# emmyoh/zebra

Measured on NVIDIA B200. Metric: queries_per_sec, higher is better.
Workload: dtype f32

## Files before the change

include/zebra_b200.h:

```cpp
#ifndef ZEBRA_B200_H
#define ZEBRA_B200_H

#include <stddef.h>
#include <stdint.h>

#ifdef __cplusplus
extern "C" {
#endif

#define ZB_ABI_VERSION 2

typedef struct zb_index zb_index;

typedef enum zb_status {
    ZB_OK = 0,
    ZB_ERR_INVALID = -1,
    ZB_ERR_CUDA = -2,
    ZB_ERR_NO_DEVICE = -3,
    ZB_ERR_OOM = -4,
    ZB_ERR_STATE = -5,
    ZB_ERR_COMM = -6
} zb_status;

typedef enum zb_metric {
    ZB_METRIC_COSINE = 0, ZB_METRIC_L2SQ = 1, ZB_METRIC_L2 = 2,
    ZB_METRIC_CHEBYSHEV = 3, ZB_METRIC_CANBERRA = 4, ZB_METRIC_BRAY_CURTIS = 5, ZB_METRIC_MANHATTAN = 6,
    ZB_METRIC_L3 = 7, ZB_METRIC_L4 = 8, ZB_METRIC_HAMMING = 9, ZB_METRIC_MINKOWSKI = 10, ZB_METRIC_PNORM = 11
} zb_metric;
#define ZB_METRIC_COUNT 12
#define ZB_METRIC_MAX_POWER 64

typedef struct zb_options {
    uint32_t dim;
    uint32_t metric;
    uint64_t max_node_size;
    uint32_t num_trees;
    int32_t device;
    uint64_t seed;
    uint32_t shard_rank;
    uint32_t shard_count;
    int32_t metric_power;
    uint32_t reserved[3];
} zb_options;

typedef struct zb_stats {
    uint64_t rows;
    uint64_t live_rows;
    uint64_t total_rows;
    uint64_t nodes, planes, leaves;
    uint64_t device_bytes;
    uint64_t last_queries, last_visits, last_pairs;
    uint64_t last_tile_visits, last_tile_pairs;
    uint64_t last_moved_bytes;
    float last_ms_plan, last_ms_scan, last_ms_select, last_ms_merge, last_ms_total;
    uint32_t last_scan_launches, last_total_launches;
    float last_ms_tile_kernel;
    uint32_t last_tiles;
    uint32_t last_filter_flagged;
    uint64_t last_unique_bytes;
    uint32_t last_filter_rows;
    float last_ms_refine;
    uint32_t last_filter_used;
} zb_stats;

const char* zb_last_error(void);
int zb_abi_version(void);
int zb_device_count(int* out_count);

int zb_index_create(const zb_options* options, zb_index** out_index);
int zb_index_destroy(zb_index* index);
int zb_index_options(zb_index* index, zb_options* out);

int zb_index_add(zb_index* index, uint64_t n, const float* rows, const uint8_t* ids16, uint8_t* out_ids16,
                 uint64_t* out_ordinals);
int zb_index_add_device(zb_index* index, uint64_t n, const float* d_rows, const uint8_t* ids16, uint8_t* out_ids16,
                        uint64_t* out_ordinals);
int zb_index_add_owned_device(zb_index* index, uint64_t n_local, const float* d_rows, const uint64_t* ordinals,
                              uint64_t total_n);

int zb_index_remove(zb_index* index, uint64_t n, const uint8_t* ids16, uint8_t* out_removed);
int zb_index_remove_ordinals(zb_index* index, uint64_t n, const uint64_t* ordinals, uint8_t* out_removed);

int zb_index_deduplicate(zb_index* index, uint64_t* out_count, uint64_t* out_ordinals, uint8_t* out_ids16, uint64_t cap);

int zb_index_clear(zb_index* index);

int zb_index_no_vectors(zb_index* index, int* out);
int zb_index_no_trees(zb_index* index, int* out);

int zb_index_search_batch(zb_index* index, uint64_t nq, const float* queries, uint64_t top_k, uint8_t* out_ids16,
                          uint64_t* out_ordinals, uint64_t* out_dist_bits, uint32_t* out_counts);
int zb_index_search_batch_device(zb_index* index, uint64_t nq, const float* d_queries, uint64_t top_k,
                                 uint64_t* d_out_ordinals, uint64_t* d_out_dist_bits, uint32_t* d_out_counts);
int zb_index_search_slice(zb_index* index, uint64_t nq_total, const float* slice_queries, uint64_t top_k, uint8_t* out_ids16,
                          uint64_t* out_ordinals, uint64_t* out_dist_bits, uint32_t* out_counts);
int zb_index_search_slice_device(zb_index* index, uint64_t nq_total, const float* d_slice_queries, uint64_t top_k,
                                 uint64_t* d_out_ordinals, uint64_t* d_out_dist_bits, uint32_t* d_out_counts);
int zb_index_search_prefetch(zb_index* index, uint64_t n, const float* queries);

int zb_index_search_exact(zb_index* index, uint64_t nq, const float* queries, uint64_t top_k, uint8_t* out_ids16,
                          uint64_t* out_ordinals, uint64_t* out_dist_bits, uint32_t* out_counts);
int zb_index_search_exact_device(zb_index* index, uint64_t nq, const float* d_queries, uint64_t top_k,
                                 uint64_t* d_out_ordinals, uint64_t* d_out_dist_bits, uint32_t* d_out_counts);

#define ZB_MAX_PROBES 32
int zb_index_search_probe(zb_index* index, uint64_t nq, const float* queries, uint64_t top_k, uint32_t probes, uint8_t* out_ids16,
                          uint64_t* out_ordinals, uint64_t* out_dist_bits, uint32_t* out_counts);
int zb_index_search_probe_device(zb_index* index, uint64_t nq, const float* d_queries, uint64_t top_k, uint32_t probes,
                                 uint64_t* d_out_ordinals, uint64_t* d_out_dist_bits, uint32_t* d_out_counts);
int zb_index_search_slice_probe(zb_index* index, uint64_t nq_total, const float* slice_queries, uint64_t top_k, uint32_t probes,
                                uint8_t* out_ids16, uint64_t* out_ordinals, uint64_t* out_dist_bits, uint32_t* out_counts);
int zb_index_search_slice_probe_device(zb_index* index, uint64_t nq_total, const float* d_slice_queries, uint64_t top_k,
                                       uint32_t probes, uint64_t* d_out_ordinals, uint64_t* d_out_dist_bits,
                                       uint32_t* d_out_counts);

int zb_index_hash(zb_index* index, uint64_t n, const float* rows, uint64_t* out_keys, uint32_t* out_depths,
                  int32_t* out_leaves);
int zb_index_hash_device(zb_index* index, uint64_t n, const float* d_rows, uint64_t* d_out_keys,
                         uint32_t* d_out_depths, int32_t* d_out_leaves);

int zb_index_forest_sizes(zb_index* index, int64_t* sizes4);
int zb_index_export_forest(zb_index* index, int32_t* nodes, int32_t* roots, float* coef, float* cst,
                           int64_t* leaf_off, uint64_t* members);
int zb_index_load_forest(zb_index* index, uint64_t n, const float* rows, const uint8_t* ids16,
                         const int64_t* sizes4, const int32_t* nodes, const int32_t* roots, const float* coef,
                         const float* cst, const int64_t* leaf_off, const uint64_t* members);

int zb_tree_blob_decode(uint32_t dim, const uint8_t* blob, uint64_t bytes, int64_t* sizes4, int32_t* nodes, float* coef,
                        float* cst, int64_t* leaf_off, uint8_t* member_ids16);
int zb_tree_blob_encode(uint32_t dim, int64_t n_nodes, const int32_t* nodes, int32_t root, const float* coef,
                        const float* cst, const int64_t* leaf_off, const uint8_t* member_ids16, uint8_t* out,
                        uint64_t cap, uint64_t* out_bytes);
int zb_zebra_file_encode(const uint8_t* uuid16, uint32_t metric, int32_t power, uint64_t max_node_size,
                         uint64_t num_trees, uint8_t* out, uint64_t cap, uint64_t* out_bytes);
int zb_zebra_file_decode(const uint8_t* data, uint64_t bytes, uint32_t metric, uint8_t* out_uuid16, int32_t* out_power,
                         uint64_t* out_max_node_size, uint64_t* out_num_trees);

typedef struct zb_import_report {
    uint64_t rows_loaded;
    uint64_t missing_ids;
    uint64_t orphan_rows;
    uint64_t nodes, planes, leaves;
    uint32_t max_depth;
    uint32_t reserved[3];
} zb_import_report;
typedef struct zb_flat_store zb_flat_store;
int zb_store_flatten(uint32_t dim, uint64_t n, const uint8_t* ids16, uint32_t n_trees, const uint8_t* const* tree_blobs,
                     const uint64_t* tree_blob_bytes, zb_flat_store** out, zb_import_report* report);
int zb_flat_store_view(const zb_flat_store* store, int64_t* sizes4, const int32_t** nodes, const int32_t** roots,
                       const float** coef, const float** cst, const int64_t** leaf_off, const uint64_t** members,
                       const uint32_t** row_order, const uint32_t** orphan_rows);
int zb_flat_store_free(zb_flat_store* store);
int zb_index_import_store(zb_index* index, uint64_t n, const uint8_t* ids16, const float* rows, uint32_t n_trees,
                          const uint8_t* const* tree_blobs, const uint64_t* tree_blob_bytes, zb_import_report* report,
                          uint8_t* out_orphan_ids16, uint64_t orphan_cap);
int zb_index_export_rows(zb_index* index, uint64_t first_ordinal, uint64_t n, float* out_rows, uint8_t* out_ids16,
                         uint8_t* out_live);
int zb_index_export_tree_blob(zb_index* index, uint32_t tree, uint8_t* out, uint64_t cap, uint64_t* out_bytes);
int zb_index_export_tree_blobs(zb_index* index, uint8_t* out, uint64_t cap, uint64_t* out_blob_bytes, uint64_t* out_total);

int zb_index_load_flat(zb_index* index, uint64_t n, const float* rows, const uint8_t* ids16, uint32_t bits,
                       const float* coef, const float* cst);

int zb_index_stats(zb_index* index, zb_stats* out);
int zb_index_stream(zb_index* index, void** out_stream);
int zb_index_set_param(zb_index* index, const char* key, int64_t value);

int zb_comm_unique_id(uint8_t* out_id128);
int zb_index_comm_init(zb_index* index, const uint8_t* id128);

int zb_metric_distance_batch(int device, uint32_t metric, int32_t power, uint64_t n, uint32_t dim, const float* a,
                             const float* b, uint64_t* out_bits);
int zb_point_is_above_batch(int device, uint64_t n, uint32_t dim, const float* coef, const float* cst, const float* x,
                            uint8_t* out);

int zb_synth_fill_device(int device, float* d_out, uint64_t first_row, uint64_t row_stride, uint64_t n, uint32_t dim,
                         uint64_t seed, uint32_t kind);

#ifdef __cplusplus
}
#endif
#endif
```

zebra_b200/_ffi.py:

```python
from __future__ import annotations

import ctypes as C
import os

_HERE = os.path.dirname(os.path.abspath(__file__))
LIB_PATH = os.path.join(_HERE, "libzebra_b200.so")

ZB_OK = 0
METRIC_COSINE, METRIC_L2SQ, METRIC_L2 = 0, 1, 2
(METRIC_CHEBYSHEV, METRIC_CANBERRA, METRIC_BRAY_CURTIS, METRIC_MANHATTAN, METRIC_L3, METRIC_L4, METRIC_HAMMING,
 METRIC_MINKOWSKI, METRIC_PNORM) = range(3, 12)
METRIC_MAX_POWER = 64


class ZebraError(RuntimeError):
    def __init__(self, code: int, msg: str):
        super().__init__(f"zebra_b200 error {code}: {msg}")
        self.code = code


class Options(C.Structure):
    _fields_ = [
        ("dim", C.c_uint32),
        ("metric", C.c_uint32),
        ("max_node_size", C.c_uint64),
        ("num_trees", C.c_uint32),
        ("device", C.c_int32),
        ("seed", C.c_uint64),
        ("shard_rank", C.c_uint32),
        ("shard_count", C.c_uint32),
        ("metric_power", C.c_int32),
        ("reserved", C.c_uint32 * 3),
    ]


class Stats(C.Structure):
    _fields_ = [
        ("rows", C.c_uint64),
        ("live_rows", C.c_uint64),
        ("total_rows", C.c_uint64),
        ("nodes", C.c_uint64),
        ("planes", C.c_uint64),
        ("leaves", C.c_uint64),
        ("device_bytes", C.c_uint64),
        ("last_queries", C.c_uint64),
        ("last_visits", C.c_uint64),
        ("last_pairs", C.c_uint64),
        ("last_tile_visits", C.c_uint64),
        ("last_tile_pairs", C.c_uint64),
        ("last_moved_bytes", C.c_uint64),
        ("last_ms_plan", C.c_float),
        ("last_ms_scan", C.c_float),
        ("last_ms_select", C.c_float),
        ("last_ms_merge", C.c_float),
        ("last_ms_total", C.c_float),
        ("last_scan_launches", C.c_uint32),
        ("last_total_launches", C.c_uint32),
        ("last_ms_tile_kernel", C.c_float),
        ("last_tiles", C.c_uint32),
        ("last_filter_flagged", C.c_uint32),
        ("last_unique_bytes", C.c_uint64),
        ("last_filter_rows", C.c_uint32),
        ("last_ms_refine", C.c_float),
        ("last_filter_used", C.c_uint32),
    ]

    def as_dict(self):
        return {n: getattr(self, n) for n, _ in self._fields_ if not n.startswith("reserved")}


class ImportReport(C.Structure):
    _fields_ = [
        ("rows_loaded", C.c_uint64),
        ("missing_ids", C.c_uint64),
        ("orphan_rows", C.c_uint64),
        ("nodes", C.c_uint64),
        ("planes", C.c_uint64),
        ("leaves", C.c_uint64),
        ("max_depth", C.c_uint32),
        ("reserved", C.c_uint32 * 3),
    ]

    def as_dict(self):
        return {n: getattr(self, n) for n, _ in self._fields_ if not n.startswith("reserved")}


_vp, _u64, _u32, _i32, _i64 = C.c_void_p, C.c_uint64, C.c_uint32, C.c_int32, C.c_int64
SYMBOLS = {
    "zb_last_error": (C.c_char_p, []),
    "zb_abi_version": (C.c_int, []),
    "zb_device_count": (C.c_int, [_vp]),
    "zb_index_create": (C.c_int, [C.POINTER(Options), C.POINTER(_vp)]),
    "zb_index_destroy": (C.c_int, [_vp]),
    "zb_index_options": (C.c_int, [_vp, C.POINTER(Options)]),
    "zb_index_add": (C.c_int, [_vp, _u64, _vp, _vp, _vp, _vp]),
    "zb_index_add_device": (C.c_int, [_vp, _u64, _vp, _vp, _vp, _vp]),
    "zb_index_add_owned_device": (C.c_int, [_vp, _u64, _vp, _vp, _u64]),
    "zb_index_remove": (C.c_int, [_vp, _u64, _vp, _vp]),
    "zb_index_remove_ordinals": (C.c_int, [_vp, _u64, _vp, _vp]),
    "zb_index_deduplicate": (C.c_int, [_vp, C.POINTER(_u64), _vp, _vp, _u64]),
    "zb_index_clear": (C.c_int, [_vp]),
    "zb_index_no_vectors": (C.c_int, [_vp, _vp]),
    "zb_index_no_trees": (C.c_int, [_vp, _vp]),
    "zb_index_search_batch": (C.c_int, [_vp, _u64, _vp, _u64, _vp, _vp, _vp, _vp]),
    "zb_index_search_batch_device": (C.c_int, [_vp, _u64, _vp, _u64, _vp, _vp, _vp]),
    "zb_index_search_slice": (C.c_int, [_vp, _u64, _vp, _u64, _vp, _vp, _vp, _vp]),
    "zb_index_search_slice_device": (C.c_int, [_vp, _u64, _vp, _u64, _vp, _vp, _vp]),
    "zb_index_search_prefetch": (C.c_int, [_vp, _u64, _vp]),
    "zb_index_search_exact": (C.c_int, [_vp, _u64, _vp, _u64, _vp, _vp, _vp, _vp]),
    "zb_index_search_exact_device": (C.c_int, [_vp, _u64, _vp, _u64, _vp, _vp, _vp]),
    "zb_index_search_probe": (C.c_int, [_vp, _u64, _vp, _u64, C.c_uint32, _vp, _vp, _vp, _vp]),
    "zb_index_search_probe_device": (C.c_int, [_vp, _u64, _vp, _u64, C.c_uint32, _vp, _vp, _vp]),
    "zb_index_search_slice_probe": (C.c_int, [_vp, _u64, _vp, _u64, C.c_uint32, _vp, _vp, _vp, _vp]),
    "zb_index_search_slice_probe_device": (C.c_int, [_vp, _u64, _vp, _u64, C.c_uint32, _vp, _vp, _vp]),
    "zb_index_hash": (C.c_int, [_vp, _u64, _vp, _vp, _vp, _vp]),
    "zb_index_hash_device": (C.c_int, [_vp, _u64, _vp, _vp, _vp, _vp]),
    "zb_index_forest_sizes": (C.c_int, [_vp, _vp]),
    "zb_index_export_forest": (C.c_int, [_vp, _vp, _vp, _vp, _vp, _vp, _vp]),
    "zb_index_load_forest": (C.c_int, [_vp, _u64, _vp, _vp, _vp, _vp, _vp, _vp, _vp, _vp, _vp]),
    "zb_tree_blob_decode": (C.c_int, [_u32, _vp, _u64, _vp, _vp, _vp, _vp, _vp, _vp]),
    "zb_tree_blob_encode": (C.c_int, [_u32, _i64, _vp, _i32, _vp, _vp, _vp, _vp, _vp, _u64, C.POINTER(_u64)]),
    "zb_zebra_file_encode": (C.c_int, [_vp, _u32, _i32, _u64, _u64, _vp, _u64, C.POINTER(_u64)]),
    "zb_zebra_file_decode": (C.c_int, [_vp, _u64, _u32, _vp, C.POINTER(_i32), C.POINTER(_u64), C.POINTER(_u64)]),
    "zb_store_flatten": (C.c_int, [_u32, _u64, _vp, _u32, _vp, _vp, C.POINTER(_vp), C.POINTER(ImportReport)]),
    "zb_flat_store_view": (C.c_int, [_vp] + [_vp] * 9),
    "zb_flat_store_free": (C.c_int, [_vp]),
    "zb_index_import_store": (C.c_int, [_vp, _u64, _vp, _vp, _u32, _vp, _vp, C.POINTER(ImportReport), _vp, _u64]),
    "zb_index_export_rows": (C.c_int, [_vp, _u64, _u64, _vp, _vp, _vp]),
    "zb_index_export_tree_blob": (C.c_int, [_vp, _u32, _vp, _u64, C.POINTER(_u64)]),
    "zb_index_export_tree_blobs": (C.c_int, [_vp, _vp, _u64, _vp, C.POINTER(_u64)]),
    "zb_index_load_flat": (C.c_int, [_vp, _u64, _vp, _vp, _u32, _vp, _vp]),
    "zb_index_stats": (C.c_int, [_vp, C.POINTER(Stats)]),
    "zb_index_stream": (C.c_int, [_vp, C.POINTER(_vp)]),
    "zb_index_set_param": (C.c_int, [_vp, C.c_char_p, _i64]),
    "zb_comm_unique_id": (C.c_int, [_vp]),
    "zb_index_comm_init": (C.c_int, [_vp, _vp]),
    "zb_metric_distance_batch": (C.c_int, [C.c_int, _u32, _i32, _u64, _u32, _vp, _vp, _vp]),
    "zb_point_is_above_batch": (C.c_int, [C.c_int, _u64, _u32, _vp, _vp, _vp, _vp]),
    "zb_synth_fill_device": (C.c_int, [C.c_int, _vp, _u64, _u64, _u64, _u32, _u64, _u32]),
}

_lib = None


def lib():
    global _lib
    if _lib is None:
        if not os.path.exists(LIB_PATH):
            raise ImportError(
                f"{LIB_PATH} is missing: build it with `make -C zebra_b200` (or __graft_entry__.build()); "
                "zebra_b200 has no CPU fallback"
            )
        L = C.CDLL(LIB_PATH, mode=C.RTLD_GLOBAL)
        for name, (res, args) in SYMBOLS.items():
            fn = getattr(L, name)
            fn.restype = res
            fn.argtypes = args
        _lib = L
    return _lib


def check(rc: int) -> None:
    if rc != ZB_OK:
        msg = lib().zb_last_error()
        raise ZebraError(rc, msg.decode("utf-8", "replace") if msg else "?")
```

zebra_b200/csrc/zb_index.cu:

```cuda
#include <algorithm>
#include <chrono>
#include <mutex>
#include <unordered_map>

#include "zb_host.h"
#include "zb_kernels.cuh"
#include "zb_scan.cuh"

namespace zb {
size_t g_device_bytes = 0;
thread_local std::string t_last_error;

struct Id16 {
    uint64_t hi, lo;
    bool operator==(const Id16& o) const { return hi == o.hi && lo == o.lo; }
};
struct Id16Hash {
    size_t operator()(const Id16& k) const { return (size_t)mix64(k.hi ^ mix64(k.lo)); }
};
static inline uint64_t load_be64(const uint8_t* p) {
    uint64_t v = 0;
    for (int i = 0; i < 8; ++i) v = (v << 8) | p[i];
    return v;
}
static inline void store_be64(uint8_t* p, uint64_t v) {
    for (int i = 7; i >= 0; --i) {
        p[i] = (uint8_t)v;
        v >>= 8;
    }
}

__global__ void remap_leaves_kernel(int* leaves, u64 n, const int* __restrict__ table) {
    u64 i = (u64)blockIdx.x * blockDim.x + threadIdx.x;
    if (i < n) leaves[i] = table[leaves[i]];
}
__global__ void count_live_kernel(const u32* __restrict__ members, const long long* __restrict__ leaf_off,
                                  const u32* __restrict__ leaf_len, const u32* __restrict__ tomb, u32 nleaves,
                                  u32* __restrict__ leaf_live) {
    u32 l = blockIdx.x * blockDim.x + threadIdx.x;
    if (l >= nleaves) return;
    u32 c = 0;
    const u32* m = members + leaf_off[l];
    for (u32 i = 0; i < leaf_len[l]; ++i) c += tomb_test(tomb, m[i]) ? 0u : 1u;
    leaf_live[l] = c;
}

struct BSeg {
    u64 key;
    int depth, node, tree;
    long long off;
    u32 len;
    u64 glen;
    u32 attempt;
};

}

using namespace zb;

struct zb_index {
    std::mutex mu;
    zb_options opt{};
    int dim = 0, dimp = 0, chunks = 0, T = 0, device = 0;
    u32 G = 1, rank = 0;
    cudaStream_t stream = nullptr;
    cudaEvent_t ev[8]{};
    Nccl nccl;
    bool comm_ready = false;
    u64 epoch_ms = 0;

    DBuf<float> rows;
    DBuf<u64> ord;
    DBuf<float> row_norm;
    DBuf<u32> tomb;
    DBuf<u32> slot_leaf;
    u64 slot_stride = 0;
    u64 n_slots = 0, n_live = 0, total_rows = 0;
    std::vector<u64> h_ord;
    std::vector<uint8_t> h_tomb;
    int id_mode = 0;
    std::vector<Id16> ids_by_ordinal;
    std::unordered_map<Id16, u64, Id16Hash> ordinal_by_id;

    std::vector<int4> h_nodes;
    std::vector<int> h_roots;
    u64 n_planes = 0;
    std::vector<long long> h_leaf_off;
    std::vector<u32> h_leaf_len, h_leaf_cap;
    std::vector<u64> h_leaf_key;
    std::vector<int> h_leaf_depth, h_leaf_node, h_leaf_tree;
    u64 members_used = 0;
    std::vector<u32> h_members;
    bool h_members_valid = false;
    bool built = false;
    u32 flat_bits = 0;
    size_t flat_nodes = 0;
    DBuf<u8> pj_sign;
    DBuf<int4> d_nodes;
    DBuf<int> d_roots;
    DBuf<float> d_coef, d_cst;
    DBuf<long long> d_leaf_off;
    DBuf<u32> d_leaf_len, d_leaf_live, d_leaf_plan, d_members;
    DBuf<int> d_leaf_export;
    bool export_table_valid = false;

    DBuf<float> bm_rows;
    DBuf<double> bm_rinv, q_rinv;
    DBuf<u32> w_tail;
    DBuf<float> bm_n2, bm_leaf_n2max;
    int filter_backoff = 0;
    DBuf<u32> bm_tomb, slot_pos, d_leaf_tree;
    alignas(64) unsigned char bm_tmap[128];
    alignas(64) unsigned char bm_tmap3[128];
    bool bm_valid = false, bm_failed = false;
    u64 bm_positions = 0;
    DBuf<long long> d_bm_off;
    DBuf<u32> d_bm_len;
    DBuf<u64> bm_ord;
    DBuf<u32> d_iota;
    DBuf<u64> srt_ord;
    DBuf<u32> srt_pos;
    DBuf<u64> d_tree_base, rm_ords;
    std::vector<u64> h_tree_base;
    DBuf<u64> loc_results;
    DBuf<u64> res_all;

    DBuf<u8> cub_tmp;
    DBuf<u32> w_counts, w_off, w_flag, w_loc_off, v_w, x_flags, x_pos;
    DBuf<uint4> x_send, x_all;
    u32 x_cap = 0;
    DBuf<float> q_all;
    struct PeerQ {
        float* mine = nullptr;
        u64 cap = 0;
        std::vector<float*> peer;
        bool failed = false;
        static const int NS = 4;
        cudaStream_t stream[NS] = {};
        cudaEvent_t fork = nullptr, done[NS] = {};
    } pq;
    DBuf<u64> plan_totals;
    DBuf<uint2> w_visits;
    u32 vpw = 32;
    DBuf<u32> v_leaf, v_np, v_q, v_ent_len, v_ent_off;
    DBuf<u64> v_pair_len, v_pair_off, pair_key;
    DBuf<u8> v_done;
    DBuf<Entry> entries, gathered;
    DBuf<float> q_stage, r_stage, hash_in;
    struct Prefetch {
        DBuf<float> buf;
        const float* host = nullptr;
        u64 rows = 0, seq = 0;
        cudaEvent_t done = nullptr;
    } pf[2];
    cudaStream_t copy_stream = nullptr;
    u64 pf_seq = 0;
    DBuf<u64> o_ord, o_bits, h_keys;
    DBuf<u32> o_counts, o_counts2, h_depths, rm_slots;
    DBuf<int> h_leaves;
    DBuf<u8> rm_flags;
    HBuf<u8> pin;
    DBuf<u32> b_work[2], b_flags, b_scan, b_above;
    DBuf<Tile> b_tiles;
    DBuf<SegDesc> b_segs;
    DBuf<u64> b_minh, b_minord, b_excl;
    DBuf<int> b_slot_a, b_slot_b;
    DBuf<float> b_pair_rows;
    ScanWorkspace scan_ws;
    ScanWorkspace pj_ws;
    ScanWorkspace qt_ws;
    ScanWorkspace ex_ws;
    u64 store_gen = 0, ex_gen = ~0ull;
    DBuf<u32> ex_iota, ex_counts;
    DBuf<double> ex_rinv;
    DBuf<float> ex_n2;
    DBuf<u64> ex_loc, ex_gath, ex_nmax;

    int64_t p_tile_min_rows = 64, p_tile_queries = 0, p_use_tile_scan = 1, p_hash_variant = 0, p_classify_variant = 0, p_seq_tile = 1, p_seq_prefetch = 0, p_flat_project = 1, p_quad_tile = 1, p_select_variant = 1, p_scan_gen = 3, p_bm_stage_mb = 2048, p_single_exchange = 1, p_p2p_queries = 1, p_l2_filter = 1, p_plan_tail = 1, p_exact_budget_mb = 256;
    zb_stats st{};

    ForestView view() const {
        ForestView f;
        f.nodes = d_nodes.p;
        f.roots = d_roots.p;
        f.coef = d_coef.p;
        f.cst = d_cst.p;
        f.leaf_off = d_leaf_off.p;
        f.leaf_len = d_leaf_len.p;
        f.leaf_plan = G > 1 ? d_leaf_plan.p : d_leaf_live.p;
        f.members = d_members.p;
        f.rows = rows.p;
        f.ord = ord.p;
        f.row_norm = row_norm.p;
        f.tomb = tomb.p;
        f.dimp = dimp;
        f.dim = dim;
        f.chunks = chunks;
        f.num_trees = T;
        return f;
    }
    ForestView scan_view() const {
        ForestView f = view();
        if (G > 1) {
            f.leaf_off = d_bm_off.p;
            f.leaf_len = d_bm_len.p;
            f.members = d_iota.p;
            f.rows = bm_rows.p;
            f.ord = bm_ord.p;
            f.tomb = bm_tomb.p;
            f.row_norm = nullptr;
        }
        return f;
    }
    bool trace_on = getenv("ZB_TRACE") != nullptr;
    bool trace_all = getenv("ZB_TRACE") != nullptr && atoi(getenv("ZB_TRACE")) >= 2;
    std::vector<std::pair<const char*, cudaEvent_t>> trace_ev;
    size_t trace_n = 0;
    void trace_mark(const char* what) {
        if (!trace_on) return;
        if (trace_n == trace_ev.size()) {
            cudaEvent_t e;
            ZB_CUDA(cudaEventCreate(&e));
            trace_ev.push_back({what, e});
        }
        trace_ev[trace_n].first = what;
        ZB_CUDA(cudaEventRecord(trace_ev[trace_n++].second, stream));
    }
    void trace_dump() {
        if (!trace_on || trace_n < 2) { trace_n = 0; return; }
        sync();
        if (rank == 0 || trace_all) {
            std::string line = fmt("[zb trace r%u]", rank);
            for (size_t i = 1; i < trace_n; ++i) {
                float ms = 0.f;
                cudaEventElapsedTime(&ms, trace_ev[i - 1].second, trace_ev[i].second);
                line += fmt(" %s %.3f |", trace_ev[i].first, ms);
            }
            line += "\n";
            fputs(line.c_str(), stderr);
        }
        trace_n = 0;
    }
    void sync() { ZB_CUDA(cudaStreamSynchronize(stream)); }
    void use_device() { ZB_CUDA(cudaSetDevice(device)); }
    void scan_tmp(size_t n) {
        size_t need = scan_temp_bytes(n);
        cub_tmp.ensure(need);
    }
    bool owns(u64 ordinal) const { return G <= 1 || ordinal % G == rank; }
    u64 slot_of(u64 ordinal) const { return G <= 1 ? ordinal : ordinal / G; }

    Id16 mint(u64 ordinal) const {
        uint64_t hi = (epoch_ms << 16) | 0x7000ull | ((ordinal >> 52) & 0xFFFull);
        uint64_t lo = (0x2ull << 62) | (((ordinal >> 46) & 0x3Full) << 56) | ((ordinal & ((1ull << 46) - 1)) << 10);
        return Id16{hi, lo};
    }
    bool unmint(const Id16& id, u64* ordinal) const {
        if ((id.hi >> 16) != (epoch_ms & 0xFFFFFFFFFFFFull) || ((id.hi >> 12) & 0xF) != 7 || (id.lo >> 62) != 2 ||
            (id.lo & 0x3FF))
            return false;
        *ordinal = ((id.hi & 0xFFFull) << 52) | (((id.lo >> 56) & 0x3Full) << 46) | ((id.lo >> 10) & ((1ull << 46) - 1));
        return true;
    }
    void id_of(u64 ordinal, uint8_t* out16) const {
        Id16 id = id_mode == 2 ? (ordinal < ids_by_ordinal.size() ? ids_by_ordinal[ordinal] : Id16{~0ull, ~0ull})
                               : mint(ordinal);
        store_be64(out16, id.hi);
        store_be64(out16 + 8, id.lo);
    }
    bool ordinal_of(const uint8_t* id16, u64* ordinal) const {
        Id16 id{load_be64(id16), load_be64(id16 + 8)};
        if (id_mode == 2) {
            auto it = ordinal_by_id.find(id);
            if (it == ordinal_by_id.end()) return false;
            *ordinal = it->second;
            return true;
        }
        return unmint(id, ordinal) && *ordinal < total_rows;
    }

    void reserve_slots(u64 need) {
        if (need <= slot_stride) return;
        u64 ncap = slot_stride ? slot_stride + slot_stride / 2 : need;
        if (ncap < need) ncap = need;
        ncap = (ncap + 31) & ~31ull;
        rows.ensure(ncap * (u64)dimp, n_slots * (u64)dimp, stream, true);
        ord.ensure(ncap, n_slots, stream, true);
        row_norm.ensure(ncap, n_slots, stream, true);
        size_t old_words = tomb.cap;
        tomb.ensure(ncap / 32 + 3, (n_slots + 31) / 32, stream, true);
        (void)old_words;
        DBuf<u32> nsl;
        nsl.ensure(ncap * (u64)T, 0, stream, true);
        if (slot_leaf.p && n_slots)
            ZB_CUDA(cudaMemcpy2DAsync(nsl.p, ncap * 4, slot_leaf.p, slot_stride * 4, n_slots * 4, T, cudaMemcpyDeviceToDevice,
                                      stream));
        sync();
        std::swap(nsl.p, slot_leaf.p);
        std::swap(nsl.cap, slot_leaf.cap);
        slot_stride = ncap;
    }
    void append_rows_device(const float* d_src, u64 src_stride, u64 n_local, const u64* ordinals) {
        if (!n_local) return;
        reserve_slots(n_slots + n_local);
        float* dst = rows.p + n_slots * (u64)dimp;
        if (dimp == dim) {
            ZB_CUDA(cudaMemcpy2DAsync(dst, (size_t)dimp * 4, d_src, src_stride * 4, (size_t)dim * 4, n_local,
                                      cudaMemcpyDeviceToDevice, stream));
        } else {
            ZB_REQUIRE(src_stride == (u64)dim, ZB_ERR_INVALID, "strided device rows need dim %% 16 == 0");
            launch_pad_rows(d_src, n_local, dim, dimp, dst, stream);
        }
        ZB_CUDA(cudaMemcpyAsync(ord.p + n_slots, ordinals, n_local * 8, cudaMemcpyHostToDevice, stream));
        if (opt.metric == ZB_METRIC_COSINE) launch_sq_norms(dst, n_local, dimp, row_norm.p + n_slots, stream);
        u64 w0 = (n_slots + 31) / 32, w1 = (n_slots + n_local + 31) / 32;
        if (n_slots == 0) w0 = 0;
        if (w1 > w0) ZB_CUDA(cudaMemsetAsync(tomb.p + w0, 0, (w1 - w0) * 4, stream));
        sync();
        h_ord.insert(h_ord.end(), ordinals, ordinals + n_local);
        h_tomb.resize(h_tomb.size() + n_local, 0);
        n_slots += n_local;
        n_live += n_local;
        ++store_gen;
    }
    void ensure_exact_side() {
        if (ex_gen == store_gen) return;
        const u64 n = n_slots ? n_slots : 1;
        ex_iota.ensure(n);
        launch_iota_u32(ex_iota.p, n_slots, 0u, stream);
        if (opt.metric == ZB_METRIC_COSINE) {
            ex_rinv.ensure(n);
            launch_rinv(rows.p, n_slots, dimp, ex_rinv.p, stream);
        } else {
            ex_n2.ensure(n);
            launch_n2(rows.p, n_slots, dimp, ex_n2.p, stream);
        }
        ex_gen = store_gen;
    }

    void upload_structure() {
        size_t nn = h_nodes.size(), nl = h_leaf_off.size();
        d_nodes.ensure(nn ? nn : 1);
        d_roots.ensure(T);
        d_leaf_off.ensure(nl ? nl : 1);
        d_leaf_len.ensure(nl ? nl : 1);
        if (nn) ZB_CUDA(cudaMemcpyAsync(d_nodes.p, h_nodes.data(), nn * sizeof(int4), cudaMemcpyHostToDevice, stream));
        ZB_CUDA(cudaMemcpyAsync(d_roots.p, h_roots.data(), (size_t)T * 4, cudaMemcpyHostToDevice, stream));
        if (nl) {
            ZB_CUDA(cudaMemcpyAsync(d_leaf_off.p, h_leaf_off.data(), nl * 8, cudaMemcpyHostToDevice, stream));
            ZB_CUDA(cudaMemcpyAsync(d_leaf_len.p, h_leaf_len.data(), nl * 4, cudaMemcpyHostToDevice, stream));
        }
        sync();
        export_table_valid = false;
        bm_valid = false;
    }
    bool ensure_bucket_major() {
        if (bm_valid) return true;
        if (G > 1) return ensure_bucket_major_sharded();
        if (bm_failed || !built || !members_used) return false;
        const u32 nl = (u32)h_leaf_off.size();
        try {
            bm_rows.ensure(members_used * (u64)dimp, 0, stream, true);
            bm_tomb.ensure(members_used / 32 + 8);
            slot_pos.ensure(slot_stride * (u64)T);
            d_leaf_tree.ensure(nl);
            if (opt.metric == ZB_METRIC_COSINE) bm_rinv.ensure(members_used);
            if (opt.metric == ZB_METRIC_L2SQ || opt.metric == ZB_METRIC_L2) {
                bm_n2.ensure(members_used);
                bm_leaf_n2max.ensure(nl ? nl : 1);
            }
        } catch (const Error& e) {
            if (e.code != ZB_ERR_OOM) throw;
            bm_rows.release();
            bm_failed = true;
            return false;
        }
        std::vector<u32> lt(h_leaf_tree.begin(), h_leaf_tree.end());
        ZB_CUDA(cudaMemcpyAsync(d_leaf_tree.p, lt.data(), (size_t)nl * 4, cudaMemcpyHostToDevice, stream));
        ZB_CUDA(cudaMemsetAsync(bm_tomb.p, 0, (members_used / 32 + 8) * 4, stream));
        u64 used = 0;
        for (u32 l = 0; l < nl; ++l) used += h_leaf_len[l];
        if (used != members_used) ZB_CUDA(cudaMemsetAsync(bm_rows.p, 0, members_used * (u64)dimp * 4, stream));
        launch_bm_gather(nl, d_leaf_off.p, d_leaf_len.p, d_leaf_tree.p, d_members.p, rows.p, tomb.p, dimp, slot_stride, bm_rows.p,
                         slot_pos.p, bm_tomb.p, stream);
        if (opt.metric == ZB_METRIC_COSINE) launch_rinv(bm_rows.p, members_used, dimp, bm_rinv.p, stream);
        if (opt.metric == ZB_METRIC_L2SQ || opt.metric == ZB_METRIC_L2) {
            launch_n2(bm_rows.p, members_used, dimp, bm_n2.p, stream);
            launch_leaf_n2max(nl, d_leaf_off.p, d_leaf_len.p, bm_n2.p, bm_leaf_n2max.p, stream);
        }
        make_row_tile_map(bm_tmap, bm_rows.p, members_used, dimp, 128, tile_scan_box_floats(2));
        make_row_tile_map(bm_tmap3, bm_rows.p, members_used, dimp, 64, tile_scan_box_floats(3));
        sync();
        bm_positions = members_used;
        bm_valid = true;
        return true;
    }
    bool ensure_bucket_major_sharded() {
        ZB_REQUIRE(comm_ready, ZB_ERR_STATE, "sharded index used before zb_index_comm_init");
        ZB_REQUIRE(total_rows < (1ull << 40), ZB_ERR_STATE, "bucket-sharded store supports up to 2^40 rows");
        const u32 nl = (u32)h_leaf_off.size();
        sync_host_members();
        DBuf<u32> d_all;
        d_all.ensure((size_t)nl * G);
        nccl.allgather(d_leaf_len.p, d_all.p, (size_t)nl * 4, stream);
        std::vector<u32> all_len((size_t)nl * G);
        ZB_CUDA(cudaMemcpyAsync(all_len.data(), d_all.p, all_len.size() * 4, cudaMemcpyDeviceToHost, stream));
        sync();
        std::vector<std::vector<u32>> owned(T);
        for (u32 l = 0; l < nl; ++l)
            if (h_leaf_node[l] >= 0 && l % G == rank) owned[h_leaf_tree[l]].push_back(l);
        std::vector<long long> off(nl, 0);
        std::vector<u32> len(nl, 0);
        h_tree_base.assign(T + 1, 0);
        u64 P = 0;
        for (int t = 0; t < T; ++t) {
            h_tree_base[t] = P;
            for (u32 l : owned[t]) {
                u64 g = 0;
                for (u32 r = 0; r < G; ++r) g += all_len[(size_t)r * nl + l];
                off[l] = (long long)P;
                len[l] = (u32)g;
                P += g;
            }
        }
        h_tree_base[T] = P;
        ZB_REQUIRE(P < (1ull << 31), ZB_ERR_STATE, "more than 2^31 bucket-major positions on one rank");
        const u64 Pa = P ? P : 1;
        bm_rows.ensure(Pa * (u64)dimp, 0, stream, true);
        bm_ord.ensure(Pa);
        bm_tomb.ensure(Pa / 32 + 8);
        d_iota.ensure(Pa);
        srt_ord.ensure(Pa);
        srt_pos.ensure(Pa);
        d_bm_off.ensure(nl ? nl : 1);
        d_bm_len.ensure(nl ? nl : 1);
        d_tree_base.ensure(T + 1);
        if (opt.metric == ZB_METRIC_COSINE) bm_rinv.ensure(Pa);
        if (opt.metric == ZB_METRIC_L2SQ || opt.metric == ZB_METRIC_L2) {
            bm_n2.ensure(Pa);
            bm_leaf_n2max.ensure(nl ? nl : 1);
        }
        ZB_CUDA(cudaMemsetAsync(bm_tomb.p, 0, (Pa / 32 + 8) * 4, stream));
        if (nl) {
            ZB_CUDA(cudaMemcpyAsync(d_bm_off.p, off.data(), (size_t)nl * 8, cudaMemcpyHostToDevice, stream));
            ZB_CUDA(cudaMemcpyAsync(d_bm_len.p, len.data(), (size_t)nl * 4, cudaMemcpyHostToDevice, stream));
        }
        ZB_CUDA(cudaMemcpyAsync(d_tree_base.p, h_tree_base.data(), (size_t)(T + 1) * 8, cudaMemcpyHostToDevice, stream));
        launch_iota_u32(d_iota.p, P, 0u, stream);
        sync();
        DBuf<u32> d_slots, sort_val[2];
        DBuf<float> snd_rows, st_rows;
        DBuf<u64> snd_key, st_key, sort_key[2];
        DBuf<RecvSeg> d_segs;
        DBuf<u8> sort_tmp;
        std::vector<std::vector<u32>> by_tree(T);
        for (u32 l = 0; l < nl; ++l)
            if (h_leaf_node[l] >= 0) by_tree[h_leaf_tree[l]].push_back(l);
        const u64 stage_rows = std::max<u64>(4096, (u64)p_bm_stage_mb * (1ull << 20) / ((u64)dimp * 4));
        for (int t = 0; t < T; ++t) {
            const std::vector<u32>& tl = by_tree[t];
            size_t own_i = 0;
            u64 tree_pos = h_tree_base[t];
            for (size_t g0 = 0; g0 < tl.size();) {
                std::vector<u64> snd_r(G, 0), st_r(G, 0);
                size_t g1 = g0;
                for (; g1 < tl.size(); ++g1) {
                    const u32 l = tl[g1];
                    u64 gl = 0, worst = 0;
                    for (u32 r = 0; r < G; ++r) gl += all_len[(size_t)r * nl + l];
                    for (u32 r = 0; r < G; ++r)
                        worst = std::max(worst, std::max(snd_r[r] + all_len[(size_t)r * nl + l], st_r[r] + (l % G == r ? gl : 0)));
                    if (g1 > g0 && worst > stage_rows) break;
                    for (u32 r = 0; r < G; ++r) snd_r[r] += all_len[(size_t)r * nl + l];
                    st_r[l % G] += gl;
                }
                std::vector<u32> slots;
                std::vector<u64> send_off(G + 1, 0);
                for (u32 d = 0; d < G; ++d) {
                    send_off[d] = slots.size();
                    for (size_t i = g0; i < g1; ++i) {
                        const u32 l = tl[i];
                        if (l % G == d)
                            slots.insert(slots.end(), h_members.begin() + h_leaf_off[l], h_members.begin() + h_leaf_off[l] + h_leaf_len[l]);
                    }
                }
                send_off[G] = slots.size();
                size_t own_j = own_i;
                while (own_j < owned[t].size() && owned[t][own_j] <= tl[g1 - 1]) ++own_j;
                std::vector<RecvSeg> segs;
                std::vector<u64> recv_off(G + 1, 0);
                u64 R = 0;
                for (u32 r = 0; r < G; ++r) {
                    recv_off[r] = R;
                    for (size_t i = own_i; i < own_j; ++i) {
                        const u32 c = all_len[(size_t)r * nl + owned[t][i]];
                        if (c) segs.push_back(RecvSeg{R, c, (u32)(i - own_i)});
                        R += c;
                    }
                }
                recv_off[G] = R;
                ZB_REQUIRE(R == st_r[rank], ZB_ERR_STATE, "bucket-sharded layout mismatch");
                ZB_REQUIRE(own_j - own_i < (1u << 24), ZB_ERR_STATE, "too many leaves in one exchange group");
                const u64 ns = slots.size();
                d_slots.ensure(ns ? ns : 1);
                snd_rows.ensure((ns ? ns : 1) * (u64)dimp);
                snd_key.ensure(ns ? ns : 1);
                st_rows.ensure((R ? R : 1) * (u64)dimp);
                st_key.ensure(R ? R : 1);
                for (int b = 0; b < 2; ++b) {
                    sort_key[b].ensure(R ? R : 1);
                    sort_val[b].ensure(R ? R : 1);
                }
                d_segs.ensure(segs.size() ? segs.size() : 1);
                sort_tmp.ensure(sort_temp_bytes(R ? R : 1));
                if (ns) ZB_CUDA(cudaMemcpyAsync(d_slots.p, slots.data(), ns * 4, cudaMemcpyHostToDevice, stream));
                if (!segs.empty()) ZB_CUDA(cudaMemcpyAsync(d_segs.p, segs.data(), segs.size() * sizeof(RecvSeg), cudaMemcpyHostToDevice, stream));
                launch_pack_rows(d_slots.p, ns, rows.p, ord.p, tomb.p, dimp, snd_rows.p, snd_key.p, stream);
                const size_t rb = (size_t)dimp * 4;
                nccl.group_start();
                for (u32 r = 0; r < G; ++r) {
                    if (r == rank) continue;
                    const u64 sc = send_off[r + 1] - send_off[r], rc = recv_off[r + 1] - recv_off[r];
                    nccl.send(snd_rows.p + send_off[r] * (u64)dimp, sc * rb, (int)r, stream);
                    nccl.send(snd_key.p + send_off[r], sc * 8, (int)r, stream);
                    nccl.recv(st_rows.p + recv_off[r] * (u64)dimp, rc * rb, (int)r, stream);
                    nccl.recv(st_key.p + recv_off[r], rc * 8, (int)r, stream);
                }
                nccl.group_end();
                {
                    const u64 sc = send_off[rank + 1] - send_off[rank];
                    ZB_REQUIRE(sc == recv_off[rank + 1] - recv_off[rank], ZB_ERR_STATE, "bucket-sharded self share mismatch");
                    if (sc) {
                        ZB_CUDA(cudaMemcpyAsync(st_rows.p + recv_off[rank] * (u64)dimp, snd_rows.p + send_off[rank] * (u64)dimp, sc * rb,
                                                cudaMemcpyDeviceToDevice, stream));
                        ZB_CUDA(cudaMemcpyAsync(st_key.p + recv_off[rank], snd_key.p + send_off[rank], sc * 8, cudaMemcpyDeviceToDevice, stream));
                    }
                }
                launch_seg_keys(d_segs.p, (u32)segs.size(), st_key.p, sort_key[0].p, sort_val[0].p, stream);
                sort_pairs_u64_u32(sort_tmp.p, sort_tmp.bytes(), sort_key[0].p, sort_key[1].p, sort_val[0].p, sort_val[1].p, R, 64, stream);
                launch_place_rows(sort_val[1].p, R, st_rows.p, st_key.p, dimp, tree_pos, bm_rows.p, bm_ord.p, bm_tomb.p, stream);
                sync();
                tree_pos += R;
                own_i = own_j;
                g0 = g1;
            }
            ZB_REQUIRE(tree_pos == h_tree_base[t + 1] && own_i == owned[t].size(), ZB_ERR_STATE, "bucket-sharded layout mismatch");
            const u64 Rt = h_tree_base[t + 1] - h_tree_base[t];
            sort_tmp.ensure(sort_temp_bytes(Rt ? Rt : 1));
            sort_pairs_u64_u32(sort_tmp.p, sort_tmp.bytes(), bm_ord.p + h_tree_base[t], srt_ord.p + h_tree_base[t],
                               d_iota.p + h_tree_base[t], srt_pos.p + h_tree_base[t], Rt, 40, stream);
            sync();
        }
        if (opt.metric == ZB_METRIC_COSINE) launch_rinv(bm_rows.p, P, dimp, bm_rinv.p, stream);
        if (opt.metric == ZB_METRIC_L2SQ || opt.metric == ZB_METRIC_L2) {
            launch_n2(bm_rows.p, P, dimp, bm_n2.p, stream);
            launch_leaf_n2max(nl, d_bm_off.p, d_bm_len.p, bm_n2.p, bm_leaf_n2max.p, stream);
        }
        make_row_tile_map(bm_tmap, bm_rows.p, Pa, dimp, 128, tile_scan_box_floats(2));
        make_row_tile_map(bm_tmap3, bm_rows.p, Pa, dimp, 64, tile_scan_box_floats(3));
        sync();
        bm_positions = P;
        bm_valid = true;
        return true;
    }
    bool ensure_peer_queries(u64 need) {
        if (pq.failed || !p_p2p_queries) return false;
        if (need <= pq.cap && !pq.peer.empty()) return true;
        release_peer_queries();
        const u64 ncap = need + need / 2;
        u32 ok = 1;
        if (cudaMalloc((void**)&pq.mine, ncap * 4) != cudaSuccess) { cudaGetLastError(); pq.mine = nullptr; ok = 0; }
        cudaIpcMemHandle_t h;
        memset(&h, 0, sizeof h);
        if (ok && cudaIpcGetMemHandle(&h, pq.mine) != cudaSuccess) { cudaGetLastError(); ok = 0; }
        const size_t rec = 80;
        DBuf<u8> d_rec, d_all;
        d_rec.ensure(rec);
        d_all.ensure(rec * G);
        u8 hrec[80];
        memset(hrec, 0, sizeof hrec);
        memcpy(hrec, &h, sizeof h);
        memcpy(hrec + 64, &ok, 4);
        ZB_CUDA(cudaMemcpyAsync(d_rec.p, hrec, rec, cudaMemcpyHostToDevice, stream));
        nccl.allgather(d_rec.p, d_all.p, rec, stream);
        std::vector<u8> all(rec * G);
        ZB_CUDA(cudaMemcpyAsync(all.data(), d_all.p, rec * G, cudaMemcpyDeviceToHost, stream));
        sync();
        bool all_ok = true;
        for (u32 r = 0; r < G; ++r) {
            u32 f = 0;
            memcpy(&f, all.data() + r * rec + 64, 4);
            all_ok = all_ok && f;
        }
        pq.peer.assign(G, nullptr);
        u32 mapped = all_ok ? 1u : 0u;
        if (all_ok) {
            for (u32 r = 0; r < G && mapped; ++r) {
                if (r == rank) { pq.peer[r] = pq.mine; continue; }
                cudaIpcMemHandle_t ph;
                memcpy(&ph, all.data() + r * rec, sizeof ph);
                void* ptr = nullptr;
                if (cudaIpcOpenMemHandle(&ptr, ph, cudaIpcMemLazyEnablePeerAccess) != cudaSuccess) { cudaGetLastError(); mapped = 0; }
                pq.peer[r] = (float*)ptr;
            }
        }
        DBuf<u32> d_flag;
        d_flag.ensure(1);
        ZB_CUDA(cudaMemcpyAsync(d_flag.p, &mapped, 4, cudaMemcpyHostToDevice, stream));
        nccl.allreduce(d_flag.p, 1, Nccl::U32, Nccl::MIN, stream);
        ZB_CUDA(cudaMemcpyAsync(&mapped, d_flag.p, 4, cudaMemcpyDeviceToHost, stream));
        sync();
        if (!mapped) {
            release_peer_queries();
            pq.failed = true;
            return false;
        }
        if (!pq.fork) {
            ZB_CUDA(cudaEventCreateWithFlags(&pq.fork, cudaEventDisableTiming));
            for (int i = 0; i < PeerQ::NS; ++i) {
                ZB_CUDA(cudaStreamCreateWithFlags(&pq.stream[i], cudaStreamNonBlocking));
                ZB_CUDA(cudaEventCreateWithFlags(&pq.done[i], cudaEventDisableTiming));
            }
        }
        pq.cap = ncap;
        g_device_bytes += ncap * 4;
        return true;
    }
    void release_peer_queries() {
        cudaDeviceSynchronize();
        for (u32 r = 0; r < pq.peer.size(); ++r)
            if (r != rank && pq.peer[r]) cudaIpcCloseMemHandle(pq.peer[r]);
        pq.peer.clear();
        if (pq.mine) {
            cudaFree(pq.mine);
            if (pq.cap) g_device_bytes -= pq.cap * 4;
        }
        pq.mine = nullptr;
        pq.cap = 0;
    }
    BucketMajor bm_view() const {
        BucketMajor b;
        b.rows = bm_rows.p;
        b.rinv = bm_rinv.p;
        b.tomb = bm_tomb.p;
        if (opt.metric == ZB_METRIC_L2SQ || opt.metric == ZB_METRIC_L2) {
            b.n2 = bm_n2.p;
            b.leaf_n2max = bm_leaf_n2max.p;
        }
        b.tmap = bm_tmap;
        b.tmap3 = bm_tmap3;
        b.positions = bm_positions;
        return b;
    }
    void recount_live() {
        u32 nl = (u32)h_leaf_off.size();
        d_leaf_live.ensure(nl ? nl : 1);
        d_leaf_plan.ensure(nl ? nl : 1);
        if (nl) count_live_kernel<<<(nl + 127) / 128, 128, 0, stream>>>(d_members.p, d_leaf_off.p, d_leaf_len.p, tomb.p, nl, d_leaf_live.p);
        refresh_plan_counts();
    }
    void refresh_plan_counts() {
        u32 nl = (u32)h_leaf_off.size();
        if (G > 1 && nl) {
            ZB_REQUIRE(comm_ready, ZB_ERR_STATE, "sharded index used before zb_index_comm_init");
            d_leaf_plan.ensure(nl);
            ZB_CUDA(cudaMemcpyAsync(d_leaf_plan.p, d_leaf_live.p, (size_t)nl * 4, cudaMemcpyDeviceToDevice, stream));
            nccl.allreduce(d_leaf_plan.p, nl, Nccl::U32, Nccl::SUM, stream);
        }
    }
    void sync_host_members() {
        if (h_members_valid) return;
        h_members.resize(members_used);
        if (members_used)
            ZB_CUDA(cudaMemcpyAsync(h_members.data(), d_members.p, members_used * 4, cudaMemcpyDeviceToHost, stream));
        sync();
        h_members_valid = true;
    }
    int new_leaf(int node, int tree, u64 key, int depth, long long off, u32 len, u32 cap) {
        int id = (int)h_leaf_off.size();
        h_leaf_off.push_back(off);
        h_leaf_len.push_back(len);
        h_leaf_cap.push_back(cap);
        h_leaf_key.push_back(key);
        h_leaf_depth.push_back(depth);
        h_leaf_node.push_back(node);
        h_leaf_tree.push_back(tree);
        return id;
    }

    void clear_forest() {
        h_nodes.clear();
        h_roots.assign(T, -1);
        n_planes = 0;
        h_leaf_off.clear(); h_leaf_len.clear(); h_leaf_cap.clear(); h_leaf_key.clear();
        h_leaf_depth.clear(); h_leaf_node.clear(); h_leaf_tree.clear();
        members_used = 0;
        h_members.clear();
        h_members_valid = false;
        built = false;
        export_table_valid = false;
        bm_valid = false;
        bm_failed = false;
    }

    void build_subtrees(std::vector<BSeg> active, u64 total) {
        const u64 max_node = opt.max_node_size;
        auto t_start = std::chrono::steady_clock::now();
        int level = 0;
        std::vector<BSeg> leaves;
        int cur = 0;
        b_work[1].ensure(total ? total : 1);
        b_flags.ensure(total + 1);
        b_scan.ensure(total + 1);
        scan_tmp(total + 1);
        std::vector<SegDesc> hsegs;
        std::vector<Tile> htiles;
        std::vector<u32> habove, hgabove;
        while (true) {
            std::vector<BSeg> split, next;
            for (const BSeg& s : active) {
                if (s.glen < max_node || s.glen < 2 || s.depth >= ZB_MAX_DEPTH || s.attempt >= ZB_MAX_ATTEMPTS) leaves.push_back(s);
                else split.push_back(s);
            }
            if (split.empty()) break;
            const u32 ns = (u32)split.size();
            d_coef.ensure((n_planes + ns) * (u64)dimp, n_planes * (u64)dimp, stream);
            d_cst.ensure(n_planes + ns, n_planes, stream);
            hsegs.resize(ns);
            htiles.clear();
            for (u32 i = 0; i < ns; ++i) {
                const BSeg& s = split[i];
                hsegs[i] = SegDesc{s.off, s.len, (u32)(n_planes + i), s.key, s.attempt, 0};
                for (u32 b = 0; b < s.len; b += 64) htiles.push_back(Tile{i, std::min<u32>(64, s.len - b), s.off + b});
            }
            const u32 nt = (u32)htiles.size();
            b_segs.ensure(ns);
            b_tiles.ensure(nt ? nt : 1);
            b_minh.ensure(ns); b_minord.ensure(ns); b_excl.ensure(ns);
            b_slot_a.ensure(ns); b_slot_b.ensure(ns); b_above.ensure(2 * (size_t)ns);
            b_pair_rows.ensure((size_t)ns * 2 * dimp);
            ZB_CUDA(cudaMemcpyAsync(b_segs.p, hsegs.data(), ns * sizeof(SegDesc), cudaMemcpyHostToDevice, stream));
            if (nt) ZB_CUDA(cudaMemcpyAsync(b_tiles.p, htiles.data(), nt * sizeof(Tile), cudaMemcpyHostToDevice, stream));
            const u32* work = b_work[cur].p;
            for (int which = 0; which < 2; ++which) {
                int* slot_out = which ? b_slot_b.p : b_slot_a.p;
                const u64* excl = which ? b_excl.p : nullptr;
                ZB_CUDA(cudaMemsetAsync(b_minh.p, 0xFF, ns * 8, stream));
                ZB_CUDA(cudaMemsetAsync(b_minord.p, 0xFF, ns * 8, stream));
                ZB_CUDA(cudaMemsetAsync(slot_out, 0xFF, ns * 4, stream));
                launch_pick(0, b_tiles.p, nt, b_segs.p, work, ord.p, excl, b_minh.p, b_minord.p, slot_out, stream);
                if (G > 1) nccl.allreduce(b_minh.p, ns, Nccl::U64, Nccl::MIN, stream);
                launch_pick(1, b_tiles.p, nt, b_segs.p, work, ord.p, excl, b_minh.p, b_minord.p, slot_out, stream);
                if (G > 1) nccl.allreduce(b_minord.p, ns, Nccl::U64, Nccl::MIN, stream);
                launch_pick(2, b_tiles.p, nt, b_segs.p, work, ord.p, excl, b_minh.p, b_minord.p, slot_out, stream);
                if (!which) ZB_CUDA(cudaMemcpyAsync(b_excl.p, b_minord.p, ns * 8, cudaMemcpyDeviceToDevice, stream));
            }
            launch_fetch_pair_rows(b_segs.p, ns, b_slot_a.p, b_slot_b.p, rows.p, dimp, b_pair_rows.p, stream);
            if (G > 1) nccl.allreduce(b_pair_rows.p, (size_t)ns * 2 * dimp, Nccl::I32, Nccl::SUM, stream);
            launch_make_planes(b_segs.p, ns, b_pair_rows.p, dimp, d_coef.p, d_cst.p, stream);
            ZB_CUDA(cudaMemsetAsync(b_flags.p, 0, (total + 1) * 4, stream));
            launch_classify(b_tiles.p, nt, b_segs.p, work, rows.p, d_coef.p, d_cst.p, dimp, b_flags.p, (int)p_classify_variant, stream);
            exclusive_scan_u32(cub_tmp.p, cub_tmp.bytes(), b_flags.p, b_scan.p, total + 1, stream);
            launch_seg_above(b_segs.p, ns, b_scan.p, b_above.p, stream);
            habove.resize(ns);
            hgabove.resize(ns);
            ZB_CUDA(cudaMemcpyAsync(habove.data(), b_above.p, ns * 4, cudaMemcpyDeviceToHost, stream));
            if (G > 1) {
                ZB_CUDA(cudaMemcpyAsync(b_above.p + ns, b_above.p, ns * 4, cudaMemcpyDeviceToDevice, stream));
                nccl.allreduce(b_above.p + ns, ns, Nccl::U32, Nccl::SUM, stream);
                ZB_CUDA(cudaMemcpyAsync(hgabove.data(), b_above.p + ns, ns * 4, cudaMemcpyDeviceToHost, stream));
            }
            if (total) ZB_CUDA(cudaMemcpyAsync(b_work[cur ^ 1].p, work, total * 4, cudaMemcpyDeviceToDevice, stream));
            launch_scatter(b_tiles.p, nt, b_segs.p, work, b_flags.p, b_scan.p, b_work[cur ^ 1].p, stream);
            sync();
            cur ^= 1;
            if (G <= 1) hgabove = habove;
            for (u32 i = 0; i < ns; ++i) {
                BSeg s = split[i];
                const u64 ga = hgabove[i], gb = s.glen - ga;
                if (ga == 0 || gb == 0) {
                    s.attempt++;
                    next.push_back(s);
                    continue;
                }
                const u32 la = habove[i], lb = s.len - la;
                const int nl = (int)h_nodes.size(), nr = nl + 1;
                h_nodes.push_back(make_int4(-1, -1, -1, -1));
                h_nodes.push_back(make_int4(-1, -1, -1, -1));
                h_nodes[s.node] = make_int4((int)(n_planes + i), nl, nr, -1);
                next.push_back(BSeg{child_key(s.key, 0), s.depth + 1, nl, s.tree, s.off, lb, gb, 0});
                next.push_back(BSeg{child_key(s.key, 1), s.depth + 1, nr, s.tree, s.off + lb, la, ga, 0});
            }
            n_planes += ns;
            active.swap(next);
            if (trace_on && rank == 0) {
                auto now = std::chrono::steady_clock::now();
                fprintf(stderr, "[zb trace] build level %d: %u nodes, %u tiles, %.3f ms\n", level, ns, nt,
                        std::chrono::duration<double, std::milli>(now - t_start).count());
                t_start = now;
            }
            ++level;
        }
        d_members.ensure(members_used + total, members_used, stream);
// ... 160 lines not shown
        const u64 slice = nqp * (u64)ix->dimp;
        ZB_CUDA(cudaEventRecord(ix->pq.fork, s));
        for (int i = 0; i < zb_index::PeerQ::NS; ++i) ZB_CUDA(cudaStreamWaitEvent(ix->pq.stream[i], ix->pq.fork, 0));
        for (u32 i = 0; i < G; ++i) {
            const u32 r = (ix->rank + i) % G;
            cudaStream_t ps = ix->pq.stream[i % zb_index::PeerQ::NS];
            float* dst = ix->pq.peer[r] + (u64)ix->rank * slice;
            if (qn) ZB_CUDA(cudaMemcpyAsync(dst, d_q, qn * (u64)ix->dimp * 4, cudaMemcpyDeviceToDevice, ps));
            if (qn < nqp) ZB_CUDA(cudaMemsetAsync(dst + qn * (u64)ix->dimp, 0, (nqp - qn) * (u64)ix->dimp * 4, ps));
        }
        for (int i = 0; i < zb_index::PeerQ::NS; ++i) ZB_CUDA(cudaEventRecord(ix->pq.done[i], ix->pq.stream[i]));
        d_q = ix->pq.mine;
    } else if (one_exchange) {
        ix->q_all.ensure(nqp * G * (u64)ix->dimp);
        d_q = ix->q_all.p;
    } else if (sliced) {
        ix->q_all.ensure(nqp * G * (u64)ix->dimp);
        float* mine = ix->q_all.p + (u64)ix->rank * nqp * ix->dimp;
        if (qn) ZB_CUDA(cudaMemcpyAsync(mine, d_q, qn * (u64)ix->dimp * 4, cudaMemcpyDeviceToDevice, s));
        if (qn < nqp) ZB_CUDA(cudaMemsetAsync(mine + qn * (u64)ix->dimp, 0, (nqp - qn) * (u64)ix->dimp * 4, s));
        ix->nccl.allgather(mine, ix->q_all.p, nqp * (u64)ix->dimp * 4, s);
        d_q = ix->q_all.p;
        ix->trace_mark("allgather of queries");
    }
    ix->w_counts.ensure(nw + 1);
    ix->w_off.ensure(nw + 1);
    ix->w_flag.ensure(4);
    ix->scan_tmp(nw + 1);
    u32 nv = 0, total_slots = 0;
    u64 total_pairs = 0;
    const bool gen3 = ix->p_scan_gen != 2 && tile_scan3_supported(ix->dimp, (u32)top_k);
    const bool tile_on = ix->opt.metric <= ZB_METRIC_L2 && ix->p_use_tile_scan && ix->opt.max_node_size >= (u64)ix->p_tile_min_rows &&
                         (gen3 || tile_scan_supported(ix->dimp, (u32)top_k)) && ix->ensure_bucket_major();
    u64 v_cap = std::max<u64>(ix->v_leaf.cap ? ix->v_leaf.cap - 1 : 0, nw * (1 + (u64)probes) + nw / 2 + 1024);
    if (probes) ix->vpw = std::max<u32>(ix->vpw, 32 + probes);
    if (sharded && !ix->x_cap) ix->x_cap = (u32)std::min<u64>(nwl + nwl / 2 + 64, 0x7FFFFFFFull);
    ix->plan_totals.ensure(8);
    bool need_plan = true, need_exchange = true;
    for (;;) {
        ix->v_leaf.ensure(v_cap + 1); ix->v_np.ensure(v_cap + 1); ix->v_q.ensure(v_cap + 1);
        ix->v_pair_len.ensure(v_cap + 1); ix->v_pair_off.ensure(v_cap + 1);
        ix->v_ent_len.ensure(v_cap + 1); ix->v_ent_off.ensure(v_cap + 1);
        ix->v_done.ensure(v_cap + 1);
        if (sharded) ix->v_w.ensure(v_cap + 1);
        ix->scan_tmp(std::max<u64>(std::max<u64>(nw, v_cap), sharded ? (u64)G * ix->x_cap : 0) + 1);
        if (need_plan) {
            ix->w_visits.ensure(nwl * ix->vpw);
            ZB_CUDA(cudaMemsetAsync(ix->w_flag.p, 0, 16, s));
            ZB_CUDA(cudaMemsetAsync(ix->w_counts.p + nwl, 0, 4, s));
            if (sharded && qn < nqp) {
                ZB_CUDA(cudaMemsetAsync(ix->w_visits.p + qn * T * ix->vpw, 0, (nqp - qn) * T * ix->vpw * sizeof(uint2), s));
                ZB_CUDA(cudaMemsetAsync(ix->w_counts.p + qn * T, 0, (nqp - qn) * T * 4, s));
            }
            u32* tail = nullptr;
            if (ix->p_plan_tail && ix->opt.max_node_size >= 4 * top_k) {
                ix->w_tail.ensure(nwl + 2);
                tail = ix->w_tail.p;
            }
            launch_plan(f, d_q_mine, (u32)qn, (u32)top_k, probes, ix->vpw, ix->w_visits.p, ix->w_counts.p, ix->w_flag.p, tail, s);
            if (tail) ix->st.last_total_launches += 1;
            ix->trace_mark("plan walk");
            if (sharded) {
                ix->w_loc_off.ensure(nwl + 1);
                exclusive_scan_u32(ix->cub_tmp.p, ix->cub_tmp.bytes(), ix->w_counts.p, ix->w_loc_off.p, nwl + 1, s);
            }
            need_plan = false;
            need_exchange = true;
            ix->st.last_total_launches += 1;
        }
        const size_t q4 = one_exchange ? (size_t)nqp * ix->dimp / 4 : 0;
        if (sharded && need_exchange) {
            const u32 C = ix->x_cap;
            const size_t B4 = (size_t)C + 1 + q4;
            ix->x_send.ensure(B4);
            ix->x_all.ensure(B4 * G);
            ix->x_flags.ensure((size_t)C * G + 1);
            ix->x_pos.ensure((size_t)C * G + 1);
            launch_pack_visits((u32)nwl, ix->vpw, ix->w_visits.p, ix->w_counts.p, ix->w_loc_off.p, (u32)((u64)ix->rank * nwl), C,
                               ix->w_flag.p, ix->x_send.p, s);
            if (one_exchange) {
                float* qdst = reinterpret_cast<float*>(ix->x_send.p + (size_t)C + 1);
                if (qn) ZB_CUDA(cudaMemcpyAsync(qdst, d_q_mine, qn * (u64)ix->dimp * 4, cudaMemcpyDeviceToDevice, s));
                if (qn < nqp) ZB_CUDA(cudaMemsetAsync(qdst + qn * (u64)ix->dimp, 0, (nqp - qn) * (u64)ix->dimp * 4, s));
            }
            if (p2p)
                for (int i = 0; i < zb_index::PeerQ::NS; ++i) ZB_CUDA(cudaStreamWaitEvent(s, ix->pq.done[i], 0));
            ix->nccl.allgather(ix->x_send.p, ix->x_all.p, B4 * sizeof(uint4), s);
            ix->trace_mark(p2p ? "push of queries + allgather of visits" : one_exchange ? "allgather of visits + queries" : "allgather of visits");
            if (one_exchange)
                ZB_CUDA(cudaMemcpy2DAsync(ix->q_all.p, (size_t)nqp * ix->dimp * 4, ix->x_all.p + (size_t)C + 1, B4 * sizeof(uint4),
                                          (size_t)nqp * ix->dimp * 4, G, cudaMemcpyDeviceToDevice, s));
            launch_own_flags(G, C, B4, ix->x_all.p, ix->rank, ix->x_flags.p, ix->w_flag.p + 2, s);
            exclusive_scan_u32(ix->cub_tmp.p, ix->cub_tmp.bytes(), ix->x_flags.p, ix->x_pos.p, (size_t)C * G + 1, s);
            need_exchange = false;
            ix->st.last_total_launches += 3;
        }
        ZB_CUDA(cudaMemsetAsync(ix->v_pair_len.p, 0, (v_cap + 1) * 8, s));
        ZB_CUDA(cudaMemsetAsync(ix->v_ent_len.p, 0, (v_cap + 1) * 4, s));
        if (sharded) {
            const u32 C = ix->x_cap;
            launch_own_scatter(fs, G, C, (size_t)C + 1 + q4, ix->x_all.p, ix->x_flags.p, ix->x_pos.p, (u32)v_cap, tile_on ? 1u : 0u, (u32)ix->p_tile_min_rows,
                               (u32)top_k, ix->v_leaf.p, ix->v_np.p, ix->v_q.p, ix->v_w.p, ix->v_pair_len.p, ix->v_ent_len.p,
                               ix->v_done.p, s);
            launch_walker_offsets((u32)nw, ix->x_pos.p + (size_t)C * G, (u32)v_cap, ix->v_w.p, ix->w_off.p, s);
        } else {
            exclusive_scan_u32(ix->cub_tmp.p, ix->cub_tmp.bytes(), ix->w_counts.p, ix->w_off.p, nw + 1, s);
            launch_compact_visits(fs, (u32)nw, ix->vpw, ix->w_visits.p, ix->w_counts.p, ix->w_off.p, 1, 0, (u32)v_cap,
                                  tile_on ? 1u : 0u, (u32)ix->p_tile_min_rows, (u32)top_k, ix->v_leaf.p, ix->v_np.p, ix->v_q.p,
                                  ix->v_pair_len.p, ix->v_ent_len.p, ix->v_done.p, s);
        }
        exclusive_scan_u32(ix->cub_tmp.p, ix->cub_tmp.bytes(), ix->v_ent_len.p, ix->v_ent_off.p, v_cap + 1, s);
        exclusive_scan_u64(ix->cub_tmp.p, ix->cub_tmp.bytes(), ix->v_pair_len.p, ix->v_pair_off.p, v_cap + 1, s);
        launch_plan_totals(sharded ? ix->w_flag.p + 2 : ix->w_flag.p, ix->w_off.p, (u32)nw, (u32)v_cap, ix->v_ent_off.p, ix->v_pair_off.p,
                           sharded ? ix->w_flag.p + 3 : nullptr, ix->plan_totals.p, s);
        u64 h_tot[5] = {0, 0, 0, 0, 0};
        ZB_CUDA(cudaMemcpyAsync(h_tot, ix->plan_totals.p, 40, cudaMemcpyDeviceToHost, s));
        ix->sync();
        ix->st.last_total_launches += 6;
        if (h_tot[0]) {
            ZB_REQUIRE(h_tot[0] == 1, ZB_ERR_STATE, "forest deeper than %d levels", ZB_MAX_DEPTH);
            ix->vpw *= 2;
            ZB_REQUIRE(ix->vpw <= (1u << 16), ZB_ERR_STATE, "visit plan does not converge");
            need_plan = true;
            continue;
        }
        if (sharded && h_tot[4] > ix->x_cap) {
            ix->x_cap = (u32)std::min<u64>(h_tot[4] + h_tot[4] / 4 + 64, 0x7FFFFFFFull);
            need_exchange = true;
            continue;
        }
        nv = (u32)h_tot[1];
        if (nv > v_cap) {
            v_cap = (u64)nv + nv / 4;
            continue;
        }
        total_slots = (u32)h_tot[2];
        total_pairs = h_tot[3];
        break;
    }
    ZB_CUDA(cudaEventRecord(ix->ev[1], s));
    ix->trace_mark("compact");

    ix->entries.ensure(total_slots ? total_slots : 1);
    ix->pair_key.ensure(total_pairs ? total_pairs : 1);
    u64 tile_pairs = 0, tile_visits = 0, moved = 0;
    u32 scan_launches = 0;
    ix->scan_ws.launched = false;
    if (nv && tile_on) {
        if (ix->opt.metric == ZB_METRIC_COSINE) {
            ix->q_rinv.ensure(nq);
            launch_rinv(d_q, nq, ix->dimp, ix->q_rinv.p, s);
        }
        ix->scan_ws.l2_filter = gen3 && ix->dimp >= 128 && (ix->p_l2_filter == 2 || (ix->p_l2_filter == 1 && ix->filter_backoff == 0));
        if (ix->filter_backoff > 0) --ix->filter_backoff;
        (gen3 ? tile_scan3 : tile_scan)(ix->scan_ws, fs, ix->bm_view(), ix->opt.metric, d_q, ix->q_rinv.p, (u32)nq, nv, ix->v_leaf.p,
                                        ix->v_np.p, ix->v_q.p, ix->v_ent_off.p, ix->v_pair_len.p, ix->v_done.p, ix->entries.p,
                                        (u32)top_k, (u32)ix->p_tile_min_rows, (u32)ix->p_tile_queries,
                                        (u32)ix->h_leaf_off.size(), s);
        ZB_REQUIRE(ix->scan_ws.launched, ZB_ERR_STATE, "tile scan did not launch for visits set aside for it");
        scan_launches = ix->scan_ws.launches + (ix->opt.metric == ZB_METRIC_COSINE ? 1 : 0);
    }

    ix->scan_ws.seq_launched = false;
    if (ix->opt.metric > ZB_METRIC_L2 && ix->p_seq_tile && total_pairs && seq_tile_scan_supported(ix->dimp))
        seq_tile_scan(ix->scan_ws, fs, ix->opt.metric, (int)ix->opt.metric_power, d_q, nv, ix->v_leaf.p, ix->v_q.p, ix->v_pair_off.p,
                      ix->pair_key.p, (u32)ix->h_leaf_off.size(), (int)ix->p_seq_prefetch, s);
    ix->qt_ws.seq_launched = false;
    if (ix->opt.metric <= ZB_METRIC_L2 && ix->p_quad_tile && total_pairs && quad_tile_scan_supported(ix->dimp))
        quad_tile_scan(ix->qt_ws, fs, ix->opt.metric, d_q, nv, ix->v_leaf.p, ix->v_q.p, ix->v_pair_off.p, ix->pair_key.p,
                       (u32)ix->h_leaf_off.size(), s);
    if (!ix->scan_ws.seq_launched && !ix->qt_ws.seq_launched)
        launch_score_pairs(fs, (int)ix->opt.metric, (int)ix->opt.metric_power, d_q, nv, ix->v_leaf.p, ix->v_q.p, ix->v_pair_off.p,
                           total_pairs, ix->pair_key.p, s);
    ZB_CUDA(cudaEventRecord(ix->ev[2], s));
    ix->trace_mark("scan");
    if (total_pairs)
        launch_select_visits(fs, nv, ix->v_leaf.p, ix->v_np.p, ix->v_pair_off.p, ix->pair_key.p, ix->v_ent_off.p,
                             ix->entries.p, ix->v_done.p, (u32)top_k, (int)ix->p_select_variant, s);
    ZB_CUDA(cudaEventRecord(ix->ev[3], s));
    ix->trace_mark("select");
    if (sharded) {
        const u64 nsk = nqp * top_k;
        const u64 nqP = nqp * G;
        u64* loc_ord = nullptr;
        u64* loc_bits = nullptr;
        ix->loc_results.ensure(2 * nqP * top_k + 1);
        loc_ord = ix->loc_results.p;
        loc_bits = loc_ord + nqP * top_k;
        if (nqP > nq) {
            ZB_CUDA(cudaMemsetAsync(loc_ord + nq * top_k, 0xFF, (nqP - nq) * top_k * 8, s));
            ZB_CUDA(cudaMemsetAsync(loc_bits + nq * top_k, 0xFF, (nqP - nq) * top_k * 8, s));
        }
        ix->o_counts.ensure(nq);
        launch_merge_queries((u32)nq, T, ix->w_off.p, ix->v_ent_off.p, ix->entries.p, (u32)top_k, loc_ord, loc_bits, ix->o_counts.p, s);
        ix->trace_mark("local merge");
        u64* gath = reinterpret_cast<u64*>((ix->gathered.ensure((size_t)nsk * G + 1), ix->gathered.p));
        ix->nccl.group_start();
        for (u32 r = 0; r < G; ++r) {
            if (r == ix->rank) continue;
            ix->nccl.send(loc_ord + (u64)r * nsk, nsk * 8, (int)r, s);
            ix->nccl.send(loc_bits + (u64)r * nsk, nsk * 8, (int)r, s);
            ix->nccl.recv(gath + (u64)r * 2 * nsk, nsk * 8, (int)r, s);
            ix->nccl.recv(gath + (u64)r * 2 * nsk + nsk, nsk * 8, (int)r, s);
        }
        ix->nccl.group_end();
        ZB_CUDA(cudaMemcpyAsync(gath + (u64)ix->rank * 2 * nsk, loc_ord + (u64)ix->rank * nsk, nsk * 8, cudaMemcpyDeviceToDevice, s));
        ZB_CUDA(cudaMemcpyAsync(gath + (u64)ix->rank * 2 * nsk + nsk, loc_bits + (u64)ix->rank * nsk, nsk * 8, cudaMemcpyDeviceToDevice, s));
        ix->trace_mark("all-to-all of local top-k");
        if (sliced) {
            launch_merge_gathered((u32)qn, (u32)nqp, (u32)top_k, G, gath, d_out_ord, d_out_bits, d_out_counts, s);
            ix->trace_mark("final merge of my slice");
        } else {
            const u64 blk = 2 * nsk + (nqp + 1) / 2;
            ix->res_all.ensure(blk * G + 1);
            u64* mine = ix->res_all.p + (u64)ix->rank * blk;
            launch_merge_gathered((u32)qn, (u32)nqp, (u32)top_k, G, gath, mine, mine + nsk, reinterpret_cast<u32*>(mine + 2 * nsk), s);
            ix->trace_mark("final merge of my slice");
            ix->nccl.allgather(mine, ix->res_all.p, blk * 8, s);
            launch_unpack_results(ix->res_all.p, blk, (u32)nq, (u32)nqp, (u32)top_k, d_out_ord, d_out_bits, d_out_counts, s);
        }
    } else {
        launch_merge_queries((u32)nq, T, ix->w_off.p, ix->v_ent_off.p, ix->entries.p, (u32)top_k, d_out_ord, d_out_bits,
                             d_out_counts, s);
    }
    ZB_CUDA(cudaEventRecord(ix->ev[4], s));
    ix->trace_mark(sharded ? "allgather of results" : "merge");
    float tile_ms = 0.f;
    u32 tiles = 0;
    u64 unique_bytes = 0;
    u64 flagged = 0, refined = 0;
    float refine_ms = 0.f;
    tile_scan_stats(ix->scan_ws, s, &tile_visits, &tile_pairs, &moved, &tile_ms, &tiles, &unique_bytes, &flagged, &refined, &refine_ms);
    ix->st.last_unique_bytes = unique_bytes;
    ix->st.last_filter_flagged = (u32)std::min<u64>(flagged, 0xFFFFFFFFull);
    ix->st.last_filter_rows = (u32)std::min<u64>(refined, 0xFFFFFFFFull);
    ix->st.last_ms_refine = refine_ms;
    ix->st.last_filter_used = ix->scan_ws.launched && ix->scan_ws.filtered ? 1u : 0u;
    if (ix->scan_ws.launched && ix->scan_ws.filtered && flagged * 16 > tile_visits) ix->filter_backoff = 32;
    u64 seq_moved = 0;
    if (ix->scan_ws.seq_launched) seq_tile_scan_stats(ix->scan_ws, s, &seq_moved, &tile_ms, &tiles);
    u64 qt_moved = 0;
    if (ix->qt_ws.seq_launched) {
        float qt_ms = 0.f;
        u32 qt_tiles = 0;
        seq_tile_scan_stats(ix->qt_ws, s, &qt_moved, &qt_ms, &qt_tiles);
        tile_ms += qt_ms;
        tiles += qt_tiles;
    }
    ix->st.last_ms_tile_kernel = tile_ms;
    ix->st.last_tiles = tiles;
    ix->sync();
    float ms;
    ix->trace_dump();
    cudaEventElapsedTime(&ms, ix->ev[0], ix->ev[1]); ix->st.last_ms_plan = ms;
    cudaEventElapsedTime(&ms, ix->ev[1], ix->ev[2]); ix->st.last_ms_scan = ms;
    cudaEventElapsedTime(&ms, ix->ev[2], ix->ev[3]); ix->st.last_ms_select = ms;
    cudaEventElapsedTime(&ms, ix->ev[3], ix->ev[4]); ix->st.last_ms_merge = ms;
    cudaEventElapsedTime(&ms, ix->ev[0], ix->ev[4]); ix->st.last_ms_total = ms;
    ix->st.last_visits = nv;
    ix->st.last_pairs = total_pairs + tile_pairs;
    ix->st.last_tile_visits = tile_visits;
    ix->st.last_tile_pairs = tile_pairs;
    ix->st.last_moved_bytes = ix->scan_ws.seq_launched ? seq_moved
                              : (ix->qt_ws.seq_launched ? moved + qt_moved : moved + total_pairs * (u64)ix->dim * 4);
    ix->st.last_scan_launches = scan_launches + (total_pairs ? (ix->scan_ws.seq_launched ? 7 : 1) : 0);
    ix->st.last_total_launches += scan_launches + 5 + (sharded ? 1 : 0) + ((ix->scan_ws.seq_launched || ix->qt_ws.seq_launched) ? 6 : 0);
}

static void exact_device(zb_index* ix, u64 nq, const float* d_q, u64 top_k, u64* d_out_ord, u64* d_out_bits, u32* d_out_counts) {
    cudaStream_t s = ix->stream;
    if (!nq) return;
    if (!top_k) {
        ZB_CUDA(cudaMemsetAsync(d_out_counts, 0, nq * 4, s));
        return;
    }
    const u32 G = ix->G;
    const bool sharded = G > 1;
    u64 n_max = ix->n_slots;
    if (sharded) {
        ix->ex_nmax.ensure(1);
        ZB_CUDA(cudaMemcpyAsync(ix->ex_nmax.p, &n_max, 8, cudaMemcpyHostToDevice, s));
        ix->nccl.allreduce(ix->ex_nmax.p, 1, Nccl::U64, Nccl::MAX, s);
        ZB_CUDA(cudaMemcpyAsync(&n_max, ix->ex_nmax.p, 8, cudaMemcpyDeviceToHost, s));
        ix->sync();
    }
    const u32 metric = ix->opt.metric;
    const bool filt = (metric == ZB_METRIC_L2SQ || metric == ZB_METRIC_L2) && top_k <= ZB_L2_FILTER_MAX_K && ix->dimp >= 128;
    ix->ensure_exact_side();
    const u64 per_query = 24 + (sharded ? 16 * top_k * (G + 1) + 4 : 0);
    const ExactPlan p = exact_plan(n_max, nq, ix->dimp, (u32)top_k, filt, per_query, (u64)ix->p_exact_budget_mb << 20);
    ForestView store = ix->view();
    store.members = ix->ex_iota.p;
    BucketMajor bm;
    bm.rows = ix->rows.p;
    bm.tomb = ix->tomb.p;
    bm.rinv = metric == ZB_METRIC_COSINE ? ix->ex_rinv.p : nullptr;
    bm.n2 = filt ? ix->ex_n2.p : nullptr;
    alignas(64) unsigned char tmap[128];
    if (ix->n_slots) make_row_tile_map(tmap, ix->rows.p, ix->n_slots, ix->dimp, 64, tile_scan_box_floats(3));
    bm.tmap3 = tmap;
    bm.positions = ix->n_slots;
    for (u64 c0 = 0; c0 < nq; c0 += p.chunk) {
        const u64 c = std::min<u64>(p.chunk, nq - c0);
        const float* q = d_q + c0 * (u64)ix->dimp;
        if (!sharded) {
            exact_scan3(ix->ex_ws, store, bm, ix->n_slots, metric, q, (u32)c, p.range_rows, (u32)top_k, filt, d_out_ord + c0 * top_k,
                        d_out_bits + c0 * top_k, d_out_counts + c0, s);
            continue;
        }
        const u64 nsk = c * top_k;
        ix->ex_loc.ensure(2 * p.chunk * top_k);
        ix->ex_gath.ensure(2 * p.chunk * top_k * G);
        ix->ex_counts.ensure(p.chunk);
        exact_scan3(ix->ex_ws, store, bm, ix->n_slots, metric, q, (u32)c, p.range_rows, (u32)top_k, filt, ix->ex_loc.p,
                    ix->ex_loc.p + nsk, ix->ex_counts.p, s);
        ix->nccl.allgather(ix->ex_loc.p, ix->ex_gath.p, 2 * nsk * 8, s);
        launch_merge_gathered((u32)c, (u32)c, (u32)top_k, G, ix->ex_gath.p, d_out_ord + c0 * top_k, d_out_bits + c0 * top_k,
                              d_out_counts + c0, s);
    }
    ix->sync();
}

static const float* stage_queries_device(zb_index* ix, const float* d_q, u64 nq) {
    if (ix->dim == ix->dimp && ((uintptr_t)d_q & 15) == 0) return d_q;
    ix->q_stage.ensure(nq * (u64)ix->dimp);
    launch_pad_rows(d_q, nq, ix->dim, ix->dimp, ix->q_stage.p, ix->stream);
    return ix->q_stage.p;
}

static void build_export_table(zb_index* ix, std::vector<int>* order_nodes, std::vector<int>* leaf_export) {
    leaf_export->assign(ix->h_leaf_off.size(), -1);
    int next_leaf = 0;
    std::vector<int> stack;
    for (int t = 0; t < ix->T && ix->built; ++t) {
        stack.push_back(ix->h_roots[t]);
        while (!stack.empty()) {
            int n = stack.back();
            stack.pop_back();
            if (order_nodes) order_nodes->push_back(n);
            int4 nd = ix->h_nodes[n];
            if (nd.x < 0) (*leaf_export)[nd.w] = next_leaf++;
            else {
                stack.push_back(nd.z);
                stack.push_back(nd.y);
            }
        }
    }
}

}

extern "C" {

const char* zb_last_error(void) { return zb::t_last_error.c_str(); }
int zb_abi_version(void) { return ZB_ABI_VERSION; }

int zb_device_count(int* out_count) {
    ZB_API_BEGIN
    ZB_REQUIRE(out_count, ZB_ERR_INVALID, "out_count is NULL");
    int n = 0;
    cudaError_t e = cudaGetDeviceCount(&n);
    if (e != cudaSuccess) {
        cudaGetLastError();
        n = 0;
    }
    *out_count = n;
    ZB_API_END
}

int zb_index_create(const zb_options* o, zb_index** out) {
    ZB_API_BEGIN
    ZB_REQUIRE(o && out, ZB_ERR_INVALID, "NULL argument");
    ZB_REQUIRE(o->dim >= 1 && o->dim <= 65536, ZB_ERR_INVALID, "dim %u out of range", o->dim);
    ZB_REQUIRE(o->metric < ZB_METRIC_COUNT, ZB_ERR_INVALID, "metric %u is not a zb_metric", o->metric);
    ZB_REQUIRE((o->metric != ZB_METRIC_MINKOWSKI && o->metric != ZB_METRIC_PNORM) ||
                   (o->metric_power >= 0 && o->metric_power <= ZB_METRIC_MAX_POWER),
               ZB_ERR_INVALID, "metric_power %d out of range 0..%d", o->metric_power, ZB_METRIC_MAX_POWER);
    ZB_REQUIRE(o->num_trees >= 1 && o->num_trees <= 4096, ZB_ERR_INVALID, "num_trees %u out of range", o->num_trees);
    int ndev = 0;
    cudaError_t e = cudaGetDeviceCount(&ndev);
    if (e != cudaSuccess || ndev == 0) {
        cudaGetLastError();
        throw zb::Error(ZB_ERR_NO_DEVICE, "no CUDA device: libzebra_b200 has no CPU fallback");
    }
    ZB_REQUIRE(o->device >= 0 && o->device < ndev, ZB_ERR_INVALID, "device %d out of range (%d devices)", o->device, ndev);
    cudaDeviceProp prop;
    ZB_CUDA(cudaGetDeviceProperties(&prop, o->device));
    ZB_REQUIRE(prop.major == 10, ZB_ERR_NO_DEVICE, "device %d is sm_%d%d; this library is built for sm_100a only",
               o->device, prop.major, prop.minor);
    zb_index* ix = new zb_index();
// ... 834 lines not shown
    ix->d_members.ensure(std::max<u64>(1, ix->members_used));
    if (ix->members_used)
        ZB_CUDA(cudaMemcpyAsync(ix->d_members.p, ix->h_members.data(), ix->members_used * 4, cudaMemcpyHostToDevice, ix->stream));
    if (ix->n_slots)
        ZB_CUDA(cudaMemcpy2DAsync(ix->slot_leaf.p, ix->slot_stride * 4, slot_leaf_h.data(), ix->n_slots * 4, ix->n_slots * 4, T,
                                  cudaMemcpyHostToDevice, ix->stream));
    ix->sync();
    ix->built = true;
    ix->upload_structure();
    ix->recount_live();
    ix->sync();
    ZB_API_END
}

static void pad_to_device(int device, const float* h, u64 n, u32 dim, int dimp, DBuf<float>& d);

int zb_index_load_flat(zb_index* ix, uint64_t n, const float* rows, const uint8_t* ids16, uint32_t bits, const float* coef,
                       const float* cst) {
    ZB_API_BEGIN
    ZB_REQUIRE(ix && (rows || !n) && coef && cst, ZB_ERR_INVALID, "NULL argument");
    ZB_REQUIRE(bits >= 1 && bits <= 16, ZB_ERR_INVALID, "bits %u out of range 1..16", bits);
    ZB_REQUIRE(n < (1ull << 32), ZB_ERR_INVALID, "too many rows for one load");
    int T, dim, dimp;
    {
        std::lock_guard<std::mutex> lk(ix->mu);
        ix->use_device();
        T = ix->T; dim = ix->dim; dimp = ix->dimp;
    }
    const int K = (int)bits, H = T * K, Hp = (H + 15) / 16 * 16;
    std::vector<u64> keys((size_t)n * T + 1);
    {
        DBuf<float> d_rows, d_coef, d_cst;
        DBuf<u8> d_sign;
        DBuf<u64> d_keys;
        pad_to_device(ix->device, rows, n, (u32)dim, dimp, d_rows);
        pad_to_device(ix->device, coef, (u64)H, (u32)dim, dimp, d_coef);
        d_cst.ensure((size_t)H);
        ZB_CUDA(cudaMemcpy(d_cst.p, cst, (size_t)H * 4, cudaMemcpyHostToDevice));
        d_sign.ensure(std::max<u64>(1, n * (u64)Hp));
        d_keys.ensure((size_t)n * T + 1);
        launch_project_flat(d_rows.p, n, d_coef.p, d_cst.p, H, dimp, d_sign.p, Hp, 0);
        launch_pack_flat_keys(d_sign.p, n, Hp, T, K, d_keys.p, nullptr, nullptr, 0);
        ZB_CUDA(cudaGetLastError());
        if (n) ZB_CUDA(cudaMemcpy(keys.data(), d_keys.p, (size_t)n * T * 8, cudaMemcpyDeviceToHost));
    }
    const int64_t per_tree = ((int64_t)2 << K) - 1, leaves_per_tree = (int64_t)1 << K;
    int64_t sizes4[4] = {per_tree * T, (int64_t)H, leaves_per_tree * T, (int64_t)n * T};
    std::vector<int32_t> nodes((size_t)sizes4[0] * 4), roots((size_t)T);
    for (int t = 0; t < T; ++t) {
        int32_t idx = (int32_t)(per_tree * t);
        roots[t] = idx;
        struct Fr { int depth; u32 prefix; int32_t parent; int side; };
        std::vector<Fr> stack{{0, 0u, -1, 0}};
        while (!stack.empty()) {
            const Fr fr = stack.back();
            stack.pop_back();
            const int32_t me = idx++;
            if (fr.parent >= 0) nodes[4 * (size_t)fr.parent + 1 + fr.side] = me;
            int32_t* nd = nodes.data() + 4 * (size_t)me;
            if (fr.depth == K) {
                nd[0] = -1; nd[1] = -1; nd[2] = -1; nd[3] = (int32_t)(leaves_per_tree * t + fr.prefix);
            } else {
                nd[0] = t * K + fr.depth; nd[1] = -1; nd[2] = -1; nd[3] = -1;
                stack.push_back({fr.depth + 1, (fr.prefix << 1) | 1u, me, 1});
                stack.push_back({fr.depth + 1, fr.prefix << 1, me, 0});
            }
        }
    }
    std::vector<int64_t> leaf_off((size_t)sizes4[2] + 1, 0);
    for (u64 o = 0; o < n; ++o)
        for (int t = 0; t < T; ++t) leaf_off[(size_t)(leaves_per_tree * t + (int64_t)keys[o * T + t]) + 1]++;
    for (size_t l = 0; l < (size_t)sizes4[2]; ++l) leaf_off[l + 1] += leaf_off[l];
    std::vector<int64_t> cursor(leaf_off.begin(), leaf_off.end() - 1);
    std::vector<uint64_t> members((size_t)n * T + 1);
    for (u64 o = 0; o < n; ++o)
        for (int t = 0; t < T; ++t) members[(size_t)cursor[(size_t)(leaves_per_tree * t + (int64_t)keys[o * T + t])]++] = o;
    int rc = zb_index_load_forest(ix, n, rows, ids16, sizes4, nodes.data(), roots.data(), coef, cst, leaf_off.data(), members.data());
    if (rc != ZB_OK) return rc;
    {
        std::lock_guard<std::mutex> lk(ix->mu);
        ix->flat_bits = bits;
        ix->flat_nodes = ix->h_nodes.size();
    }
    ZB_API_END
}

int zb_index_options(zb_index* ix, zb_options* out) {
    ZB_API_BEGIN
    ZB_REQUIRE(ix && out, ZB_ERR_INVALID, "NULL argument");
    std::lock_guard<std::mutex> lk(ix->mu);
    *out = ix->opt;
    ZB_API_END
}

int zb_index_export_rows(zb_index* ix, uint64_t first_ordinal, uint64_t n, float* out_rows, uint8_t* out_ids16,
                         uint8_t* out_live) {
    ZB_API_BEGIN
    ZB_REQUIRE(ix, ZB_ERR_INVALID, "NULL argument");
    std::lock_guard<std::mutex> lk(ix->mu);
    ix->use_device();
    ZB_REQUIRE(ix->G <= 1, ZB_ERR_STATE, "zb_index_export_rows needs an unsharded index (a shard holds 1/G of the rows)");
    ZB_REQUIRE(first_ordinal <= ix->total_rows && n <= ix->total_rows - first_ordinal, ZB_ERR_INVALID,
               "rows [%llu, +%llu) out of range (%llu rows)", (unsigned long long)first_ordinal, (unsigned long long)n,
               (unsigned long long)ix->total_rows);
    if (out_rows && n) {
        ZB_CUDA(cudaMemcpy2DAsync(out_rows, (size_t)ix->dim * 4, ix->rows.p + first_ordinal * (u64)ix->dimp, (size_t)ix->dimp * 4,
                                  (size_t)ix->dim * 4, n, cudaMemcpyDeviceToHost, ix->stream));
        ix->sync();
    }
    for (u64 i = 0; i < n; ++i) {
        if (out_ids16) ix->id_of(first_ordinal + i, out_ids16 + 16 * i);
        if (out_live) out_live[i] = ix->h_tomb[first_ordinal + i] ? 0 : 1;
    }
    ZB_API_END
}

int zb_index_stats(zb_index* ix, zb_stats* out) {
    ZB_API_BEGIN
    ZB_REQUIRE(ix && out, ZB_ERR_INVALID, "NULL argument");
    std::lock_guard<std::mutex> lk(ix->mu);
    ix->st.rows = ix->n_slots;
    ix->st.live_rows = ix->n_live;
    ix->st.total_rows = ix->total_rows;
    ix->st.nodes = ix->h_nodes.size();
    ix->st.planes = ix->n_planes;
    ix->st.leaves = ix->h_leaf_off.size();
    ix->st.device_bytes = zb::g_device_bytes;
    *out = ix->st;
    ZB_API_END
}

int zb_index_stream(zb_index* ix, void** out_stream) {
    ZB_API_BEGIN
    ZB_REQUIRE(ix && out_stream, ZB_ERR_INVALID, "NULL argument");
    *out_stream = (void*)ix->stream;
    ZB_API_END
}

int zb_index_set_param(zb_index* ix, const char* key, int64_t value) {
    ZB_API_BEGIN
    ZB_REQUIRE(ix && key, ZB_ERR_INVALID, "NULL argument");
    std::lock_guard<std::mutex> lk(ix->mu);
    std::string k(key);
    if (k == "tile_min_rows") ix->p_tile_min_rows = value;
    else if (k == "tile_queries") ix->p_tile_queries = value;
    else if (k == "use_tile_scan") ix->p_use_tile_scan = value;
    else if (k == "scan_gen") ix->p_scan_gen = value;
    else if (k == "classify_variant") ix->p_classify_variant = value;
    else if (k == "seq_prefetch") ix->p_seq_prefetch = value;
    else if (k == "select_variant") ix->p_select_variant = value;
    else if (k == "quad_tile") ix->p_quad_tile = value;
    else if (k == "flat_project") ix->p_flat_project = value;
    else if (k == "l2_filter") { ix->p_l2_filter = value; ix->filter_backoff = 0; }
    else if (k == "long_list_warps") { ZB_REQUIRE(value == 4 || value == 8, ZB_ERR_INVALID, "long_list_warps is 4 or 8"); ix->scan_ws.long_list_warps = (int)value; }
    else if (k == "exact_budget_mb") {
        ZB_REQUIRE(value >= 1 && value <= (1 << 20), ZB_ERR_INVALID, "exact_budget_mb out of range");
        ix->p_exact_budget_mb = value;
    }
    else if (k == "plan_tail") ix->p_plan_tail = value;
    else if (k == "p2p_queries") ix->p_p2p_queries = value;
    else if (k == "single_exchange") ix->p_single_exchange = value;
    else if (k == "bm_stage_mb") ix->p_bm_stage_mb = value > 0 ? value : 1;
    else if (k == "seq_tile") ix->p_seq_tile = value;
    else if (k == "hash_variant") ix->p_hash_variant = value;
    else if (k == "visit_slots") {
        ZB_REQUIRE(value >= 2 && value <= 65536, ZB_ERR_INVALID, "visit_slots out of range");
        ix->vpw = (u32)value;
    }
    else throw zb::Error(ZB_ERR_INVALID, "unknown parameter " + k);
    ZB_API_END
}

int zb_comm_unique_id(uint8_t* out_id128) {
    ZB_API_BEGIN
    ZB_REQUIRE(out_id128, ZB_ERR_INVALID, "NULL argument");
    Nccl::unique_id(out_id128);
    ZB_API_END
}

int zb_index_comm_init(zb_index* ix, const uint8_t* id128) {
    ZB_API_BEGIN
    ZB_REQUIRE(ix && id128, ZB_ERR_INVALID, "NULL argument");
    std::lock_guard<std::mutex> lk(ix->mu);
    ZB_REQUIRE(ix->G > 1, ZB_ERR_STATE, "index is not sharded");
    ZB_REQUIRE(!ix->comm_ready, ZB_ERR_STATE, "communicator already initialised");
    ix->nccl.init(id128, (int)ix->rank, (int)ix->G, ix->device);
    ix->comm_ready = true;
    ix->b_minh.ensure(1);
    ZB_CUDA(cudaMemcpyAsync(ix->b_minh.p, &ix->epoch_ms, 8, cudaMemcpyHostToDevice, ix->stream));
    ix->nccl.allreduce(ix->b_minh.p, 1, Nccl::U64, Nccl::MIN, ix->stream);
    ZB_CUDA(cudaMemcpyAsync(&ix->epoch_ms, ix->b_minh.p, 8, cudaMemcpyDeviceToHost, ix->stream));
    ix->sync();
    ZB_API_END
}

static void pad_to_device(int device, const float* h, u64 n, u32 dim, int dimp, DBuf<float>& d) {
    d.ensure(std::max<u64>(1, n * (u64)dimp));
    if (!n) return;
    ZB_CUDA(cudaMemset(d.p, 0, n * (u64)dimp * 4));
    ZB_CUDA(cudaMemcpy2D(d.p, (size_t)dimp * 4, h, (size_t)dim * 4, (size_t)dim * 4, n, cudaMemcpyHostToDevice));
}

int zb_metric_distance_batch(int device, uint32_t metric, int32_t power, uint64_t n, uint32_t dim, const float* a, const float* b,
                             uint64_t* out_bits) {
    ZB_API_BEGIN
    ZB_REQUIRE(metric < ZB_METRIC_COUNT && dim >= 1 && ((a && b && out_bits) || !n), ZB_ERR_INVALID, "bad argument");
    ZB_REQUIRE((metric != ZB_METRIC_MINKOWSKI && metric != ZB_METRIC_PNORM) || (power >= 0 && power <= ZB_METRIC_MAX_POWER),
               ZB_ERR_INVALID, "power %d out of range 0..%d", power, ZB_METRIC_MAX_POWER);
    int ndev = 0;
    if (cudaGetDeviceCount(&ndev) != cudaSuccess || !ndev) {
        cudaGetLastError();
        throw zb::Error(ZB_ERR_NO_DEVICE, "no CUDA device: libzebra_b200 has no CPU fallback");
    }
    ZB_CUDA(cudaSetDevice(device));
    const int dimp = ((int)dim + 15) / 16 * 16;
    DBuf<float> da, db;
    DBuf<u64> dout;
    pad_to_device(device, a, n, dim, dimp, da);
    pad_to_device(device, b, n, dim, dimp, db);
    dout.ensure(std::max<u64>(1, n));
    launch_pair_metric((int)metric, (int)power, da.p, db.p, n, (int)dim, dimp, dout.p, 0);
    ZB_CUDA(cudaMemcpy(out_bits, dout.p, n * 8, cudaMemcpyDeviceToHost));
    ZB_API_END
}

int zb_point_is_above_batch(int device, uint64_t n, uint32_t dim, const float* coef, const float* cst, const float* x,
                            uint8_t* out) {
    ZB_API_BEGIN
    ZB_REQUIRE(dim >= 1 && ((coef && cst && x && out) || !n), ZB_ERR_INVALID, "bad argument");
    int ndev = 0;
    if (cudaGetDeviceCount(&ndev) != cudaSuccess || !ndev) {
        cudaGetLastError();
        throw zb::Error(ZB_ERR_NO_DEVICE, "no CUDA device: libzebra_b200 has no CPU fallback");
    }
    ZB_CUDA(cudaSetDevice(device));
    const int dimp = ((int)dim + 15) / 16 * 16;
    DBuf<float> dc, dx, dk;
    DBuf<u8> dout;
    pad_to_device(device, coef, n, dim, dimp, dc);
    pad_to_device(device, x, n, dim, dimp, dx);
    dk.ensure(std::max<u64>(1, n));
    dout.ensure(std::max<u64>(1, n));
    if (n) ZB_CUDA(cudaMemcpy(dk.p, cst, n * 4, cudaMemcpyHostToDevice));
    launch_pair_above(dc.p, dk.p, dx.p, n, dimp, dout.p, 0);
    if (n) ZB_CUDA(cudaMemcpy(out, dout.p, n, cudaMemcpyDeviceToHost));
    ZB_API_END
}

int zb_synth_fill_device(int device, float* d_out, uint64_t first_row, uint64_t row_stride, uint64_t n, uint32_t dim,
                         uint64_t seed, uint32_t kind) {
    ZB_API_BEGIN
    ZB_REQUIRE(d_out || !n, ZB_ERR_INVALID, "NULL argument");
    ZB_CUDA(cudaSetDevice(device));
    launch_synth(d_out, first_row, row_stride, n, dim, seed, kind, 0);
    ZB_CUDA(cudaStreamSynchronize(0));
    ZB_API_END
}

}
```

zebra_b200/csrc/zb_scan.cu:

```cuda
#include <cub/device/device_radix_sort.cuh>
#include <cub/device/device_scan.cuh>
#include <cuda.h>

#include "zb_scan.cuh"

namespace zb {

#define TS_TEAMS 2
#define TS_TWARPS 4
#define TS_QT 8
#define TS_RB 128
#define TS_KC 3
#define TS_SLICE_FLOATS (TS_KC * 16)
#define TS_STAGE_BYTES (TS_RB * TS_SLICE_FLOATS * 4)
#define TS_CWARPS (TS_TEAMS * TS_TWARPS)
#define TS_THREADS 384
#define TS_MAX_STAGES 8
#define TS_KL 32
#define TS_NOPOS 0xFFFFFFFFu
#define TS_PACE_WINDOW 8
#define TS_PACE_EVERY 4

#ifdef ZB_SCAN_TIMING
#define TS_T(var) const long long var = clock64()
// ... 367 lines not shown
    cx.s_stage = s_stage; cx.s_q = s_q; cx.s_list = s_list;
    cx.bar_full = bar_full; cx.bar_empty = bar_empty;
    cx.S = S; cx.dimp = dimp; cx.chunks = chunks; cx.nsl = nsl;
    const int tw = warp % TS_TWARPS, sub = lane & 3;
    u32 rbuf = 0, rph = 0;
#ifdef ZB_SCAN_TIMING
    long long tacc[8] = {0, 0, 0, 0, 0, 0, 0, 0};
#define TS_TACC , tacc
#else
#define TS_TACC
#endif
    for (u32 it = 0;; ++it) {
        TS_T(t_tile0);
        mbar_wait(bar_ifull + 8 * (it & 1), (it >> 1) & 1);
        const TileInfo inf = s_info[it & 1];
        if (inf.tile == 0xFFFFFFFFu) break;
        const u32 nqt = inf.nqt;
        const bool narrow = nqt <= 4;
        const int g = narrow ? 0 : tw >> 1, wr = narrow ? tw : tw & 1;
        const int nq_mine = min(4, (int)nqt - g * 4);
        u32 my_visit = 0, my_np = 0, my_q = 0;
        double my_qrinv = 0.0;
        if (sub < nq_mine) {
            my_visit = tp.order[inf.first + g * 4 + sub];
            my_np = tp.v_np[my_visit];
            my_q = tp.v_q[my_visit];
            if (METRIC == 0) my_qrinv = tp.q_rinv[my_q];
        }
        mbar_wait(bar_qfull, it & 1);
        TS_T(t_tile1);
        TS_ACC(0, t_tile0, t_tile1);
        if (narrow) scan_tile<METRIC, 4>(cx, f, tp, inf, g, wr, tw, lane, rbuf, rph, my_np, my_q, my_qrinv, nq_mine TS_TACC);
        else scan_tile<METRIC, 8>(cx, f, tp, inf, g, wr, tw, lane, rbuf, rph, my_np, my_q, my_qrinv, nq_mine TS_TACC);
        TS_T(t_m0);
        if (lane == 0) mbar_arrive(bar_qempty);
        asm volatile("bar.sync %0, 128;" ::"r"(team + 1) : "memory");
        if (wr == 0) {
            const int nslab = narrow ? 4 : 2;
            const ListEntry* mine_l = s_list + (size_t)tw * 4 * TS_KL;
#pragma unroll 1
            for (int j = 0; j < nq_mine; ++j) {
                const int np = (int)__shfl_sync(0xffffffffu, my_np, j);
                const u32 v = __shfl_sync(0xffffffffu, my_visit, j);
                ListEntry a = mine_l[j * TS_KL + lane];
                u64 k = a.key;
                u32 p = a.pos;
#pragma unroll 1
                for (int o = 1; o < nslab; ++o) {
                    const ListEntry bb = mine_l[(size_t)o * 4 * TS_KL + j * TS_KL + (31 - lane)];
                    if (kp_less(bb.key, bb.pos, k, p)) { k = bb.key; p = bb.pos; }
#pragma unroll
                    for (int x = 16; x >= 1; x >>= 1) {
                        const u64 ok = shfl_xor64(k, x);
                        const u32 op = __shfl_xor_sync(0xffffffffu, p, x);
                        const bool lower = (lane & x) == 0;
                        const bool other_less = kp_less(ok, op, k, p);
                        if (lower == other_less) { k = ok; p = op; }
                    }
                }
                const u32 e0 = tp.v_ent_off[v], e1 = tp.v_ent_off[v + 1];
                if ((u32)lane < e1 - e0) {
                    Entry e{ZB_SENTINEL, ZB_SENTINEL};
                    if (lane < np && p != TS_NOPOS) e = Entry{k, f.ord[f.members[p]]};
                    tp.entries[e0 + lane] = e;
                }
            }
        }
        asm volatile("bar.sync %0, 128;" ::"r"(team + 1) : "memory");
        TS_T(t_m1);
        TS_ACC(5, t_m0, t_m1);
    }
#ifdef ZB_SCAN_TIMING
    if (lane == 0)
        for (int i = 0; i < 8; ++i) atomicAdd(&tp.stats[8 + i], (u64)tacc[i]);
#endif
}

typedef CUtensorMap T3Map;
__device__ __forceinline__ bool t3_isinf_pos(double x) { return isinf(x) && x > 0.0; }
__device__ __forceinline__ double t3_dmul(double a, double b) { return __dmul_rn(a, b); }
__device__ __forceinline__ double t3_dsub(double a, double b) { return __dsub_rn(a, b); }
__device__ __forceinline__ u64 t3_dbits(double x) { return (u64)__double_as_longlong(x); }
__device__ __forceinline__ float t3_fadd(float a, float b) { return __fadd_rn(a, b); }
__host__ __device__ __forceinline__ u32 t3_fbits(float x) {
#ifdef __CUDA_ARCH__
    return __float_as_uint(x);
#else
    u32 b; memcpy(&b, &x, 4); return b;
#endif
}
__host__ __device__ __forceinline__ float t3_bitsf(u32 b) {
#ifdef __CUDA_ARCH__
    return __uint_as_float(b);
#else
    float x; memcpy(&x, &b, 4); return x;
#endif
}
__device__ __forceinline__ float t3_fadd_ru(float a, float b) { return __fadd_ru(a, b); }
__device__ __forceinline__ float t3_fmul_ru(float a, float b) { return __fmul_ru(a, b); }
__device__ __forceinline__ float t3_fmaf(float a, float b, float c) { return __fmaf_rn(a, b, c); }
__device__ __forceinline__ float t3_fsub(float a, float b) { return __fsub_rn(a, b); }
typedef float4 T3F4;
__device__ __forceinline__ T3F4 t3_ld_f4(const float* p) { return __ldg(reinterpret_cast<const float4*>(p)); }
__device__ __forceinline__ u64 t3_pk2(float lo, float hi) { return pk2(lo, hi); }
__device__ __forceinline__ void t3_upk2(u64 v, float& lo, float& hi) { upk2(v, lo, hi); }
#ifndef T3_ASM_ORDER
#define T3_ASM_ORDER
#endif
__device__ __forceinline__ u64 t3_fma2(u64 a, u64 b, u64 c) {
    u64 d;
    asm T3_ASM_ORDER("fma.rn.f32x2 %0, %1, %2, %3;" : "=l"(d) : "l"(a), "l"(b), "l"(c));
    return d;
}
__device__ __forceinline__ u64 t3_sub2(u64 a, u64 b) {
    u64 d;
    asm T3_ASM_ORDER("sub.rn.f32x2 %0, %1, %2;" : "=l"(d) : "l"(a), "l"(b));
    return d;
}
__device__ __forceinline__ u64 t3_ldcg_u64(const u64* p) { return __ldcg(p); }
__device__ __forceinline__ void t3_atomic_min_u64(u64* p, u64 v) { atomicMin(p, v); }
__device__ __forceinline__ u64 t3_shfl64(u64 v, int src) { return shfl64(v, src); }
__device__ __forceinline__ double t3_shfl_f64(double v, int src) { return __longlong_as_double((long long)shfl64((u64)__double_as_longlong(v), src)); }
__device__ __forceinline__ u64 t3_shfl_up64(u64 v) { return shfl_up64(v); }
__device__ __forceinline__ void t3_team_sync(int team, int threads) { asm volatile("bar.sync %0, %1;" ::"r"(team + 1), "r"(threads) : "memory"); }
__device__ __forceinline__ void t3_fence_barrier_init() {
    asm volatile("fence.mbarrier_init.release.cluster;" ::: "memory");
    asm volatile("fence.proxy.async.shared::cta;" ::: "memory");
}
#ifndef T3_REGS_MATH
#define T3_REGS_MATH 232
#define T3_REGS_AUX 40
#endif
#define T3_STR2(x) #x
#define T3_STR(x) T3_STR2(x)
static_assert(256 * T3_REGS_MATH + 128 * T3_REGS_AUX <= 384 * 168, "setmaxnreg split exceeds the CTA's registers");
template <int TW>
__device__ __forceinline__ void t3_setmaxnreg_dec() {
    if (TW == 4) asm volatile("setmaxnreg.dec.sync.aligned.u32 " T3_STR(T3_REGS_AUX) ";");
    else asm volatile("setmaxnreg.dec.sync.aligned.u32 32;");
}
template <int TW>
__device__ __forceinline__ void t3_setmaxnreg_inc() {
    if (TW == 4) asm volatile("setmaxnreg.inc.sync.aligned.u32 " T3_STR(T3_REGS_MATH) ";");
    else asm volatile("setmaxnreg.inc.sync.aligned.u32 112;");
}
__device__ __forceinline__ void t3_prefetch_map(const T3Map& m) { asm volatile("prefetch.tensormap [%0];" ::"l"(&m) : "memory"); }
__device__ __forceinline__ void t3_tma_2d_g2s(u32 dst, const T3Map& map, int c0, long long row, u32 bar) {
    tma_2d_g2s(dst, &map, c0, (int)row, bar);
}
__device__ __forceinline__ void t3_prefetch_l1(const void* p) { asm volatile("prefetch.global.L1 [%0];" ::"l"(p)); }
__device__ __forceinline__ bool t3_above_from_dot(float dot, float constant) { return above_from_dot(dot, constant); }
}
#include "zb_scan3_kernel.cuh"
namespace zb {

template <int METRIC, int KR, int TW>
__global__ void __launch_bounds__(T3Shape<TW>::THREADS, 1) tile_scan3_kernel(const __grid_constant__ CUtensorMap tmap, ForestView f, T3Params tp) {
    extern __shared__ __align__(1024) unsigned char smem3[];
    t3_body<METRIC, 0, KR, TW>(tmap, f, tp, smem3);
}
#define RF_THREADS 256
template <int METRIC>
__global__ void __launch_bounds__(RF_THREADS) refine_visits_kernel(ForestView f, T3RefineParams rp) {
    t3_refine_warp<METRIC>(f, rp, (int)(threadIdx.x & 31u));
}
__global__ void __launch_bounds__(T3Shape<4>::THREADS, 1) project3_kernel(const __grid_constant__ CUtensorMap tmap, ForestView f, T3Params tp) {
    extern __shared__ __align__(1024) unsigned char smem3[];
    t3_body<0, 1, 1, 4>(tmap, f, tp, smem3);
}

__global__ void ts_count_kernel(ForestView f, u32 nv, const u32* __restrict__ v_leaf, const u32* __restrict__ v_np,
                                u32 min_rows, u32 kmax, u32* __restrict__ leaf_count) {
    u32 v = blockIdx.x * blockDim.x + threadIdx.x;
    if (v >= nv) return;
    u32 leaf = v_leaf[v];
    if (f.leaf_len[leaf] >= min_rows && v_np[v] <= kmax) atomicAdd(&leaf_count[leaf], 1u);
}
__global__ void ts_tilecount_kernel(u32 nleaves, const u32* __restrict__ leaf_count, u32 tq, u32* __restrict__ tile_cnt) {
    u32 l = blockIdx.x * blockDim.x + threadIdx.x;
    if (l <= nleaves) tile_cnt[l] = l < nleaves ? (leaf_count[l] + tq - 1) / tq : 0u;
}
__global__ void ts_scatter_kernel(ForestView f, u32 nv, const u32* __restrict__ v_leaf, const u32* __restrict__ v_np,
                                  u32 min_rows, u32 kmax, const u32* __restrict__ leaf_start, u32* __restrict__ leaf_cursor,
                                  u32* __restrict__ order, u64* __restrict__ v_pair_len, u8* __restrict__ v_done) {
    u32 v = blockIdx.x * blockDim.x + threadIdx.x;
    if (v >= nv) return;
    u32 leaf = v_leaf[v];
    if (f.leaf_len[leaf] >= min_rows && v_np[v] <= kmax) {
        u32 pos = leaf_start[leaf] + atomicAdd(&leaf_cursor[leaf], 1u);
        order[pos] = v;
        v_pair_len[v] = 0;
        v_done[v] = 1;
    }
}
__global__ void ts_filltiles_kernel(u32 nleaves, const u32* __restrict__ leaf_count, const u32* __restrict__ leaf_start,
                                    const u32* __restrict__ tile_start, u32 tq, u32* __restrict__ tile_leaf,
                                    u32* __restrict__ tile_first, u32* __restrict__ tile_count, const u32* __restrict__ leaf_len,
                                    u64 row_bytes, u64* __restrict__ unique_bytes) {
    u32 l = blockIdx.x * blockDim.x + threadIdx.x;
    if (l >= nleaves) return;
    const u32 c = leaf_count[l], ts = tile_start[l];
    if (!c) return;
    atomicAdd(unique_bytes, (u64)leaf_len[l] * row_bytes);
    const u32 nt = (c + tq - 1) / tq;
    for (u32 j = 0, done = 0; j < nt; ++j) {
        const u32 n = c - done < tq ? c - done : tq;
        tile_leaf[ts + j] = l;
        tile_first[ts + j] = leaf_start[l] + done;
        tile_count[ts + j] = n;
        done += n;
    }
}

__global__ void ts_leafkey_kernel(u32 nleaves, const u32* __restrict__ leaf_count, const u32* __restrict__ leaf_len,
                                  u32* __restrict__ key, u32* __restrict__ val) {
    const u32 l = blockIdx.x * blockDim.x + threadIdx.x;
    if (l >= nleaves) return;
    const u64 cost = (u64)leaf_count[l] * leaf_len[l];
    key[l] = leaf_count[l] ? ~(u32)(cost > 0xFFFFFFFEull ? 0xFFFFFFFEull : cost) : 0xFFFFFFFFu;
    val[l] = l;
}
__global__ void ts_tilecount_sorted_kernel(u32 nleaves, const u32* __restrict__ sorted_leaf, const u32* __restrict__ leaf_count, u32 tq,
                                           u32* __restrict__ tile_cnt) {
    const u32 i = blockIdx.x * blockDim.x + threadIdx.x;
    if (i <= nleaves) tile_cnt[i] = i < nleaves ? (leaf_count[sorted_leaf[i]] + tq - 1) / tq : 0u;
}
__global__ void ts_filltiles_sorted_kernel(u32 nleaves, const u32* __restrict__ sorted_leaf, const u32* __restrict__ leaf_count,
                                           const u32* __restrict__ leaf_start, const u32* __restrict__ tile_start, u32 tq,
                                           u32* __restrict__ tile_leaf, u32* __restrict__ tile_first, u32* __restrict__ tile_count,
                                           const u32* __restrict__ leaf_len, u64 row_bytes, u64* __restrict__ unique_bytes) {
    const u32 i = blockIdx.x * blockDim.x + threadIdx.x;
    if (i >= nleaves) return;
    const u32 l = sorted_leaf[i];
    const u32 c = leaf_count[l], ts = tile_start[i];
    if (!c) return;
    atomicAdd(unique_bytes, (u64)leaf_len[l] * row_bytes);
    const u32 nt = (c + tq - 1) / tq;
    const u32 per = c / nt, extra = c - per * nt;
    for (u32 j = 0, done = 0; j < nt; ++j) {
        const u32 n = per + (j < extra ? 1u : 0u);
        tile_leaf[ts + j] = l;
        tile_first[ts + j] = leaf_start[l] + done;
        tile_count[ts + j] = n;
        done += n;
    }
}

__global__ void __launch_bounds__(128) rinv_kernel(const float* __restrict__ x_, u64 n, int dimp, double* __restrict__ out) {
    const u64 i = (u64)blockIdx.x * 32ull + (threadIdx.x >> 2);
    if (i >= n) return;
    const int sub = threadIdx.x & 3;
    const float4* x = reinterpret_cast<const float4*>(x_ + i * dimp);
    float4 acc = make_float4(0.f, 0.f, 0.f, 0.f);
    for (int c = 0; c < dimp / 16; ++c) {
        float4 v = x[c * 4 + sub];
        fma4(acc, v, v);
    }
    float sum = quad_reduce16(acc, quad_mask());
    if (sub == 0) out[i] = __ddiv_rn(1.0, __dsqrt_rn((double)sum));
}
void launch_rinv(const float* d_x, u64 n, int dimp, double* d_out, cudaStream_t s) {
    if (!n) return;
    rinv_kernel<<<(u32)((n + 31) / 32), 128, 0, s>>>(d_x, n, dimp, d_out);
}

__global__ void __launch_bounds__(128) n2_kernel(const float* __restrict__ x_, u64 n, int dimp, float* __restrict__ out) {
    const u64 i = (u64)blockIdx.x * 32ull + (threadIdx.x >> 2);
    if (i >= n) return;
    const int sub = threadIdx.x & 3;
    const float4* x = reinterpret_cast<const float4*>(x_ + i * dimp);
    float4 acc = make_float4(0.f, 0.f, 0.f, 0.f);
    for (int c = 0; c < dimp / 16; ++c) {
        float4 v = x[c * 4 + sub];
        fma4(acc, v, v);
    }
    float sum = quad_reduce16(acc, quad_mask());
    if (sub == 0) out[i] = sum;
}
void launch_n2(const float* d_x, u64 n, int dimp, float* d_out, cudaStream_t s) {
    if (!n) return;
    n2_kernel<<<(u32)((n + 31) / 32), 128, 0, s>>>(d_x, n, dimp, d_out);
}
__global__ void __launch_bounds__(256) leaf_n2max_kernel(u32 nleaves, const long long* __restrict__ leaf_off, const u32* __restrict__ leaf_len,
                                                         const float* __restrict__ n2, float* __restrict__ out) {
    const u32 l = blockIdx.x * 8u + (threadIdx.x >> 5);
    if (l >= nleaves) return;
    const u32 lane = threadIdx.x & 31u, len = leaf_len[l];
    const float* x = n2 + leaf_off[l];
    float m = 0.f;
    for (u32 i = lane; i < len; i += 32u) {
        const float v = x[i];
        if (v <= T3_N2_LIMIT && v > m) m = v;
    }
    for (int o = 16; o >= 1; o >>= 1) m = fmaxf(m, __shfl_xor_sync(0xffffffffu, m, o));
    if (lane == 0) out[l] = m;
}
void launch_leaf_n2max(u32 nleaves, const long long* d_leaf_off, const u32* d_leaf_len, const float* d_n2, float* d_out, cudaStream_t s) {
    if (!nleaves) return;
    leaf_n2max_kernel<<<(nleaves + 7) / 8, 256, 0, s>>>(nleaves, d_leaf_off, d_leaf_len, d_n2, d_out);
}

static size_t ts_smem_bytes(int nst, int dimp) { return TS_TEAMS * ts_team_bytes(nst, dimp) + 1024; }

typedef CUresult (*EncodeTiledFn)(CUtensorMap*, CUtensorMapDataType, cuuint32_t, void*, const cuuint64_t*, const cuuint64_t*,
                                  const cuuint32_t*, const cuuint32_t*, CUtensorMapInterleave, CUtensorMapSwizzle,
                                  CUtensorMapL2promotion, CUtensorMapFloatOOBfill);
static EncodeTiledFn encode_tiled_fn() {
    static EncodeTiledFn fn = nullptr;
    if (!fn) {
        void* p = nullptr;
        cudaDriverEntryPointQueryResult qres;
        ZB_CUDA(cudaGetDriverEntryPoint("cuTensorMapEncodeTiled", &p, cudaEnableDefault, &qres));
        ZB_REQUIRE(p && qres == cudaDriverEntryPointSuccess, ZB_ERR_CUDA, "cuTensorMapEncodeTiled is not available");
        fn = (EncodeTiledFn)p;
    }
    return fn;
}
void make_row_tile_map(void* out_map128, const float* bm_rows, u64 positions, int dimp, int box_rows, int box_floats) {
    CUtensorMap* m = reinterpret_cast<CUtensorMap*>(out_map128);
    cuuint64_t gdim[2] = {(cuuint64_t)dimp, (cuuint64_t)(positions ? positions : 1)};
    cuuint64_t gstride[1] = {(cuuint64_t)dimp * 4};
    cuuint32_t box[2] = {(cuuint32_t)box_floats, (cuuint32_t)box_rows};
    cuuint32_t estr[2] = {1, 1};
    CUresult r = encode_tiled_fn()(m, CU_TENSOR_MAP_DATA_TYPE_FLOAT32, 2, (void*)bm_rows, gdim, gstride, box, estr,
                                   CU_TENSOR_MAP_INTERLEAVE_NONE, CU_TENSOR_MAP_SWIZZLE_NONE, CU_TENSOR_MAP_L2_PROMOTION_L2_256B,
                                   CU_TENSOR_MAP_FLOAT_OOB_FILL_NONE);
    ZB_REQUIRE(r == CUDA_SUCCESS, ZB_ERR_CUDA, "cuTensorMapEncodeTiled failed (%d)", (int)r);
}

int tile_scan_box_floats(int generation) { return generation == 2 ? TS_SLICE_FLOATS : T3_SLICE_FLOATS; }

bool tile_scan_supported(int dimp, u32 top_k) {
    int dev = 0, max_smem = 0;
    cudaGetDevice(&dev);
    cudaDeviceGetAttribute(&max_smem, cudaDevAttrMaxSharedMemoryPerBlockOptin, dev);
    return top_k >= 1 && top_k <= TS_KL && ts_smem_bytes(2, dimp) <= (size_t)max_smem;
}

void tile_scan(ScanWorkspace& ws, const ForestView& f, const BucketMajor& bm, u32 metric, const float* d_q, const double* d_q_rinv,
               u32 nq, u32 nv, const u32* v_leaf, const u32* v_np, const u32* v_q, const u32* v_ent_off, u64* v_pair_len,
               u8* v_done, Entry* entries, u32 top_k, u32 min_rows, u32 tile_queries, u32 nleaves, cudaStream_t s) {
    ws.launched = false;
    ws.filtered = false;
    const u32 pace_window = tile_queries >> 9;
    const bool lpt_order = false;
    tile_queries &= 0xFF;
    if (!nv || !nleaves || !tile_scan_supported(f.dimp, top_k)) return;
    const u32 tq = tile_queries >= 1 && tile_queries <= TS_QT ? tile_queries : TS_QT;
    int dev = 0, max_smem = 0, sms = 0;
    cudaGetDevice(&dev);
    cudaDeviceGetAttribute(&max_smem, cudaDevAttrMaxSharedMemoryPerBlockOptin, dev);
    cudaDeviceGetAttribute(&sms, cudaDevAttrMultiProcessorCount, dev);
    int nst = 0;
    for (int cand = TS_MAX_STAGES; cand >= 2; --cand)
        if (ts_smem_bytes(cand, f.dimp) <= (size_t)max_smem) { nst = cand; break; }
    if (!nst) return;
    const size_t smem = ts_smem_bytes(nst, f.dimp);

    ws.leaf_count.ensure(nleaves + 1);
    ws.leaf_start.ensure(nleaves + 1);
    ws.leaf_cursor.ensure(nleaves + 1);
    ws.order.ensure(nv);
    ws.tile_leaf.ensure(nv);
    ws.tile_first.ensure(nv);
    ws.counters.ensure(64);
    ws.tile_prog.ensure(nv);
    ZB_CUDA(cudaMemsetAsync(ws.tile_prog.p, 0, (size_t)nv * 4, s));
    ws.gthr.ensure(nq ? nq : 1);
    ZB_CUDA(cudaMemsetAsync(ws.gthr.p, 0xFF, (size_t)(nq ? nq : 1) * 8, s));
    size_t tmp_bytes = 0;
    cub::DeviceScan::ExclusiveSum(nullptr, tmp_bytes, (const u32*)nullptr, (u32*)nullptr, (long long)(nleaves + 1));
    ws.tmp.ensure(tmp_bytes + 256);

    ZB_CUDA(cudaMemsetAsync(ws.leaf_count.p, 0, (size_t)(nleaves + 1) * 4, s));
    ZB_CUDA(cudaMemsetAsync(ws.leaf_cursor.p, 0, (size_t)(nleaves + 1) * 4, s));
    ZB_CUDA(cudaMemsetAsync(ws.counters.p, 0, 64 * 4, s));
    const u32 kmax = top_k;
    ts_count_kernel<<<(nv + 255) / 256, 256, 0, s>>>(f, nv, v_leaf, v_np, min_rows, kmax, ws.leaf_count.p);
    cub::DeviceScan::ExclusiveSum(ws.tmp.p, tmp_bytes, ws.leaf_count.p, ws.leaf_start.p, (long long)(nleaves + 1), s);
    ts_scatter_kernel<<<(nv + 255) / 256, 256, 0, s>>>(f, nv, v_leaf, v_np, min_rows, kmax, ws.leaf_start.p,
                                                       ws.leaf_cursor.p, ws.order.p, v_pair_len, v_done);
    ws.tile_per_leaf.ensure(nleaves + 1);
    ws.tile_start.ensure(nleaves + 1);
    ws.tile_cnt.ensure(nv);
    if (lpt_order) {
        for (int b = 0; b < 2; ++b) {
            ws.sort_key[b].ensure(nleaves);
            ws.sort_val[b].ensure(nleaves);
        }
        size_t sort_bytes = 0;
        cub::DeviceRadixSort::SortPairs(nullptr, sort_bytes, (const u32*)nullptr, (u32*)nullptr, (const u32*)nullptr, (u32*)nullptr,
                                        (long long)nleaves, 0, 32, s);
        ws.sort_tmp.ensure(sort_bytes + 256);
        ts_leafkey_kernel<<<(nleaves + 255) / 256, 256, 0, s>>>(nleaves, ws.leaf_count.p, f.leaf_len, ws.sort_key[0].p, ws.sort_val[0].p);
        cub::DeviceRadixSort::SortPairs(ws.sort_tmp.p, sort_bytes, ws.sort_key[0].p, ws.sort_key[1].p, ws.sort_val[0].p, ws.sort_val[1].p,
                                        (long long)nleaves, 0, 32, s);
        ts_tilecount_sorted_kernel<<<(nleaves + 256) / 256, 256, 0, s>>>(nleaves, ws.sort_val[1].p, ws.leaf_count.p, tq, ws.tile_per_leaf.p);
        cub::DeviceScan::ExclusiveSum(ws.tmp.p, tmp_bytes, ws.tile_per_leaf.p, ws.tile_start.p, (long long)(nleaves + 1), s);
        ts_filltiles_sorted_kernel<<<(nleaves + 255) / 256, 256, 0, s>>>(nleaves, ws.sort_val[1].p, ws.leaf_count.p, ws.leaf_start.p,
                                                                         ws.tile_start.p, tq, ws.tile_leaf.p, ws.tile_first.p, ws.tile_cnt.p,
                                                                         f.leaf_len, (u64)f.dimp * 4ull,
                                                                         reinterpret_cast<u64*>(ws.counters.p + 4) + 3);
    } else {
        ts_tilecount_kernel<<<(nleaves + 256) / 256, 256, 0, s>>>(nleaves, ws.leaf_count.p, tq, ws.tile_per_leaf.p);
        cub::DeviceScan::ExclusiveSum(ws.tmp.p, tmp_bytes, ws.tile_per_leaf.p, ws.tile_start.p, (long long)(nleaves + 1), s);
        ts_filltiles_kernel<<<(nleaves + 255) / 256, 256, 0, s>>>(nleaves, ws.leaf_count.p, ws.leaf_start.p, ws.tile_start.p, tq,
                                                                  ws.tile_leaf.p, ws.tile_first.p, ws.tile_cnt.p, f.leaf_len,
                                                                  (u64)f.dimp * 4ull, reinterpret_cast<u64*>(ws.counters.p + 4) + 3);
    }

    TileParams tp;
    tp.tile_leaf = ws.tile_leaf.p;
    tp.tile_first = ws.tile_first.p;
    tp.tile_count = ws.tile_cnt.p;
    tp.ntiles = ws.tile_start.p + nleaves;
    ws.ntiles_ptr = tp.ntiles;
    tp.tile_counter = ws.counters.p;
    tp.order = ws.order.p;
    tp.v_np = v_np;
    tp.v_q = v_q;
    tp.v_ent_off = v_ent_off;
    tp.entries = entries;
    tp.queries = d_q;
    tp.q_rinv = d_q_rinv;
    tp.bm_rinv = bm.rinv;
    tp.bm_tomb = bm.tomb;
    tp.stats = reinterpret_cast<u64*>(ws.counters.p + 4);
    tp.pace_window = pace_window;
    tp.tile_prog = ws.tile_prog.p;
    tp.gthr = ws.gthr.p;
    tp.top_k = top_k;
    tp.nst = nst;
    const CUtensorMap& tmap = *reinterpret_cast<const CUtensorMap*>(bm.tmap);
    const int grid = sms;
    if (!ws.ev0) {
        ZB_CUDA(cudaEventCreate(&ws.ev0));
        ZB_CUDA(cudaEventCreate(&ws.ev1));
    }
    ZB_CUDA(cudaEventRecord(ws.ev0, s));
    if (metric == 0) {
        ZB_CUDA(cudaFuncSetAttribute(tile_scan_kernel<0>, cudaFuncAttributeMaxDynamicSharedMemorySize, (int)smem));
        tile_scan_kernel<0><<<grid, TS_THREADS, smem, s>>>(tmap, f, tp);
    } else if (metric == 1) {
        ZB_CUDA(cudaFuncSetAttribute(tile_scan_kernel<1>, cudaFuncAttributeMaxDynamicSharedMemorySize, (int)smem));
        tile_scan_kernel<1><<<grid, TS_THREADS, smem, s>>>(tmap, f, tp);
    } else {
        ZB_CUDA(cudaFuncSetAttribute(tile_scan_kernel<2>, cudaFuncAttributeMaxDynamicSharedMemorySize, (int)smem));
        tile_scan_kernel<2><<<grid, TS_THREADS, smem, s>>>(tmap, f, tp);
    }
    ZB_CUDA(cudaGetLastError());
    ZB_CUDA(cudaEventRecord(ws.ev1, s));
    ws.launched = true;
    ws.launches = 7;
}

void tile_scan_stats(ScanWorkspace& ws, cudaStream_t s, u64* tile_visits, u64* tile_pairs, u64* moved_bytes, float* kernel_ms,
                     u32* tiles, u64* unique_bytes, u64* flagged_visits, u64* refined_rows, float* refine_ms) {
    *tile_visits = *tile_pairs = *moved_bytes = *unique_bytes = 0;
    *kernel_ms = 0.f;
    *tiles = 0;
    if (flagged_visits) *flagged_visits = 0;
    if (refined_rows) *refined_rows = 0;
    if (refine_ms) *refine_ms = 0.f;
    if (!ws.launched) return;
    u64 h[6] = {0, 0, 0, 0, 0, 0};
    ZB_CUDA(cudaMemcpyAsync(h, reinterpret_cast<u64*>(ws.counters.p + 4), 48, cudaMemcpyDeviceToHost, s));
    ZB_CUDA(cudaMemcpyAsync(tiles, ws.ntiles_ptr, 4, cudaMemcpyDeviceToHost, s));
    ZB_CUDA(cudaStreamSynchronize(s));
    cudaEventElapsedTime(kernel_ms, ws.ev0, ws.ev1);
    *tile_visits = h[0];
    *tile_pairs = h[1];
    *moved_bytes = h[2];
    *unique_bytes = h[3];
    if (ws.filtered) {
        if (flagged_visits) *flagged_visits = h[4];
        if (refined_rows) *refined_rows = h[5];
        if (refine_ms) cudaEventElapsedTime(refine_ms, ws.ev1, ws.ev2);
    }
#ifdef ZB_SCAN_TIMING
    u64 t[8];
    ZB_CUDA(cudaMemcpy(t, reinterpret_cast<u64*>(ws.counters.p + 4) + 8, 64, cudaMemcpyDeviceToHost));
    fprintf(stderr, "[scan timing, Mcycles summed over math warps] tile-wait %.1f stage-wait %.1f math %.1f fold %.1f insert %.1f merge %.1f idle %.1f\n",
            t[0] / 1e6, t[1] / 1e6, t[2] / 1e6, t[3] / 1e6, t[4] / 1e6, t[5] / 1e6, t[7] / 1e6);
#endif
}

static size_t t3_smem_bytes(int nst, int dimp, int qcap, int kr) { return T3_TEAMS * (size_t)t3_layout(nst, dimp, qcap, kr).total + 1024; }
static int t3_kr(u32 top_k) { return top_k <= T3_KL ? 1 : T3_KR_MAX; }
static bool t3_config(int dimp, int kr, int* nst_out, int* qcap_out) {
    int dev = 0, max_smem = 0;
    cudaGetDevice(&dev);
    cudaDeviceGetAttribute(&max_smem, cudaDevAttrMaxSharedMemoryPerBlockOptin, dev);
    for (int qcap = T3_QT; qcap >= 4; qcap >>= 1)
        for (int nst = T3_MAX_STAGES; nst >= 3; --nst)
            if (t3_smem_bytes(nst, dimp, qcap, kr) <= (size_t)max_smem) {
                *nst_out = nst;
                *qcap_out = qcap;
                return true;
            }
    return false;
}
bool tile_scan3_supported(int dimp, u32 top_k) {
    int nst, qcap;
    return top_k >= 1 && top_k <= T3_KL * T3_KR_MAX && t3_config(dimp, t3_kr(top_k), &nst, &qcap);
}
static void t3_launch(ScanWorkspace& ws, const ForestView& f, const BucketMajor& bm, u32 metric, const float* d_q, const double* d_q_rinv,
                      u32 nq, u32 nv, const u32* v_leaf, const u32* v_np, const u32* v_q, const u32* v_ent_off, Entry* entries, u32 top_k,
                      int kr, int nst, int qcap, int sms, const u32* ntiles, const u32* nvisits, cudaStream_t s);

void tile_scan3(ScanWorkspace& ws, const ForestView& f, const BucketMajor& bm, u32 metric, const float* d_q, const double* d_q_rinv,
                u32 nq, u32 nv, const u32* v_leaf, const u32* v_np, const u32* v_q, const u32* v_ent_off, u64* v_pair_len,
                u8* v_done, Entry* entries, u32 top_k, u32 min_rows, u32 tile_queries, u32 nleaves, cudaStream_t s) {
    ws.launched = false;
    ws.filtered = false;
    int nst = 0, qcap = 0;
    const int kr = t3_kr(top_k);
    if (!nv || !nleaves || top_k < 1 || top_k > T3_KL * T3_KR_MAX || !t3_config(f.dimp, kr, &nst, &qcap)) return;
    const bool lpt_order = ((tile_queries >> 8) & 1u) == 0;
    tile_queries &= 0xFF;
    const u32 tq = tile_queries >= 1 && tile_queries <= (u32)qcap ? tile_queries : (u32)qcap;
    int dev = 0, sms = 0;
    cudaGetDevice(&dev);
    cudaDeviceGetAttribute(&sms, cudaDevAttrMultiProcessorCount, dev);

    ws.leaf_count.ensure(nleaves + 1);
    ws.leaf_start.ensure(nleaves + 1);
    ws.leaf_cursor.ensure(nleaves + 1);
    ws.order.ensure(nv);
    ws.tile_leaf.ensure(nv);
    ws.tile_first.ensure(nv);
    ws.counters.ensure(64);
    ws.gthr.ensure(nq ? nq : 1);
    ZB_CUDA(cudaMemsetAsync(ws.gthr.p, 0xFF, (size_t)(nq ? nq : 1) * 8, s));
    size_t tmp_bytes = 0;
    cub::DeviceScan::ExclusiveSum(nullptr, tmp_bytes, (const u32*)nullptr, (u32*)nullptr, (long long)(nleaves + 1));
    ws.tmp.ensure(tmp_bytes + 256);
    ZB_CUDA(cudaMemsetAsync(ws.leaf_count.p, 0, (size_t)(nleaves + 1) * 4, s));
    ZB_CUDA(cudaMemsetAsync(ws.leaf_cursor.p, 0, (size_t)(nleaves + 1) * 4, s));
    ZB_CUDA(cudaMemsetAsync(ws.counters.p, 0, 64 * 4, s));
    const u32 kmax = top_k;
    ts_count_kernel<<<(nv + 255) / 256, 256, 0, s>>>(f, nv, v_leaf, v_np, min_rows, kmax, ws.leaf_count.p);
    cub::DeviceScan::ExclusiveSum(ws.tmp.p, tmp_bytes, ws.leaf_count.p, ws.leaf_start.p, (long long)(nleaves + 1), s);
    ts_scatter_kernel<<<(nv + 255) / 256, 256, 0, s>>>(f, nv, v_leaf, v_np, min_rows, kmax, ws.leaf_start.p,
                                                       ws.leaf_cursor.p, ws.order.p, v_pair_len, v_done);
    ws.tile_per_leaf.ensure(nleaves + 1);
    ws.tile_start.ensure(nleaves + 1);
    ws.tile_cnt.ensure(nv);
    if (lpt_order) {
        for (int b = 0; b < 2; ++b) {
            ws.sort_key[b].ensure(nleaves);
            ws.sort_val[b].ensure(nleaves);
        }
        size_t sort_bytes = 0;
        cub::DeviceRadixSort::SortPairs(nullptr, sort_bytes, (const u32*)nullptr, (u32*)nullptr, (const u32*)nullptr, (u32*)nullptr,
                                        (long long)nleaves, 0, 32, s);
        ws.sort_tmp.ensure(sort_bytes + 256);
        ts_leafkey_kernel<<<(nleaves + 255) / 256, 256, 0, s>>>(nleaves, ws.leaf_count.p, f.leaf_len, ws.sort_key[0].p, ws.sort_val[0].p);
        cub::DeviceRadixSort::SortPairs(ws.sort_tmp.p, sort_bytes, ws.sort_key[0].p, ws.sort_key[1].p, ws.sort_val[0].p, ws.sort_val[1].p,
                                        (long long)nleaves, 0, 32, s);
        ts_tilecount_sorted_kernel<<<(nleaves + 256) / 256, 256, 0, s>>>(nleaves, ws.sort_val[1].p, ws.leaf_count.p, tq, ws.tile_per_leaf.p);
        cub::DeviceScan::ExclusiveSum(ws.tmp.p, tmp_bytes, ws.tile_per_leaf.p, ws.tile_start.p, (long long)(nleaves + 1), s);
        ts_filltiles_sorted_kernel<<<(nleaves + 255) / 256, 256, 0, s>>>(nleaves, ws.sort_val[1].p, ws.leaf_count.p, ws.leaf_start.p,
                                                                         ws.tile_start.p, tq, ws.tile_leaf.p, ws.tile_first.p, ws.tile_cnt.p,
                                                                         f.leaf_len, (u64)f.dimp * 4ull,
                                                                         reinterpret_cast<u64*>(ws.counters.p + 4) + 3);
    } else {
        ts_tilecount_kernel<<<(nleaves + 256) / 256, 256, 0, s>>>(nleaves, ws.leaf_count.p, tq, ws.tile_per_leaf.p);
        cub::DeviceScan::ExclusiveSum(ws.tmp.p, tmp_bytes, ws.tile_per_leaf.p, ws.tile_start.p, (long long)(nleaves + 1), s);
        ts_filltiles_kernel<<<(nleaves + 255) / 256, 256, 0, s>>>(nleaves, ws.leaf_count.p, ws.leaf_start.p, ws.tile_start.p, tq,
                                                                  ws.tile_leaf.p, ws.tile_first.p, ws.tile_cnt.p, f.leaf_len,
                                                                  (u64)f.dimp * 4ull, reinterpret_cast<u64*>(ws.counters.p + 4) + 3);
    }
    t3_launch(ws, f, bm, metric, d_q, d_q_rinv, nq, nv, v_leaf, v_np, v_q, v_ent_off, entries, top_k, kr, nst, qcap, sms,
              ws.tile_start.p + nleaves, ws.leaf_start.p + nleaves, s);
}

static void t3_launch(ScanWorkspace& ws, const ForestView& f, const BucketMajor& bm, u32 metric, const float* d_q, const double* d_q_rinv,
                      u32 nq, u32 nv, const u32* v_leaf, const u32* v_np, const u32* v_q, const u32* v_ent_off, Entry* entries, u32 top_k,
                      int kr, int nst, int qcap, int sms, const u32* ntiles, const u32* nvisits, cudaStream_t s) {
    const size_t smem = t3_smem_bytes(nst, f.dimp, qcap, kr);
    const bool filt = ws.l2_filter && (metric == 1 || metric == 2) && kr == 1 && top_k <= ZB_L2_FILTER_MAX_K && bm.n2 && bm.leaf_n2max;
    ws.filtered = filt;
    T3Params tp{};
    if (filt) {
        ws.q_n2.ensure(nq ? nq : 1);
        launch_n2(d_q, nq, f.dimp, ws.q_n2.p, s);
        ws.cand.ensure((size_t)nv * T3_KL);
        ws.cand_cut.ensure(nv);
        ws.cand_flag.ensure(nv);
        tp.bm_n2 = bm.n2;
        tp.q_n2 = ws.q_n2.p;
        tp.leaf_n2max = bm.leaf_n2max;
        tp.ecoef = (float)(4 * f.chunks + 32) * 5.9604645e-8f * 1.01f;
        tp.cand = ws.cand.p;
        tp.cand_cut = ws.cand_cut.p;
        tp.cand_flag = ws.cand_flag.p;
    }
    tp.tile_leaf = ws.tile_leaf.p;
    tp.tile_first = ws.tile_first.p;
    tp.tile_count = ws.tile_cnt.p;
    tp.ntiles = ntiles;
    ws.ntiles_ptr = tp.ntiles;
    tp.tile_counter = ws.counters.p;
    tp.order = ws.order.p;
    tp.v_np = v_np;
    tp.v_q = v_q;
    tp.v_ent_off = v_ent_off;
    tp.entries = entries;
    tp.queries = d_q;
    tp.q_rinv = d_q_rinv;
    tp.bm_rinv = bm.rinv;
    tp.bm_tomb = bm.tomb;
    tp.stats = reinterpret_cast<u64*>(ws.counters.p + 4);
    tp.gthr = ws.gthr.p;
    tp.top_k = top_k;
    tp.nst = nst;
    tp.qcap = qcap;
    tp.kr = kr;
    const CUtensorMap& tmap = *reinterpret_cast<const CUtensorMap*>(bm.tmap3);
    const int grid = sms;
    if (!ws.ev0) {
        ZB_CUDA(cudaEventCreate(&ws.ev0));
        ZB_CUDA(cudaEventCreate(&ws.ev1));
    }
    ZB_CUDA(cudaEventRecord(ws.ev0, s));
    auto launch = [&](auto kern, int threads) {
        ZB_CUDA(cudaFuncSetAttribute(kern, cudaFuncAttributeMaxDynamicSharedMemorySize, (int)smem));
        kern<<<grid, threads, smem, s>>>(tmap, f, tp);
    };
    if (filt) launch(tile_scan3_kernel<3, 1, 4>, T3Shape<4>::THREADS);
    else if (kr == 1) {
        if (metric == 0) launch(tile_scan3_kernel<0, 1, 4>, T3Shape<4>::THREADS);
        else if (metric == 1) launch(tile_scan3_kernel<1, 1, 4>, T3Shape<4>::THREADS);
        else launch(tile_scan3_kernel<2, 1, 4>, T3Shape<4>::THREADS);
    } else if (ws.long_list_warps == 4) {
        if (metric == 0) launch(tile_scan3_kernel<0, T3_KR_MAX, 4>, T3Shape<4>::THREADS);
        else if (metric == 1) launch(tile_scan3_kernel<1, T3_KR_MAX, 4>, T3Shape<4>::THREADS);
        else launch(tile_scan3_kernel<2, T3_KR_MAX, 4>, T3Shape<4>::THREADS);
    } else {
        if (metric == 0) launch(tile_scan3_kernel<0, T3_KR_MAX, 8>, T3Shape<8>::THREADS);
        else if (metric == 1) launch(tile_scan3_kernel<1, T3_KR_MAX, 8>, T3Shape<8>::THREADS);
        else launch(tile_scan3_kernel<2, T3_KR_MAX, 8>, T3Shape<8>::THREADS);
    }
    ZB_CUDA(cudaGetLastError());
    ZB_CUDA(cudaEventRecord(ws.ev1, s));
    ws.launched = true;
    ws.launches = 7;
    if (filt) {
        T3RefineParams rp{};
        rp.bm_rows = bm.rows;
        rp.bm_tomb = bm.tomb;
        rp.queries = d_q;
        rp.order = ws.order.p;
        rp.nvisits = nvisits;
        rp.v_leaf = v_leaf;
        rp.v_np = v_np;
        rp.v_q = v_q;
        rp.v_ent_off = v_ent_off;
        rp.cand = ws.cand.p;
        rp.cand_cut = ws.cand_cut.p;
        rp.cand_flag = ws.cand_flag.p;
        rp.gthr = ws.gthr.p;
        rp.q_n2 = ws.q_n2.p;
        rp.leaf_n2max = bm.leaf_n2max;
        rp.ecoef = tp.ecoef;
        rp.entries = entries;
        rp.work_counter = ws.counters.p + 1;
        rp.stats = tp.stats;
        const int rgrid = sms * 6;
        if (metric == 1) refine_visits_kernel<1><<<rgrid, RF_THREADS, 0, s>>>(f, rp);
        else refine_visits_kernel<2><<<rgrid, RF_THREADS, 0, s>>>(f, rp);
        ZB_CUDA(cudaGetLastError());
        if (!ws.ev2) ZB_CUDA(cudaEventCreate(&ws.ev2));
        ZB_CUDA(cudaEventRecord(ws.ev2, s));
        ws.launches = 9;
    }
}

__global__ void pj_tiles_kernel(u32 nranges, u32 npt, u32 range_rows, u64 n, u32 H, u32 tq, long long* __restrict__ leaf_off,
                                u32* __restrict__ leaf_len, u32* __restrict__ tile_leaf, u32* __restrict__ tile_first,
                                u32* __restrict__ tile_count, u32* __restrict__ ntiles) {
    const u32 i = blockIdx.x * blockDim.x + threadIdx.x;
    if (i == 0) *ntiles = nranges * npt;
    if (i < nranges) {
        leaf_off[i] = (long long)i * range_rows;
        const u64 left = n - (u64)i * range_rows;
        leaf_len[i] = left < range_rows ? (u32)left : range_rows;
    }
    if (i < nranges * npt) {
        const u32 r = i / npt, p = i - r * npt;
        tile_leaf[i] = r;
        tile_first[i] = p * tq;
        tile_count[i] = H - p * tq < tq ? H - p * tq : tq;
    }
}
bool project3_supported(int dimp) {
    int nst, qcap;
    return t3_config(dimp, 1, &nst, &qcap);
}
void project3(ScanWorkspace& ws, const float* d_rows, u64 n, const float* d_coef, const float* d_cst, int H, int dimp, u8* d_sign, int Hp,
              cudaStream_t s) {
    int nst = 0, qcap = 0;
    if (!n || !H) return;
    ZB_REQUIRE(t3_config(dimp, 1, &nst, &qcap), ZB_ERR_STATE, "project3: rows of %d floats do not fit the tile kernel", dimp);
    ZB_REQUIRE(n < (1ull << 31), ZB_ERR_INVALID, "project3: too many rows in one call");
    int dev = 0, sms = 0;
    cudaGetDevice(&dev);
    cudaDeviceGetAttribute(&sms, cudaDevAttrMultiProcessorCount, dev);
    const u32 tq = (u32)qcap;
    const u32 npt = ((u32)H + tq - 1) / tq;
    u32 range_rows = 2048;
    while (range_rows > 64 && (n + range_rows - 1) / range_rows * npt < (u64)sms * T3_TEAMS * 8) range_rows >>= 1;
    const u32 nranges = (u32)((n + range_rows - 1) / range_rows);
    const u64 nt = (u64)nranges * npt;
    ZB_REQUIRE(nt < (1ull << 31), ZB_ERR_INVALID, "project3: too many tiles");
    ws.pj_off.ensure(nranges);
    ws.leaf_count.ensure(nranges);
    ws.tile_leaf.ensure(nt);
    ws.tile_first.ensure(nt);
    ws.tile_cnt.ensure(nt);
    ws.counters.ensure(64);
    ZB_CUDA(cudaMemsetAsync(ws.counters.p, 0, 64 * 4, s));
    pj_tiles_kernel<<<(u32)((nt + 255) / 256), 256, 0, s>>>(nranges, npt, range_rows, n, (u32)H, tq, ws.pj_off.p, ws.leaf_count.p,
                                                           ws.tile_leaf.p, ws.tile_first.p, ws.tile_cnt.p, ws.counters.p + 2);
    alignas(64) CUtensorMap tmap;
    make_row_tile_map(&tmap, d_rows, n, dimp, T3_RB, T3_SLICE_FLOATS);
    ForestView f{};
    f.leaf_off = ws.pj_off.p;
    f.leaf_len = ws.leaf_count.p;
    f.dimp = dimp;
    f.dim = dimp;
    f.chunks = dimp / 16;
    T3Params tp{};
    tp.tile_leaf = ws.tile_leaf.p;
    tp.tile_first = ws.tile_first.p;
    tp.tile_count = ws.tile_cnt.p;
    tp.ntiles = ws.counters.p + 2;
    tp.tile_counter = ws.counters.p;
    tp.queries = d_coef;
    tp.stats = reinterpret_cast<u64*>(ws.counters.p + 4);
    tp.nst = nst;
    tp.qcap = qcap;
    tp.kr = 1;
    tp.pj_cst = d_cst;
    tp.pj_sign = d_sign;
    tp.pj_hp = Hp;
    const size_t smem = t3_smem_bytes(nst, dimp, qcap, 1);
    ZB_CUDA(cudaFuncSetAttribute(project3_kernel, cudaFuncAttributeMaxDynamicSharedMemorySize, (int)smem));
    project3_kernel<<<sms, T3Shape<4>::THREADS, smem, s>>>(tmap, f, tp);
    ZB_CUDA(cudaGetLastError());
}

__global__ void ex_visits_kernel(u32 nranges, u32 nq, u32 ntq, u32 range_rows, u64 n, u32 top_k, long long* __restrict__ leaf_off,
                                 u32* __restrict__ leaf_len, u32* __restrict__ v_leaf, u32* __restrict__ v_np, u32* __restrict__ v_q,
                                 u32* __restrict__ order, u32* __restrict__ ent_off, u32* __restrict__ woff, u32* __restrict__ tile_leaf,
                                 u32* __restrict__ tile_first, u32* __restrict__ tile_count, u32* __restrict__ counters) {
    const u64 i = (u64)blockIdx.x * blockDim.x + threadIdx.x;
    const u64 nv = (u64)nranges * nq, nt = (u64)nranges * ntq;
    if (i == 0) {
        counters[2] = (u32)nt;
        counters[3] = (u32)nv;
    }
    if (i < nranges) {
        leaf_off[i] = (long long)i * range_rows;
        const u64 left = n - i * range_rows;
        leaf_len[i] = left < range_rows ? (u32)left : range_rows;
    }
    if (i < nv) {
        const u32 q = (u32)(i / nranges), r = (u32)(i - (u64)q * nranges);
        v_leaf[i] = r;
        v_np[i] = top_k;
        v_q[i] = q;
        order[(u64)r * nq + q] = (u32)i;
    }
    if (i <= nv) ent_off[i] = (u32)(i * top_k);
    if (i <= nq) woff[i] = (u32)(i * nranges);
    if (i < nt) {
        const u32 r = (u32)(i / ntq), j = (u32)(i - (u64)r * ntq);
        const u32 per = nq / ntq, extra = nq - per * ntq;
        tile_leaf[i] = r;
        tile_first[i] = r * nq + j * per + (j < extra ? j : extra);
        tile_count[i] = per + (j < extra ? 1u : 0u);
    }
}

static u64 ex_visit_bytes(u32 top_k, bool l2_filter) {
    return 5 * 4 + 3 * 4 + (u64)top_k * sizeof(Entry) + (l2_filter ? (u64)T3_KL * 8 + 4 + 1 : 0);
}

ExactPlan exact_plan(u64 n, u64 nq, int dimp, u32 top_k, bool l2_filter, u64 per_query_bytes, u64 budget_bytes) {
    ExactPlan p;
    int nst = 0, qcap = 0;
    ZB_REQUIRE(t3_config(dimp, t3_kr(top_k), &nst, &qcap), ZB_ERR_INVALID, "exact search: rows of %d floats do not fit the tile kernel", dimp);
    int dev = 0, sms = 0;
    cudaGetDevice(&dev);
    cudaDeviceGetAttribute(&sms, cudaDevAttrMultiProcessorCount, dev);
    const u64 vb = ex_visit_bytes(top_k, l2_filter);
    n = n ? n : 1;
    auto nranges = [&](u64 rr) { return (n + rr - 1) / rr; };
    auto chunk = [&](u64 rr) { return std::max<u64>(1, budget_bytes / (nranges(rr) * vb + per_query_bytes + 16)); };
    u64 rr = 4096;
    while (rr > 64 && nranges(rr) * ((std::min(nq, chunk(rr)) + qcap - 1) / qcap) < (u64)sms * T3_TEAMS * 8) rr >>= 1;
    while (nranges(rr) * vb + per_query_bytes > budget_bytes && rr < (1ull << 24)) rr <<= 1;
    p.range_rows = (u32)rr;
    p.chunk = std::min<u64>(chunk(rr), nq ? nq : 1);
    ZB_REQUIRE(nranges(rr) * p.chunk < (1ull << 31) && nranges(rr) * p.chunk * top_k < (1ull << 32), ZB_ERR_INVALID,
               "exact search: too many visits in one chunk");
    return p;
}

__global__ void ex_empty_kernel(u32 nq, u32 top_k, u64* __restrict__ out_ord, u64* __restrict__ out_bits, u32* __restrict__ out_counts) {
    const u64 i = (u64)blockIdx.x * blockDim.x + threadIdx.x;
    if (i < (u64)nq * top_k) out_ord[i] = out_bits[i] = ZB_SENTINEL;
    if (i < nq) out_counts[i] = 0;
}

void exact_scan3(ScanWorkspace& ws, const ForestView& store, const BucketMajor& bm, u64 n, u32 metric, const float* d_q, u32 nq,
                 u32 range_rows, u32 top_k, bool l2_filter, u64* out_ord, u64* out_bits, u32* out_counts, cudaStream_t s) {
    ws.launched = false;
    ws.filtered = false;
    if (!nq || !top_k) return;
    if (!n) {
        const u64 tot = std::max<u64>((u64)nq * top_k, nq);
        ex_empty_kernel<<<(u32)((tot + 255) / 256), 256, 0, s>>>(nq, top_k, out_ord, out_bits, out_counts);
        ZB_CUDA(cudaGetLastError());
        return;
    }
    int nst = 0, qcap = 0;
    const int kr = t3_kr(top_k);
    ZB_REQUIRE(metric <= 2 && top_k <= T3_KL * T3_KR_MAX && t3_config(store.dimp, kr, &nst, &qcap), ZB_ERR_INVALID,
               "exact search: no fused-kernel configuration for metric %u, top_k %u, %d floats", metric, top_k, store.dimp);
    ZB_REQUIRE(n < (1ull << 31) && range_rows % T3_RB == 0, ZB_ERR_INVALID, "exact search: %llu rows in ranges of %u",
               (unsigned long long)n, range_rows);
    int dev = 0, sms = 0;
    cudaGetDevice(&dev);
    cudaDeviceGetAttribute(&sms, cudaDevAttrMultiProcessorCount, dev);
    const u32 nranges = (u32)((n + range_rows - 1) / range_rows);
    const u32 ntq = (nq + (u32)qcap - 1) / (u32)qcap;
    const u64 nv = (u64)nranges * nq, nt = (u64)nranges * ntq;
    ZB_REQUIRE(nv < (1ull << 31) && nv * top_k < (1ull << 32), ZB_ERR_INVALID, "exact search: too many visits in one call");
    ws.pj_off.ensure(nranges);
    ws.leaf_count.ensure(nranges);
    ws.ex_leaf.ensure(nv);
    ws.ex_np.ensure(nv);
    ws.ex_q.ensure(nv);
    ws.order.ensure(nv);
    ws.ex_ent_off.ensure(nv + 1);
    ws.ex_woff.ensure((u64)nq + 1);
    ws.tile_leaf.ensure(nt);
    ws.tile_first.ensure(nt);
    ws.tile_cnt.ensure(nt);
    ws.ex_entries.ensure(nv * top_k);
    ws.counters.ensure(64);
    ws.gthr.ensure(nq);
    ZB_CUDA(cudaMemsetAsync(ws.counters.p, 0, 64 * 4, s));
    ZB_CUDA(cudaMemsetAsync(ws.gthr.p, 0xFF, (size_t)nq * 8, s));
    ex_visits_kernel<<<(u32)((nv + 1 + 255) / 256), 256, 0, s>>>(nranges, nq, ntq, range_rows, n, top_k, ws.pj_off.p, ws.leaf_count.p,
                                                                ws.ex_leaf.p, ws.ex_np.p, ws.ex_q.p, ws.order.p, ws.ex_ent_off.p,
                                                                ws.ex_woff.p, ws.tile_leaf.p, ws.tile_first.p, ws.tile_cnt.p,
                                                                ws.counters.p);
    ZB_CUDA(cudaGetLastError());
    ForestView f = store;
    f.leaf_off = ws.pj_off.p;
    f.leaf_len = ws.leaf_count.p;
    f.num_trees = 1;
    BucketMajor b = bm;
    const double* q_rinv = nullptr;
    if (metric == 0) {
        ws.ex_q_rinv.ensure(nq);
        launch_rinv(d_q, nq, f.dimp, ws.ex_q_rinv.p, s);
        q_rinv = ws.ex_q_rinv.p;
    }
    ws.l2_filter = l2_filter && (metric == 1 || metric == 2) && bm.n2;
    if (ws.l2_filter) {
        ws.ex_n2max.ensure(nranges);
        launch_leaf_n2max(nranges, ws.pj_off.p, ws.leaf_count.p, bm.n2, ws.ex_n2max.p, s);
        b.leaf_n2max = ws.ex_n2max.p;
    }
    t3_launch(ws, f, b, metric, d_q, q_rinv, nq, (u32)nv, ws.ex_leaf.p, ws.ex_np.p, ws.ex_q.p, ws.ex_ent_off.p, ws.ex_entries.p, top_k, kr,
              nst, qcap, sms, ws.counters.p + 2, ws.counters.p + 3, s);
    launch_merge_queries(nq, 1, ws.ex_woff.p, ws.ex_ent_off.p, ws.ex_entries.p, top_k, out_ord, out_bits, out_counts, s);
}

#define SQ_THREADS 256
#define SQ_TQ 8
#define SQ_CTAS_PER_SM 4

__global__ void sq_count_kernel(u32 nv, const u32* __restrict__ v_leaf, const u64* __restrict__ v_pair_off, u32* __restrict__ leaf_count) {
    u32 v = blockIdx.x * blockDim.x + threadIdx.x;
    if (v >= nv) return;
    if (v_pair_off[v + 1] > v_pair_off[v]) atomicAdd(&leaf_count[v_leaf[v]], 1u);
}
__global__ void sq_scatter_kernel(u32 nv, const u32* __restrict__ v_leaf, const u64* __restrict__ v_pair_off,
                                  const u32* __restrict__ leaf_start, u32* __restrict__ leaf_cursor, u32* __restrict__ order) {
    u32 v = blockIdx.x * blockDim.x + threadIdx.x;
    if (v >= nv) return;
    if (v_pair_off[v + 1] > v_pair_off[v]) {
        const u32 leaf = v_leaf[v];
        order[leaf_start[leaf] + atomicAdd(&leaf_cursor[leaf], 1u)] = v;
    }
}

struct SeqTileParams {
    const u32* tile_leaf;
    const u32* tile_first;
    const u32* tile_count;
    const u32* ntiles;
    u32* tile_counter;
    const u32* order;
    const u32* v_q;
    const u64* v_pair_off;
    u64* pair_key;
    const float* queries;
    u64* stats;
    int power;
    int pf_lines;
};

template <int CODE, int NQ>
__device__ __forceinline__ void seq_tile_rows(const ForestView& f, const SeqTileParams& tp, const float* __restrict__ s_q,
                                              const u64* __restrict__ s_pbase, u32 c, u32 leaf) {
    const u32 len = f.leaf_len[leaf];
    const long long off = f.leaf_off[leaf];
    const int n4 = f.dim >> 2, q4 = f.dimp >> 2;
    const int n8 = n4 >> 1;
    const int pf = tp.pf_lines * 8;
    const float4* q = reinterpret_cast<const float4*>(s_q);
    for (u32 r = threadIdx.x; r < len; r += SQ_THREADS) {
        const u32 slot = f.members[off + r];
        if (tomb_test(f.tomb, slot)) {
#pragma unroll
            for (int j = 0; j < NQ; ++j)
                if ((u32)j < c) tp.pair_key[s_pbase[j] + r] = ZB_SENTINEL;
            continue;
        }
        SeqAcc st[NQ];
#pragma unroll
        for (int j = 0; j < NQ; ++j) seq_init(st[j]);
        const float* row = f.rows + (size_t)slot * f.dimp;
        const float4* a = reinterpret_cast<const float4*>(row);
        float4 c0 = make_float4(0.f, 0.f, 0.f, 0.f), c1 = c0;
        if (n8 > 0) { c0 = __ldg(a); c1 = __ldg(a + 1); }
#pragma unroll 1
        for (int g = 0; g < n8; ++g) {
            float4 x0 = c0, x1 = c1;
            if (g + 1 < n8) { c0 = __ldg(a + 2 * g + 2); c1 = __ldg(a + 2 * g + 3); }
            if (pf != 0 && (g & 3) == 0 && 2 * g + pf < n4) asm volatile("prefetch.global.L2 [%0];" ::"l"(a + 2 * g + pf));
#pragma unroll
            for (int j = 0; j < NQ; ++j) {
                const float4 b0 = q[j * q4 + 2 * g], b1 = q[j * q4 + 2 * g + 1];
                seq_step<CODE>(st[j], x0.x, b0.x, tp.power);
                seq_step<CODE>(st[j], x0.y, b0.y, tp.power);
                seq_step<CODE>(st[j], x0.z, b0.z, tp.power);
                seq_step<CODE>(st[j], x0.w, b0.w, tp.power);
                seq_step<CODE>(st[j], x1.x, b1.x, tp.power);
                seq_step<CODE>(st[j], x1.y, b1.y, tp.power);
                seq_step<CODE>(st[j], x1.z, b1.z, tp.power);
                seq_step<CODE>(st[j], x1.w, b1.w, tp.power);
            }
        }
        for (int i = n8 * 2; i < n4; ++i) {
            const float4 av = __ldg(a + i);
#pragma unroll
            for (int j = 0; j < NQ; ++j) {
                const float4 bv = q[j * q4 + i];
                seq_step<CODE>(st[j], av.x, bv.x, tp.power);
                seq_step<CODE>(st[j], av.y, bv.y, tp.power);
                seq_step<CODE>(st[j], av.z, bv.z, tp.power);
                seq_step<CODE>(st[j], av.w, bv.w, tp.power);
            }
        }
        for (int i = n4 * 4; i < f.dim; ++i) {
            const float x = __ldg(row + i);
// ... 214 lines not shown
```

zebra_b200/csrc/zb_scan.cuh:

```cuda
#pragma once
#include "zb_host.h"
#include "zb_kernels.cuh"

namespace zb {

struct ScanWorkspace {
    DBuf<u32> leaf_count, leaf_start, leaf_cursor, tile_per_leaf, tile_start, order, tile_leaf, tile_first, tile_cnt;
    DBuf<u32> counters, tile_prog;
    DBuf<u64> gthr;
    DBuf<float> q_n2, cand_cut;
    DBuf<u64> cand;
    DBuf<u8> cand_flag;
    bool l2_filter = false;
    bool filtered = false;
    int long_list_warps = 8;
    cudaEvent_t ev2 = nullptr;
    DBuf<long long> pj_off;
    DBuf<u32> ex_leaf, ex_np, ex_q, ex_ent_off, ex_woff;
    DBuf<float> ex_n2max;
    DBuf<Entry> ex_entries;
    DBuf<double> ex_q_rinv;
    DBuf<u8> tmp, sort_tmp;
    DBuf<u32> sort_key[2], sort_val[2];
    bool launched = false;
    bool seq_launched = false;
    u32 launches = 0;
    cudaEvent_t ev0 = nullptr, ev1 = nullptr;
    const u32* ntiles_ptr = nullptr;
};

struct BucketMajor {
    const float* rows = nullptr;
    const double* rinv = nullptr;
    const u32* tomb = nullptr;
    const float* n2 = nullptr;
    const float* leaf_n2max = nullptr;
    const void* tmap = nullptr;
    const void* tmap3 = nullptr;
    u64 positions = 0;
};

void make_row_tile_map(void* out_map128, const float* bm_rows, u64 positions, int dimp, int box_rows, int box_floats);
int tile_scan_box_floats(int generation);
bool tile_scan_supported(int dimp, u32 top_k);
void launch_rinv(const float* d_x, u64 n, int dimp, double* d_out, cudaStream_t s);
void launch_n2(const float* d_x, u64 n, int dimp, float* d_out, cudaStream_t s);
void launch_leaf_n2max(u32 nleaves, const long long* d_leaf_off, const u32* d_leaf_len, const float* d_n2, float* d_out, cudaStream_t s);
#define ZB_L2_FILTER_MAX_K 16

void tile_scan(ScanWorkspace& ws, const ForestView& f, const BucketMajor& bm, u32 metric, const float* d_q, const double* d_q_rinv,
               u32 nq, u32 nv, const u32* v_leaf, const u32* v_np, const u32* v_q, const u32* v_ent_off, u64* v_pair_len,
               u8* v_done, Entry* entries, u32 top_k, u32 min_rows, u32 tile_queries, u32 nleaves, cudaStream_t s);
bool tile_scan3_supported(int dimp, u32 top_k);
void tile_scan3(ScanWorkspace& ws, const ForestView& f, const BucketMajor& bm, u32 metric, const float* d_q, const double* d_q_rinv,
                u32 nq, u32 nv, const u32* v_leaf, const u32* v_np, const u32* v_q, const u32* v_ent_off, u64* v_pair_len,
                u8* v_done, Entry* entries, u32 top_k, u32 min_rows, u32 tile_queries, u32 nleaves, cudaStream_t s);
bool project3_supported(int dimp);
void project3(ScanWorkspace& ws, const float* d_rows, u64 n, const float* d_coef, const float* d_cst, int H, int dimp, u8* d_sign, int Hp,
              cudaStream_t s);
#define ZB_EXACT_MAX_K 128
struct ExactPlan {
    u32 range_rows = 0;
    u64 chunk = 0;
};
ExactPlan exact_plan(u64 n, u64 nq, int dimp, u32 top_k, bool l2_filter, u64 per_query_bytes, u64 budget_bytes);
void exact_scan3(ScanWorkspace& ws, const ForestView& store, const BucketMajor& bm, u64 n, u32 metric, const float* d_q, u32 nq,
                 u32 range_rows, u32 top_k, bool l2_filter, u64* out_ord, u64* out_bits, u32* out_counts, cudaStream_t s);
void tile_scan_stats(ScanWorkspace& ws, cudaStream_t s, u64* tile_visits, u64* tile_pairs, u64* moved_bytes, float* kernel_ms,
                     u32* tiles, u64* unique_bytes, u64* flagged_visits = nullptr, u64* refined_rows = nullptr, float* refine_ms = nullptr);

bool seq_tile_scan_supported(int dimp);
void seq_tile_scan(ScanWorkspace& ws, const ForestView& f, u32 metric, int power, const float* d_q, u32 nv, const u32* v_leaf,
                   const u32* v_q, const u64* v_pair_off, u64* pair_key, u32 nleaves, int prefetch_lines, cudaStream_t s);
bool quad_tile_scan_supported(int dimp);
void quad_tile_scan(ScanWorkspace& ws, const ForestView& f, u32 metric, const float* d_q, u32 nv, const u32* v_leaf, const u32* v_q,
                    const u64* v_pair_off, u64* pair_key, u32 nleaves, cudaStream_t s);
void seq_tile_scan_stats(ScanWorkspace& ws, cudaStream_t s, u64* moved_bytes, float* kernel_ms, u32* tiles);

}
```

Measured before the change: 2.631 million.

## Add tcgen05 TF32 tensor-core L2 filter scan kernel with split-precision dot products

```diff
diff --git a/include/zebra_b200.h b/include/zebra_b200.h
--- a/include/zebra_b200.h
+++ b/include/zebra_b200.h
@@ -61,6 +61,7 @@
     uint32_t last_filter_rows;
     float last_ms_refine;
     uint32_t last_filter_used;
+    uint32_t last_filter_tc;
 } zb_stats;
 
 const char* zb_last_error(void);
diff --git a/zebra_b200/_ffi.py b/zebra_b200/_ffi.py
--- a/zebra_b200/_ffi.py
+++ b/zebra_b200/_ffi.py
@@ -63,6 +63,7 @@
         ("last_filter_rows", C.c_uint32),
         ("last_ms_refine", C.c_float),
         ("last_filter_used", C.c_uint32),
+        ("last_filter_tc", C.c_uint32),
     ]
 
     def as_dict(self):
diff --git a/zebra_b200/csrc/zb_index.cu b/zebra_b200/csrc/zb_index.cu
--- a/zebra_b200/csrc/zb_index.cu
+++ b/zebra_b200/csrc/zb_index.cu
@@ -112,6 +112,7 @@
     DBuf<u32> bm_tomb, slot_pos, d_leaf_tree;
     alignas(64) unsigned char bm_tmap[128];
     alignas(64) unsigned char bm_tmap3[128];
+    alignas(64) unsigned char bm_tmap_tc[128];
     bool bm_valid = false, bm_failed = false;
     u64 bm_positions = 0;
     DBuf<long long> d_bm_off;
@@ -176,7 +177,7 @@
     DBuf<float> ex_n2;
     DBuf<u64> ex_loc, ex_gath, ex_nmax;
 
-    int64_t p_tile_min_rows = 64, p_tile_queries = 0, p_use_tile_scan = 1, p_hash_variant = 0, p_classify_variant = 0, p_seq_tile = 1, p_seq_prefetch = 0, p_flat_project = 1, p_quad_tile = 1, p_select_variant = 1, p_scan_gen = 3, p_bm_stage_mb = 2048, p_single_exchange = 1, p_p2p_queries = 1, p_l2_filter = 1, p_plan_tail = 1, p_exact_budget_mb = 256;
+    int64_t p_tile_min_rows = 64, p_tile_queries = 0, p_use_tile_scan = 1, p_hash_variant = 0, p_classify_variant = 0, p_seq_tile = 1, p_seq_prefetch = 0, p_flat_project = 1, p_quad_tile = 1, p_select_variant = 1, p_scan_gen = 3, p_bm_stage_mb = 2048, p_single_exchange = 1, p_p2p_queries = 1, p_l2_filter = 1, p_l2_filter_tc = 1, p_plan_tail = 1, p_exact_budget_mb = 256;
     zb_stats st{};
 
     ForestView view() const {
@@ -390,6 +391,7 @@
         }
         make_row_tile_map(bm_tmap, bm_rows.p, members_used, dimp, 128, tile_scan_box_floats(2));
         make_row_tile_map(bm_tmap3, bm_rows.p, members_used, dimp, 64, tile_scan_box_floats(3));
+        make_row_tile_map(bm_tmap_tc, bm_rows.p, members_used, dimp, 128, 32, true);
         sync();
         bm_positions = members_used;
         bm_valid = true;
@@ -558,6 +560,7 @@
         }
         make_row_tile_map(bm_tmap, bm_rows.p, Pa, dimp, 128, tile_scan_box_floats(2));
         make_row_tile_map(bm_tmap3, bm_rows.p, Pa, dimp, 64, tile_scan_box_floats(3));
+        make_row_tile_map(bm_tmap_tc, bm_rows.p, Pa, dimp, 128, 32, true);
         sync();
         bm_positions = P;
         bm_valid = true;
@@ -649,6 +652,7 @@
         }
         b.tmap = bm_tmap;
         b.tmap3 = bm_tmap3;
+        if (opt.metric == ZB_METRIC_L2SQ || opt.metric == ZB_METRIC_L2) b.tmap_tc = bm_tmap_tc;
         b.positions = bm_positions;
         return b;
     }
@@ -1115,6 +1119,7 @@
             launch_rinv(d_q, nq, ix->dimp, ix->q_rinv.p, s);
         }
         ix->scan_ws.l2_filter = gen3 && ix->dimp >= 128 && (ix->p_l2_filter == 2 || (ix->p_l2_filter == 1 && ix->filter_backoff == 0));
+        ix->scan_ws.l2_filter_tc = ix->p_l2_filter_tc != 0;
         if (ix->filter_backoff > 0) --ix->filter_backoff;
         (gen3 ? tile_scan3 : tile_scan)(ix->scan_ws, fs, ix->bm_view(), ix->opt.metric, d_q, ix->q_rinv.p, (u32)nq, nv, ix->v_leaf.p,
                                         ix->v_np.p, ix->v_q.p, ix->v_ent_off.p, ix->v_pair_len.p, ix->v_done.p, ix->entries.p,
@@ -1199,6 +1204,7 @@
     ix->st.last_filter_rows = (u32)std::min<u64>(refined, 0xFFFFFFFFull);
     ix->st.last_ms_refine = refine_ms;
     ix->st.last_filter_used = ix->scan_ws.launched && ix->scan_ws.filtered ? 1u : 0u;
+    ix->st.last_filter_tc = ix->scan_ws.launched && ix->scan_ws.filtered_tc ? 1u : 0u;
     if (ix->scan_ws.launched && ix->scan_ws.filtered && flagged * 16 > tile_visits) ix->filter_backoff = 32;
     u64 seq_moved = 0;
     if (ix->scan_ws.seq_launched) seq_tile_scan_stats(ix->scan_ws, s, &seq_moved, &tile_ms, &tiles);
@@ -2339,6 +2345,7 @@
     else if (k == "quad_tile") ix->p_quad_tile = value;
     else if (k == "flat_project") ix->p_flat_project = value;
     else if (k == "l2_filter") { ix->p_l2_filter = value; ix->filter_backoff = 0; }
+    else if (k == "l2_filter_tc") ix->p_l2_filter_tc = value;
     else if (k == "long_list_warps") { ZB_REQUIRE(value == 4 || value == 8, ZB_ERR_INVALID, "long_list_warps is 4 or 8"); ix->scan_ws.long_list_warps = (int)value; }
     else if (k == "exact_budget_mb") {
         ZB_REQUIRE(value >= 1 && value <= (1 << 20), ZB_ERR_INVALID, "exact_budget_mb out of range");
diff --git a/zebra_b200/csrc/zb_scan.cu b/zebra_b200/csrc/zb_scan.cu
--- a/zebra_b200/csrc/zb_scan.cu
+++ b/zebra_b200/csrc/zb_scan.cu
@@ -543,12 +543,17 @@
 __device__ __forceinline__ bool t3_above_from_dot(float dot, float constant) { return above_from_dot(dot, constant); }
 }
 #include "zb_scan3_kernel.cuh"
+#include "zb_scan_tc.cuh"
 namespace zb {
 
 template <int METRIC, int KR, int TW>
 __global__ void __launch_bounds__(T3Shape<TW>::THREADS, 1) tile_scan3_kernel(const __grid_constant__ CUtensorMap tmap, ForestView f, T3Params tp) {
     extern __shared__ __align__(1024) unsigned char smem3[];
     t3_body<METRIC, 0, KR, TW>(tmap, f, tp, smem3);
+}
+__global__ void __launch_bounds__(TC_THREADS, 1) tile_scan_tc_kernel(const __grid_constant__ CUtensorMap tmap, ForestView f, T3Params tp) {
+    extern __shared__ __align__(1024) unsigned char smem_tc[];
+    tc_body(tmap, f, tp, smem_tc);
 }
 #define RF_THREADS 256
 template <int METRIC>
@@ -707,14 +712,15 @@
     }
     return fn;
 }
-void make_row_tile_map(void* out_map128, const float* bm_rows, u64 positions, int dimp, int box_rows, int box_floats) {
+void make_row_tile_map(void* out_map128, const float* bm_rows, u64 positions, int dimp, int box_rows, int box_floats, bool swizzle128) {
     CUtensorMap* m = reinterpret_cast<CUtensorMap*>(out_map128);
     cuuint64_t gdim[2] = {(cuuint64_t)dimp, (cuuint64_t)(positions ? positions : 1)};
     cuuint64_t gstride[1] = {(cuuint64_t)dimp * 4};
     cuuint32_t box[2] = {(cuuint32_t)box_floats, (cuuint32_t)box_rows};
     cuuint32_t estr[2] = {1, 1};
     CUresult r = encode_tiled_fn()(m, CU_TENSOR_MAP_DATA_TYPE_FLOAT32, 2, (void*)bm_rows, gdim, gstride, box, estr,
-                                   CU_TENSOR_MAP_INTERLEAVE_NONE, CU_TENSOR_MAP_SWIZZLE_NONE, CU_TENSOR_MAP_L2_PROMOTION_L2_256B,
+                                   CU_TENSOR_MAP_INTERLEAVE_NONE, swizzle128 ? CU_TENSOR_MAP_SWIZZLE_128B : CU_TENSOR_MAP_SWIZZLE_NONE,
+                                   CU_TENSOR_MAP_L2_PROMOTION_L2_256B,
                                    CU_TENSOR_MAP_FLOAT_OOB_FILL_NONE);
     ZB_REQUIRE(r == CUDA_SUCCESS, ZB_ERR_CUDA, "cuTensorMapEncodeTiled failed (%d)", (int)r);
 }
@@ -733,6 +739,7 @@
                u8* v_done, Entry* entries, u32 top_k, u32 min_rows, u32 tile_queries, u32 nleaves, cudaStream_t s) {
     ws.launched = false;
     ws.filtered = false;
+    ws.filtered_tc = false;
     const u32 pace_window = tile_queries >> 9;
     const bool lpt_order = false;
     tile_queries &= 0xFF;
@@ -898,12 +905,22 @@
 static void t3_launch(ScanWorkspace& ws, const ForestView& f, const BucketMajor& bm, u32 metric, const float* d_q, const double* d_q_rinv,
                       u32 nq, u32 nv, const u32* v_leaf, const u32* v_np, const u32* v_q, const u32* v_ent_off, Entry* entries, u32 top_k,
                       int kr, int nst, int qcap, int sms, const u32* ntiles, const u32* nvisits, cudaStream_t s);
+static int tc_stages(int dimp) {
+    int dev = 0, max_smem = 0;
+    cudaGetDevice(&dev);
+    cudaDeviceGetAttribute(&max_smem, cudaDevAttrMaxSharedMemoryPerBlockOptin, dev);
+    if (dimp < 128) return 0;
+    for (int nst = TC_MAX_STAGES; nst >= 3; --nst)
+        if ((size_t)tc_layout(nst, dimp).total + 1024 <= (size_t)max_smem) return nst;
+    return 0;
+}
 
 void tile_scan3(ScanWorkspace& ws, const ForestView& f, const BucketMajor& bm, u32 metric, const float* d_q, const double* d_q_rinv,
                 u32 nq, u32 nv, const u32* v_leaf, const u32* v_np, const u32* v_q, const u32* v_ent_off, u64* v_pair_len,
                 u8* v_done, Entry* entries, u32 top_k, u32 min_rows, u32 tile_queries, u32 nleaves, cudaStream_t s) {
     ws.launched = false;
     ws.filtered = false;
+    ws.filtered_tc = false;
     int nst = 0, qcap = 0;
     const int kr = t3_kr(top_k);
     if (!nv || !nleaves || top_k < 1 || top_k > T3_KL * T3_KR_MAX || !t3_config(f.dimp, kr, &nst, &qcap)) return;
@@ -971,7 +988,9 @@
                       int kr, int nst, int qcap, int sms, const u32* ntiles, const u32* nvisits, cudaStream_t s) {
     const size_t smem = t3_smem_bytes(nst, f.dimp, qcap, kr);
     const bool filt = ws.l2_filter && (metric == 1 || metric == 2) && kr == 1 && top_k <= ZB_L2_FILTER_MAX_K && bm.n2 && bm.leaf_n2max;
+    const int tc_nst = filt && ws.l2_filter_tc && bm.tmap_tc ? tc_stages(f.dimp) : 0;
     ws.filtered = filt;
+    ws.filtered_tc = tc_nst > 0;
     T3Params tp{};
     if (filt) {
         ws.q_n2.ensure(nq ? nq : 1);
@@ -983,6 +1002,10 @@
         tp.q_n2 = ws.q_n2.p;
         tp.leaf_n2max = bm.leaf_n2max;
         tp.ecoef = (float)(4 * f.chunks + 32) * 5.9604645e-8f * 1.01f;
+        if (tc_nst) {
+            const int ksteps = 4 * ((f.dimp + tc::ATOM_FLOATS - 1) / tc::ATOM_FLOATS);
+            tp.ecoef = (float)(3 * f.chunks + 20 * ksteps + 80) * 5.9604645e-8f * 1.01f;
+        }
         tp.cand = ws.cand.p;
         tp.cand_cut = ws.cand_cut.p;
         tp.cand_flag = ws.cand_flag.p;
@@ -1019,7 +1042,12 @@
         ZB_CUDA(cudaFuncSetAttribute(kern, cudaFuncAttributeMaxDynamicSharedMemorySize, (int)smem));
         kern<<<grid, threads, smem, s>>>(tmap, f, tp);
     };
-    if (filt) launch(tile_scan3_kernel<3, 1, 4>, T3Shape<4>::THREADS);
+    if (tc_nst) {
+        tp.nst = tc_nst;
+        const size_t tsmem = (size_t)tc_layout(tc_nst, f.dimp).total + 1024;
+        ZB_CUDA(cudaFuncSetAttribute(tile_scan_tc_kernel, cudaFuncAttributeMaxDynamicSharedMemorySize, (int)tsmem));
+        tile_scan_tc_kernel<<<grid, TC_THREADS, tsmem, s>>>(*reinterpret_cast<const CUtensorMap*>(bm.tmap_tc), f, tp);
+    } else if (filt) launch(tile_scan3_kernel<3, 1, 4>, T3Shape<4>::THREADS);
     else if (kr == 1) {
         if (metric == 0) launch(tile_scan3_kernel<0, 1, 4>, T3Shape<4>::THREADS);
         else if (metric == 1) launch(tile_scan3_kernel<1, 1, 4>, T3Shape<4>::THREADS);
@@ -1210,6 +1238,7 @@
                  u32 range_rows, u32 top_k, bool l2_filter, u64* out_ord, u64* out_bits, u32* out_counts, cudaStream_t s) {
     ws.launched = false;
     ws.filtered = false;
+    ws.filtered_tc = false;
     if (!nq || !top_k) return;
     if (!n) {
         const u64 tot = std::max<u64>((u64)nq * top_k, nq);
diff --git a/zebra_b200/csrc/zb_scan.cuh b/zebra_b200/csrc/zb_scan.cuh
--- a/zebra_b200/csrc/zb_scan.cuh
+++ b/zebra_b200/csrc/zb_scan.cuh
@@ -13,6 +13,8 @@
     DBuf<u8> cand_flag;
     bool l2_filter = false;
     bool filtered = false;
+    bool l2_filter_tc = true;
+    bool filtered_tc = false;
     int long_list_warps = 8;
     cudaEvent_t ev2 = nullptr;
     DBuf<long long> pj_off;
@@ -37,10 +39,11 @@
     const float* leaf_n2max = nullptr;
     const void* tmap = nullptr;
     const void* tmap3 = nullptr;
+    const void* tmap_tc = nullptr;
     u64 positions = 0;
 };
 
-void make_row_tile_map(void* out_map128, const float* bm_rows, u64 positions, int dimp, int box_rows, int box_floats);
+void make_row_tile_map(void* out_map128, const float* bm_rows, u64 positions, int dimp, int box_rows, int box_floats, bool swizzle128 = false);
 int tile_scan_box_floats(int generation);
 bool tile_scan_supported(int dimp, u32 top_k);
 void launch_rinv(const float* d_x, u64 n, int dimp, double* d_out, cudaStream_t s);
diff --git a/zebra_b200/csrc/zb_scan_tc.cuh b/zebra_b200/csrc/zb_scan_tc.cuh
--- /dev/null
+++ b/zebra_b200/csrc/zb_scan_tc.cuh
@@ -0,0 +1,346 @@
+#pragma once
+#include "zb_tc.cuh"
+
+namespace zb {
+
+#define TC_WARPS 10
+#define TC_THREADS (TC_WARPS * 32)
+#define TC_MAX_STAGES 8
+#define TC_TMEM_COLS 512u
+#define TC_ACC_COL(b) (64u * (b))
+#define TC_LO_COL(s) (128u + 32u * (s))
+#define TC_N2_FLOOR 1.2621774e-29f
+
+struct TcLayout {
+    u32 stage, qimg, sums, lists, meta, info, bars, tmem, total;
+};
+__host__ __device__ __forceinline__ TcLayout tc_layout(int nst, int dimp) {
+    const u32 natoms = (u32)(dimp + tc::ATOM_FLOATS - 1) / tc::ATOM_FLOATS;
+    TcLayout l;
+    u32 o = 0;
+    l.stage = o; o += (u32)nst * tc::ATOM_A_BYTES;
+    l.qimg = o; o += natoms * tc::ATOM_B_BYTES;
+    l.sums = o; o += 2u * tc::QN * tc::ROWS * 4u;
+    l.lists = o; o += tc::QN * 3u * T3_KL * 4u;
+    l.meta = o; o += tc::QN * 5u * 4u;
+    o = (o + 15u) & ~15u;
+    l.info = o; o += 2u * (u32)sizeof(T3TileInfo);
+    l.bars = o; o += (3u * TC_MAX_STAGES + 16u) * 8u;
+    l.tmem = o; o += 16u;
+    l.total = (o + 1023u) & ~1023u;
+    return l;
+}
+
+__device__ __forceinline__ void tc_list_block(const T3Params& tp, const float* sums, u32* s_lists, const u32* s_meta, const u32 nqt,
+                                              const u32 nrows, const u32 base, const int lw, const int lane, u64 (&thr)[4]) {
+    constexpr int NR = tc::ROWS / 32;
+    u64 gbound[4];
+#pragma unroll
+    for (int e = 0; e < 4; ++e) {
+        const u32 q = (u32)lw + 4u * e;
+        gbound[e] = t3_ldcg_u64(tp.gthr + (q < nqt ? s_meta[2 * tc::QN + q] : 0u));
+    }
+    float n2[NR];
+#pragma unroll
+    for (int i = 0; i < NR; ++i) n2[i] = (u32)(lane + 32 * i) < nrows ? tp.bm_n2[base + lane + 32 * i] : 0.f;
+    u32 tword = 0;
+    if (lane < 5 && (base >> 5) + lane <= (base + nrows - 1) >> 5) tword = tp.bm_tomb[(base >> 5) + lane];
+#pragma unroll
+    for (int e = 0; e < 4; ++e) {
+        const u32 q = (u32)lw + 4u * e;
+        if (q >= nqt) break;
+        const int np = (int)s_meta[tc::QN + q];
+        const u32 gq = s_meta[2 * tc::QN + q];
+        const u64 gb = t3_shfl64(gbound[e], 0);
+        const float n2q = t3_bitsf(s_meta[3 * tc::QN + q]), Eq = t3_bitsf(s_meta[4 * tc::QN + q]);
+        if (gb != ZB_SENTINEL) {
+            const u64 gf = (u64)t3_ford(t3_fadd_ru(t3_funord((u32)gb), Eq));
+            if (gf < thr[e]) thr[e] = gf;
+        }
+        u64 key[NR];
+        bool any = false;
+#pragma unroll
+        for (int i = 0; i < NR; ++i) {
+            key[i] = ZB_SENTINEL;
+            if ((u32)(lane + 32 * i) < nrows) {
+                const float w = t3_fadd(n2[i], n2q);
+                const float a = t3_fmaf(-2.0f, sums[(size_t)q * tc::ROWS + lane + 32 * i], w);
+                key[i] = (w <= T3_N2_LIMIT && w >= TC_N2_FLOOR && a == a) ? (u64)t3_ford(a) : 0ull;
+                any = any || key[i] <= thr[e];
+            }
+        }
+        if (!__ballot_sync(0xffffffffu, any)) continue;
+        u32* lst = s_lists + (size_t)q * 3 * T3_KL;
+        u64 Lk = ((u64)lst[T3_KL + lane] << 32) | lst[lane];
+        u32 Lp = lst[2 * T3_KL + lane];
+        u64 th = thr[e];
+#pragma unroll
+        for (int i = 0; i < NR; ++i) {
+            unsigned m = __ballot_sync(0xffffffffu, (u32)(lane + 32 * i) < nrows && key[i] <= th);
+            while (m) {
+                const int src = __ffs(m) - 1;
+                m &= m - 1;
+                const u64 nk = t3_shfl64(key[i], src);
+                if (nk > th) continue;
+                const u32 npos = base + (u32)src + 32u * i;
+                const u32 w = __shfl_sync(0xffffffffu, tword, (int)((npos >> 5) - (base >> 5)));
+                if ((w >> (npos & 31)) & 1u) continue;
+                const unsigned mm = __ballot_sync(0xffffffffu, t3_kp_less(nk, npos, Lk, Lp));
+                const int il = mm ? __ffs(mm) - 1 : T3_KL;
+                if (il >= T3_KL) continue;
+                const u64 upk = t3_shfl_up64(Lk);
+                const u32 upp = __shfl_up_sync(0xffffffffu, Lp, 1);
+                if (lane > il) { Lk = upk; Lp = upp; }
+                else if (lane == il) { Lk = nk; Lp = npos; }
+                u64 lk = t3_shfl64(Lk, np - 1);
+                if (lk != ZB_SENTINEL) lk = (u64)t3_ford(t3_fadd_ru(t3_funord((u32)lk), t3_fadd_ru(Eq, Eq)));
+                if (lk < th) th = lk;
+            }
+        }
+        lst[lane] = (u32)Lk;
+        lst[T3_KL + lane] = (u32)(Lk >> 32);
+        lst[2 * T3_KL + lane] = Lp;
+        thr[e] = th;
+        if (np == (int)tp.top_k) {
+            const u64 kn = t3_shfl64(Lk, np - 1), k0 = t3_shfl64(Lk, 0);
+            if (lane == 0 && kn != ZB_SENTINEL && k0 != 0ull) {
+                const u64 g = (u64)t3_ford(t3_fadd_ru(t3_funord((u32)kn), Eq));
+                if (g < gb) t3_atomic_min_u64(tp.gthr + gq, g);
+            }
+        }
+        __syncwarp();
+    }
+}
+
+__device__ __forceinline__ void tc_body(const CUtensorMap& tmap, const ForestView& f, const T3Params& tp, unsigned char* smem_raw) {
+    const int tid = threadIdx.x, warp = tid >> 5, lane = tid & 31;
+    const int dimp = f.dimp, natoms = (dimp + tc::ATOM_FLOATS - 1) / tc::ATOM_FLOATS;
+    const u32 S = (u32)tp.nst;
+    const TcLayout lay = tc_layout(tp.nst, dimp);
+    unsigned char* tb = smem_raw + ((1024u - (smem_u32(smem_raw) & 1023u)) & 1023u);
+    const u32 sb = smem_u32(tb);
+    T3TileInfo* s_info = reinterpret_cast<T3TileInfo*>(tb + lay.info);
+    float* s_sums = reinterpret_cast<float*>(tb + lay.sums);
+    u32* s_lists = reinterpret_cast<u32*>(tb + lay.lists);
+    u32* s_meta = reinterpret_cast<u32*>(tb + lay.meta);
+    const u32 bar_full = sb + lay.bars, bar_split = bar_full + 8 * TC_MAX_STAGES, bar_empty = bar_split + 8 * TC_MAX_STAGES;
+    const u32 bar_x = bar_empty + 8 * TC_MAX_STAGES;
+    const u32 bar_ifull = bar_x, bar_iempty = bar_x + 16, bar_afull = bar_x + 32, bar_aempty = bar_x + 48;
+    const u32 bar_sfull = bar_x + 64, bar_sempty = bar_x + 80, bar_qready = bar_x + 96, bar_qfree = bar_x + 104;
+    volatile u32* s_tmem = reinterpret_cast<volatile u32*>(tb + lay.tmem);
+
+    if (tid == 0) {
+        for (u32 i = 0; i < S; ++i) {
+            mbar_init(bar_full + 8 * i, 1);
+            mbar_init(bar_split + 8 * i, 4);
+            mbar_init(bar_empty + 8 * i, 1);
+        }
+        for (u32 i = 0; i < 2; ++i) {
+            mbar_init(bar_ifull + 8 * i, 1);
+            mbar_init(bar_iempty + 8 * i, 9);
+            mbar_init(bar_afull + 8 * i, 1);
+            mbar_init(bar_aempty + 8 * i, 4);
+            mbar_init(bar_sfull + 8 * i, 4);
+            mbar_init(bar_sempty + 8 * i, 4);
+        }
+        mbar_init(bar_qready, 4);
+        mbar_init(bar_qfree, 1);
+        t3_fence_barrier_init();
+    }
+    if (warp == 1) tc::tmem_alloc(sb + lay.tmem, TC_TMEM_COLS);
+    tc::fence_before();
+    __syncthreads();
+    tc::fence_after();
+    const u32 tmem = *s_tmem;
+
+    if (warp == 0) {
+        if (lane == 0) {
+            t3_prefetch_map(tmap);
+            const u32 ntiles = *tp.ntiles;
+            u32 buf = 0, eph = 1;
+            u32 tile = atomicAdd(tp.tile_counter, 1u);
+            for (u32 it = 0;; ++it) {
+                mbar_wait(bar_iempty + 8 * (it & 1), ((it >> 1) & 1) ^ 1u);
+                T3TileInfo* inf = s_info + (it & 1);
+                if (tile >= ntiles) {
+                    inf->tile = T3_NOTILE;
+                    mbar_arrive(bar_ifull + 8 * (it & 1));
+                    break;
+                }
+                const u32 leaf = tp.tile_leaf[tile], first = tp.tile_first[tile], nqt = tp.tile_count[tile];
+                const u32 L = f.leaf_len[leaf];
+                const long long moff = f.leaf_off[leaf];
+                inf->tile = tile; inf->leaf = leaf; inf->first = first; inf->nqt = nqt; inf->L = L; inf->qh = 0; inf->moff = moff;
+                mbar_arrive(bar_ifull + 8 * (it & 1));
+                const u32 nblocks = (L + tc::ROWS - 1) / tc::ROWS;
+                for (u32 b = 0; b < nblocks; ++b)
+                    for (int s = 0; s < natoms; ++s) {
+                        mbar_wait(bar_empty + 8 * buf, eph);
+                        mbar_arrive_expect_tx(bar_full + 8 * buf, tc::ATOM_A_BYTES);
+                        t3_tma_2d_g2s(sb + lay.stage + buf * tc::ATOM_A_BYTES, tmap, s * tc::ATOM_FLOATS, moff + (long long)b * tc::ROWS,
+                                      bar_full + 8 * buf);
+                        if (++buf == S) { buf = 0; eph ^= 1u; }
+                    }
+                const u32 next_tile = atomicAdd(tp.tile_counter, 1u);
+                atomicAdd(&tp.stats[0], (u64)nqt);
+                atomicAdd(&tp.stats[1], (u64)nqt * L);
+                atomicAdd(&tp.stats[2], ((u64)L + nqt) * (u64)dimp * 4ull);
+                tile = next_tile;
+            }
+        }
+    } else if (warp == 1) {
+        if (lane == 0) {
+            u32 buf = 0, ph = 0, ab = 0;
+            for (u32 it = 0;; ++it) {
+                mbar_wait(bar_ifull + 8 * (it & 1), (it >> 1) & 1);
+                const T3TileInfo inf = s_info[it & 1];
+                mbar_arrive(bar_iempty + 8 * (it & 1));
+                if (inf.tile == T3_NOTILE) break;
+                mbar_wait(bar_qready, it & 1);
+                const u32 nblocks = (inf.L + tc::ROWS - 1) / tc::ROWS;
+                for (u32 b = 0; b < nblocks; ++b, ++ab) {
+                    const u32 acc = tmem + TC_ACC_COL(ab & 1u);
+                    mbar_wait(bar_aempty + 8 * (ab & 1u), ((ab >> 1) & 1u) ^ 1u);
+                    tc::fence_after();
+                    for (int s = 0; s < natoms; ++s) {
+                        mbar_wait(bar_split + 8 * buf, ph);
+                        tc::fence_after();
+                        tc::mma_atom(acc, sb + lay.stage + buf * tc::ATOM_A_BYTES, sb + lay.qimg + (u32)s * tc::ATOM_B_BYTES,
+                                     tmem + TC_LO_COL(buf), s == 0);
+                        tc::commit(bar_empty + 8 * buf);
+                        if (++buf == S) { buf = 0; ph ^= 1u; }
+                    }
+                    tc::commit(bar_afull + 8 * (ab & 1u));
+                }
+                tc::commit(bar_qfree);
+            }
+        }
+    } else if (warp < 6) {
+        const int quarter = warp & 3, row = 32 * quarter + lane;
+        const u32 lanebase = (u32)(32 * quarter) << 16;
+        u32 buf = 0, ph = 0, ab = 0;
+        auto finish_block = [&](u32 blk) {
+            mbar_wait(bar_afull + 8 * (blk & 1u), (blk >> 1) & 1u);
+            tc::fence_after();
+            float sv[16];
+            tc::read_sums(tmem + lanebase + TC_ACC_COL(blk & 1u), sv);
+            tc::fence_before();
+            __syncwarp();
+            if (lane == 0) mbar_arrive(bar_aempty + 8 * (blk & 1u));
+            mbar_wait(bar_sempty + 8 * (blk & 1u), ((blk >> 1) & 1u) ^ 1u);
+            float* dst = s_sums + (size_t)(blk & 1u) * tc::QN * tc::ROWS + row;
+#pragma unroll
+            for (int j = 0; j < 16; ++j) dst[j * tc::ROWS] = sv[j];
+            __syncwarp();
+            if (lane == 0) mbar_arrive(bar_sfull + 8 * (blk & 1u));
+        };
+        for (u32 it = 0;; ++it) {
+            mbar_wait(bar_ifull + 8 * (it & 1), (it >> 1) & 1);
+            const T3TileInfo inf = s_info[it & 1];
+            __syncwarp();
+            if (lane == 0) mbar_arrive(bar_iempty + 8 * (it & 1));
+            if (inf.tile == T3_NOTILE) break;
+            if (it > 0) mbar_wait(bar_qfree, (it - 1) & 1);
+            u32 gq = 0;
+            if ((u32)lane < inf.nqt) gq = tp.v_q[tp.order[inf.first + lane]];
+            const int nqt = (int)inf.nqt;
+            tc::write_qimg(sb + lay.qimg, natoms, dimp, tid - 64, [&](int j) -> const float* {
+                const u32 g = __shfl_sync(0xffffffffu, gq, j);
+                return j < nqt ? tp.queries + (size_t)g * dimp : nullptr;
+            });
+            tc::fence_async_smem();
+            __syncwarp();
+            if (lane == 0) mbar_arrive(bar_qready);
+            const u32 nblocks = (inf.L + tc::ROWS - 1) / tc::ROWS;
+            for (u32 b = 0; b < nblocks; ++b, ++ab) {
+                for (int s = 0; s < natoms; ++s) {
+                    mbar_wait(bar_full + 8 * buf, ph);
+                    tc::split_row(sb + lay.stage + buf * tc::ATOM_A_BYTES, row, tmem + lanebase + TC_LO_COL(buf));
+                    tc::fence_before();
+                    __syncwarp();
+                    if (lane == 0) mbar_arrive(bar_split + 8 * buf);
+                    if (++buf == S) { buf = 0; ph ^= 1u; }
+                }
+                if (b > 0) finish_block(ab - 1);
+            }
+            if (nblocks) finish_block(ab - 1);
+        }
+    } else {
+        const int lw = warp - 6;
+        u32 ab = 0;
+        for (u32 it = 0;; ++it) {
+            mbar_wait(bar_ifull + 8 * (it & 1), (it >> 1) & 1);
+            const T3TileInfo inf = s_info[it & 1];
+            __syncwarp();
+            if (lane == 0) mbar_arrive(bar_iempty + 8 * (it & 1));
+            if (inf.tile == T3_NOTILE) break;
+            const u32 nqt = inf.nqt;
+            if (lane < 4) {
+                const u32 q = (u32)lw + 4u * lane;
+                if (q < nqt) {
+                    const u32 visit = tp.order[inf.first + q];
+                    s_meta[q] = visit;
+                    s_meta[tc::QN + q] = tp.v_np[visit];
+                    const u32 gq = tp.v_q[visit];
+                    s_meta[2 * tc::QN + q] = gq;
+                    const float n2q = tp.q_n2[gq];
+                    s_meta[3 * tc::QN + q] = t3_fbits(n2q);
+                    s_meta[4 * tc::QN + q] = t3_fbits(t3_fadd_ru(t3_fmul_ru(tp.ecoef, t3_fadd_ru(tp.leaf_n2max[inf.leaf], n2q)), 1e-37f));
+                }
+            }
+#pragma unroll
+            for (int e = 0; e < 4; ++e) {
+                const u32 q = (u32)lw + 4u * e;
+                if (q < nqt) {
+                    u32* lst = s_lists + (size_t)q * 3 * T3_KL;
+#pragma unroll
+                    for (int x = 0; x < 3; ++x) lst[x * T3_KL + lane] = 0xFFFFFFFFu;
+                }
+            }
+            u64 thr[4] = {ZB_SENTINEL, ZB_SENTINEL, ZB_SENTINEL, ZB_SENTINEL};
+            __syncwarp();
+            const u32 nblocks = (inf.L + tc::ROWS - 1) / tc::ROWS;
+            for (u32 b = 0; b < nblocks; ++b, ++ab) {
+                const u32 nrows = min((u32)tc::ROWS, inf.L - b * tc::ROWS);
+                const u32 base = (u32)(inf.moff + (long long)b * tc::ROWS);
+                mbar_wait(bar_sfull + 8 * (ab & 1u), (ab >> 1) & 1u);
+                tc_list_block(tp, s_sums + (size_t)(ab & 1u) * tc::QN * tc::ROWS, s_lists, s_meta, nqt, nrows, base, lw, lane, thr);
+                __syncwarp();
+                if (lane == 0) mbar_arrive(bar_sempty + 8 * (ab & 1u));
+            }
+#pragma unroll 1
+            for (int e = 0; e < 4; ++e) {
+                const u32 q = (u32)lw + 4u * e;
+                if (q >= nqt) break;
+                const u32 v = s_meta[q];
+                const int np = (int)s_meta[tc::QN + q];
+                const u32* lst = s_lists + (size_t)q * 3 * T3_KL;
+                const u64 k = ((u64)lst[T3_KL + lane] << 32) | lst[lane];
+                const u32 p = lst[2 * T3_KL + lane];
+                tp.cand[(size_t)v * T3_KL + lane] = (u64)(u32)k | ((u64)(k == ZB_SENTINEL ? T3_NOPOS : p) << 32);
+                const u64 kn = t3_shfl64(k, np - 1), k31 = t3_shfl64(k, T3_KL - 1), k0 = t3_shfl64(k, 0);
+                if (lane == 0) {
+                    const float Eq = t3_bitsf(s_meta[4 * tc::QN + q]);
+                    float cut = t3_bitsf(0x7F800000u);
+                    bool over = k0 == 0ull;
+                    if (!over && kn != ZB_SENTINEL) {
+                        cut = t3_fadd_ru(t3_funord((u32)kn), t3_fadd_ru(Eq, Eq));
+                        over = !(cut == cut) || (k31 != ZB_SENTINEL && (u32)k31 <= t3_ford(cut));
+                    }
+                    tp.cand_cut[v] = cut;
+                    tp.cand_flag[v] = over ? 1 : 0;
+                }
+            }
+            __syncwarp();
+        }
+    }
+    __syncwarp();
+    tc::fence_before();
+    __syncthreads();
+    if (warp == 1) {
+        tc::fence_after();
+        tc::tmem_free(tmem, TC_TMEM_COLS);
+    }
+}
+
+}
diff --git a/zebra_b200/csrc/zb_tc.cuh b/zebra_b200/csrc/zb_tc.cuh
--- /dev/null
+++ b/zebra_b200/csrc/zb_tc.cuh
@@ -0,0 +1,139 @@
+#pragma once
+#include <cstdint>
+
+namespace zb {
+namespace tc {
+
+constexpr int ATOM_FLOATS = 32;
+constexpr int ROWS = 128;
+constexpr int QN = 16;
+constexpr uint32_t ATOM_A_BYTES = ROWS * 128;
+constexpr uint32_t ATOM_B_BYTES = 2 * QN * 128;
+
+__host__ __device__ __forceinline__ uint32_t tf32_hi_bits(uint32_t b) { return b & 0xFFFFE000u; }
+
+__device__ __forceinline__ uint64_t sw128_desc(uint32_t saddr) {
+    return (uint64_t)((saddr >> 4) & 0x3FFFu)
+         | (uint64_t)1u << 16
+         | (uint64_t)(1024u >> 4) << 32
+         | (uint64_t)1u << 46
+         | (uint64_t)2u << 61;
+}
+__host__ __device__ constexpr uint32_t idesc_tf32(int n) {
+    return (1u << 4) | (2u << 7) | (2u << 10) | ((uint32_t)(n >> 3) << 17) | ((uint32_t)(ROWS >> 4) << 24);
+}
+
+__device__ __forceinline__ void mma_ss(uint32_t d, uint64_t a, uint64_t b, uint32_t idesc, uint32_t acc) {
+    asm volatile("{.reg .pred p; setp.ne.u32 p, %4, 0;\n"
+                 "tcgen05.mma.cta_group::1.kind::tf32 [%0], %1, %2, %3, p;}" ::"r"(d), "l"(a), "l"(b), "r"(idesc), "r"(acc));
+}
+__device__ __forceinline__ void mma_ts(uint32_t d, uint32_t a_tmem, uint64_t b, uint32_t idesc, uint32_t acc) {
+    asm volatile("{.reg .pred p; setp.ne.u32 p, %4, 0;\n"
+                 "tcgen05.mma.cta_group::1.kind::tf32 [%0], [%1], %2, %3, p;}" ::"r"(d), "r"(a_tmem), "l"(b), "r"(idesc), "r"(acc));
+}
+__device__ __forceinline__ void commit(uint32_t bar) {
+    asm volatile("tcgen05.commit.cta_group::1.mbarrier::arrive::one.shared::cluster.b64 [%0];" ::"r"(bar) : "memory");
+}
+__device__ __forceinline__ void fence_before() { asm volatile("tcgen05.fence::before_thread_sync;" ::: "memory"); }
+__device__ __forceinline__ void fence_after() { asm volatile("tcgen05.fence::after_thread_sync;" ::: "memory"); }
+__device__ __forceinline__ void fence_async_smem() { asm volatile("fence.proxy.async.shared::cta;" ::: "memory"); }
+__device__ __forceinline__ void tmem_alloc(uint32_t dst_saddr, uint32_t cols) {
+    asm volatile("tcgen05.alloc.cta_group::1.sync.aligned.shared::cta.b32 [%0], %1;" ::"r"(dst_saddr), "r"(cols) : "memory");
+    asm volatile("tcgen05.relinquish_alloc_permit.cta_group::1.sync.aligned;" ::: "memory");
+}
+__device__ __forceinline__ void tmem_free(uint32_t base, uint32_t cols) {
+    asm volatile("tcgen05.dealloc.cta_group::1.sync.aligned.b32 %0, %1;" ::"r"(base), "r"(cols) : "memory");
+}
+
+__device__ __forceinline__ void mma_atom(uint32_t acc, uint32_t a_stage, uint32_t b_atom, uint32_t lo_a, bool first) {
+#pragma unroll
+    for (int kk = 0; kk < 4; ++kk) {
+        const uint64_t ad = sw128_desc(a_stage + 32u * kk), bd = sw128_desc(b_atom + 32u * kk);
+        const uint32_t on = (first && kk == 0) ? 0u : 1u;
+        mma_ss(acc, ad, bd, idesc_tf32(32), on);
+        mma_ts(acc + 32u, lo_a + 8u * kk, bd, idesc_tf32(16), on);
+    }
+}
+
+__device__ __forceinline__ void split_row(uint32_t stage_saddr, int row, uint32_t tm) {
+    uint32_t v[32];
+    const uint32_t rbase = stage_saddr + (uint32_t)row * 128u;
+#pragma unroll
+    for (int c = 0; c < 8; ++c) {
+        const uint32_t addr = rbase + (uint32_t)((c ^ (row & 7)) << 4);
+        float x0, x1, x2, x3;
+        asm volatile("ld.shared.v4.f32 {%0, %1, %2, %3}, [%4];" : "=f"(x0), "=f"(x1), "=f"(x2), "=f"(x3) : "r"(addr));
+        const float xs[4] = {x0, x1, x2, x3};
+#pragma unroll
+        for (int e = 0; e < 4; ++e) {
+            const float hi = __uint_as_float(tf32_hi_bits(__float_as_uint(xs[e])));
+            v[4 * c + e] = __float_as_uint(__fsub_rn(xs[e], hi));
+        }
+    }
+    asm volatile(
+        "tcgen05.st.sync.aligned.32x32b.x32.b32 [%0], {%1, %2, %3, %4, %5, %6, %7, %8, %9, %10, %11, %12, %13, %14, %15, %16, "
+        "%17, %18, %19, %20, %21, %22, %23, %24, %25, %26, %27, %28, %29, %30, %31, %32};" ::"r"(tm),
+        "r"(v[0]), "r"(v[1]), "r"(v[2]), "r"(v[3]), "r"(v[4]), "r"(v[5]), "r"(v[6]), "r"(v[7]), "r"(v[8]), "r"(v[9]), "r"(v[10]),
+        "r"(v[11]), "r"(v[12]), "r"(v[13]), "r"(v[14]), "r"(v[15]), "r"(v[16]), "r"(v[17]), "r"(v[18]), "r"(v[19]), "r"(v[20]),
+        "r"(v[21]), "r"(v[22]), "r"(v[23]), "r"(v[24]), "r"(v[25]), "r"(v[26]), "r"(v[27]), "r"(v[28]), "r"(v[29]), "r"(v[30]),
+        "r"(v[31])
+        : "memory");
+    asm volatile("tcgen05.wait::st.sync.aligned;" ::: "memory");
+}
+
+template <class QRow>
+__device__ __forceinline__ void write_qimg(uint32_t img_saddr, int natoms, int dimp, int tid, QRow qrow) {
+    constexpr int B = 8;
+    const int c = tid & 7, j = (tid >> 3) & (QN - 1);
+    const float* q = qrow(j);
+    const uint32_t off = img_saddr + (uint32_t)((c ^ (j & 7)) << 4);
+    for (int s0 = 0; s0 < natoms; s0 += B) {
+        float4 x[B];
+#pragma unroll
+        for (int u = 0; u < B; ++u) {
+            const int k = (s0 + u) * ATOM_FLOATS + 4 * c;
+            x[u] = make_float4(0.f, 0.f, 0.f, 0.f);
+            if (q && s0 + u < natoms && k < dimp) x[u] = __ldg(reinterpret_cast<const float4*>(q + k));
+        }
+#pragma unroll
+        for (int u = 0; u < B; ++u) {
+            if (s0 + u >= natoms) break;
+            const float xs[4] = {x[u].x, x[u].y, x[u].z, x[u].w};
+            uint32_t m[4], l[4];
+#pragma unroll
+            for (int e = 0; e < 4; ++e) {
+                m[e] = tf32_hi_bits(__float_as_uint(xs[e]));
+                l[e] = __float_as_uint(__fsub_rn(xs[e], __uint_as_float(m[e])));
+            }
+            const uint32_t o = off + (uint32_t)(s0 + u) * ATOM_B_BYTES;
+            asm volatile("st.shared.v4.b32 [%0], {%1, %2, %3, %4};" ::"r"(o + (uint32_t)j * 128u), "r"(m[0]), "r"(m[1]), "r"(m[2]), "r"(m[3])
+                         : "memory");
+            asm volatile("st.shared.v4.b32 [%0], {%1, %2, %3, %4};" ::"r"(o + (uint32_t)(QN + j) * 128u), "r"(l[0]), "r"(l[1]), "r"(l[2]),
+                         "r"(l[3])
+                         : "memory");
+        }
+    }
+}
+
+__device__ __forceinline__ void tmem_ld16(uint32_t tm, float (&x)[16]) {
+    uint32_t v[16];
+    asm volatile(
+        "tcgen05.ld.sync.aligned.32x32b.x16.b32 {%0, %1, %2, %3, %4, %5, %6, %7, %8, %9, %10, %11, %12, %13, %14, %15}, [%16];"
+        : "=r"(v[0]), "=r"(v[1]), "=r"(v[2]), "=r"(v[3]), "=r"(v[4]), "=r"(v[5]), "=r"(v[6]), "=r"(v[7]), "=r"(v[8]), "=r"(v[9]),
+          "=r"(v[10]), "=r"(v[11]), "=r"(v[12]), "=r"(v[13]), "=r"(v[14]), "=r"(v[15])
+        : "r"(tm));
+    asm volatile("tcgen05.wait::ld.sync.aligned;" ::: "memory");
+#pragma unroll
+    for (int i = 0; i < 16; ++i) x[i] = __uint_as_float(v[i]);
+}
+__device__ __forceinline__ void read_sums(uint32_t acc, float (&s)[16]) {
+    float hh[16], hl[16], d2[16];
+    tmem_ld16(acc, hh);
+    tmem_ld16(acc + 16u, hl);
+    tmem_ld16(acc + 32u, d2);
+#pragma unroll
+    for (int j = 0; j < 16; ++j) s[j] = __fadd_rn(hh[j], __fadd_rn(hl[j], d2[j]));
+}
+
+}
+}
```

Result: faster. 2.692 million (median of 6 runs) (+2.3%).
